# c976237222/HunyuanVideo_efficiency

Measured on AMD Instinct MI355X. Metric: denoise-steps/sec (720x1280x129f, HunyuanVideo DiT 20+40 blocks, bf16), higher is better.
Workload: dtype bf16

## Files before the change

hunyuanvideo_efficiency_amd/_lib.py:

```python
from __future__ import annotations

import ctypes as C
import os
import re

_HERE = os.path.dirname(os.path.abspath(__file__))
LIB_PATH = os.path.join(_HERE, "lib", "libhv_kernels.so")
TORCH_OPS_PATH = os.path.join(_HERE, "lib", "libhv_torch_ops.so")
ABI_VERSION = 8

_p, _i, _l, _f = C.c_void_p, C.c_int, C.c_int64, C.c_float

SIGNATURES = {
    "hv_abi_version": [],
    "hv_ln_modulate_bf16": [_p, _p, _p, _p, _l, _i, _l, _l, _f, _i, _p],
    "hv_qknorm_rope_bf16": [_p, _p, _p, _p, _p, _l, _l, _i, _i, _l, _l, _f, _p],
    "hv_qknorm_rope_scatter_bf16": [_p, _p, _p, _p, _p, _l, _l, _i, _i, _l, _l, _f, _p, _l, _i, _l, _p],
    "hv_gemm_bf16": [_p, _l, _p, _l, _p, _i, _i, _i, _p, _l, _i, _i, _p, _l, _i, _p, _p, _l, _p],
    "hv_linear_smallm_bf16": [_p, _p, _p, _p, _p, _i, _i, _i, _l, _l, _i, _p],
    "hv_timestep_embedding_bf16": [_p, _p, _i, _i, _f, _p],
    "hv_attn_fwd_bf16": [_p, _p, _p, _p, _l, _l, _l, _l, _i, _i, _i, _i, _f, _p, _l, _p],
    "hv_attn_workspace_bytes": [_i, _i, _i],
    "hv_attn_w4_loop_signature": [],
    "hv_attn_partial_bf16": [_p, _p, _p, _l, _l, _l, _i, _i, _i, _i, _f, _p, _p, _i, _i, _i, _p],
    "hv_attn_merge_bf16": [_p, _p, _p, _l, _i, _i, _i, _p],
    "hv_attn_suggest_splits": [_i, _i, _i],
    "hv_patchify_f32_bf16": [_p, _p, _i, _i, _i, _i, _p],
    "hv_unpatchify_bf16": [_p, _p, _i, _i, _i, _i, _l, _p],
    "hv_euler_step_f32": [_p, _p, _f, _l, _p],
    "hv_euler_step_f32_f32": [_p, _p, _f, _l, _p],
    "hv_masked_mean_bf16": [_p, _p, _p, _i, _i, _p],
    "hv_broadcast_row_bf16": [_p, _p, _l, _i, _l, _p],
    "hv_copy3d_bf16": [_p, _p, _i, _l, _i, _l, _l, _l, _l, _p],
    "hv_fp8_dequant_bf16": [_p, _p, _p, _l, _p],
    "hv_ln_modulate_fp8": [_p, _p, _p, _p, _p, _l, _i, _l, _l, _f, _p],
    "hv_quant_rows_fp8": [_p, _l, _p, _l, _p, _l, _i, _p],
    "hv_gemm_fp8": [_p, _l, _p, _p, _l, _p, _p, _i, _i, _i, _p, _l, _i, _i, _p, _l, _i, _p, _p, _l, _p],
    "hv_gemm_f16": [_p, _l, _p, _l, _p, _i, _i, _i, _p, _l, _i, _p, _l, _p],
    "hv_conv3d_causal_f16": [_p, _l, _p, _p, _p, _l, _i, _i, _i, _i, _i, _i, _i, _p, _l, _p, _l, _p],
    "hv_gn_partial_rows": [_l],
    "hv_subpixel_gn_partial_rows": [_i, _i, _i, _i],
    "hv_groupnorm_finalize_f16": [_p, _l, _l, _l, _i, _i, _f, _p, _p, _p, _p],
    "hv_groupnorm_affine_f16": [_p, _l, _l, _i, _i, _f, _p, _p, _p, _l, _p, _p],
    "hv_groupnorm_apply_f16": [_p, _l, _p, _l, _l, _i, _p, _i, _p],
    "hv_softmax_rows_f32_f16": [_p, _l, _p, _l, _i, _i, _i, _f, _i, _p],
    "hv_transpose_16b": [_p, _l, _p, _l, _i, _i, _p],
    "hv_conv3d_upsampled_subpixel_f16": [_p, _l, _p, _p, _i, _p, _p, _l, _i, _i, _i, _i, _i, _i, _p, _l, _p],
    "hv_conv3d_cout4_f16": [_p, _l, _p, _i, _p, _p, _p, _l, _i, _i, _i, _i, _i, _p, _l, _p],
    "hv_conv3d_cout4_planes_floats": [_l],
    "hv_conv3d_causal_strided_f16": [_p, _l, _p, _p, _p, _l, _i, _i, _i, _i, _i, _i, _i, _i, _p],
    "hv_temporal_resample_f16": [_p, _l, _p, _l, _i, _l, _i, _i, _i, _i, _p],
    "hv_vae_latent_tile_f16": [_p, _l, _l, _l, _l, _i, _i, _i, _i, _i, _p, _p],
    "hv_vae_blend_f16": [_p, _p, _p, _p, _p, _i, _i, _p],
    "hv_copy4d_16b": [_p, _p, _p, _p, _p, _p],
    "hv_vae_postprocess_f16_f32": [_p, _p, _l, _p],
    "hv_video_metrics": [_p, _l, _l, _l, _p, _l, _l, _l, _i, _i, _i, _i, _i, _i, _i, _p, _p, _p, _p, _l, _p],
    "hv_video_metrics_workspace_bytes": [_i, _i, _i, _i],
    "hv_lpips_conv1_f32": [_p, _l, _l, _l, _p, _l, _l, _l, _i, _i, _i, _i, _i, _p, _p, _p, _p, _p],
    "hv_lpips_conv2d_f32": [_p, _p, _p, _p, _i, _i, _i, _i, _i, _i, _i, _p],
    "hv_lpips_maxpool_f32": [_p, _p, _i, _i, _i, _i, _p],
    "hv_lpips_distance_f32": [_p, _p, _i, _l, _i, _i, _p, _p, _l, _p],
    "hv_lpips_distance_workspace_bytes": [_i, _l],
}


class HVKernelError(RuntimeError):
    pass


_lib = None


def load():
    global _lib
    if _lib is not None:
        return _lib
    if not os.path.exists(LIB_PATH):
        raise HVKernelError(
            f"{LIB_PATH} is missing: the HIP extension is not built (run __graft_entry__.build()). "
            "hunyuanvideo_efficiency_amd has no CPU or eager fallback.")
    lib = C.CDLL(LIB_PATH)
    for name, argtypes in SIGNATURES.items():
        try:
            fn = getattr(lib, name)
        except AttributeError as e:
            raise HVKernelError(f"{LIB_PATH} does not export {name}") from e
        fn.argtypes = argtypes
        fn.restype = C.c_int64 if name in ("hv_attn_workspace_bytes", "hv_gn_partial_rows", "hv_subpixel_gn_partial_rows", "hv_conv3d_cout4_planes_floats",
                                            "hv_video_metrics_workspace_bytes", "hv_lpips_distance_workspace_bytes") else C.c_int
    v = lib.hv_abi_version()
    if v != ABI_VERSION:
        raise HVKernelError(f"libhv_kernels ABI {v} != expected {ABI_VERSION}: rebuild the extension")
    inc = os.path.join(_HERE, "csrc", "hv_attention_w4_loop.inc")
    if os.path.exists(inc) and os.environ.get("HV_ALLOW_EXPERIMENT_LIB") != "1":
        with open(inc) as f:
            m = re.search(r"#define HV_W4_LOOP_SIGNATURE 0x([0-9a-f]{8})u", f.read(600))
        if m is None or (lib.hv_attn_w4_loop_signature() & 0xFFFFFFFF) != int(m.group(1), 16):
            raise HVKernelError(f"{LIB_PATH} was not compiled from {inc}: rebuild the extension (make -C hunyuanvideo_efficiency_amd/csrc); "
                                "HV_ALLOW_EXPERIMENT_LIB=1 admits a library built from another checkout (same-box A/Bs: tools/ab_attn.sh, tools/ab_run.sh)")
    _lib = lib
    return lib


def check(code: int, what: str):
    if code != 0:
        raise HVKernelError(f"{what} failed with code {code} "
                            f"({'bad argument' if code == -1 else 'launch failure' if code == -2 else 'unknown'})")


_hv = None


def torch_ops():
    global _hv
    if _hv is not None:
        return _hv
    import torch
    if not os.path.exists(TORCH_OPS_PATH):
        raise HVKernelError(
            f"{TORCH_OPS_PATH} is missing: the PyTorch custom-op library is not built (run __graft_entry__.build()). "
            "hunyuanvideo_efficiency_amd has no CPU or eager fallback.")
    torch.ops.load_library(TORCH_OPS_PATH)
    hv = torch.ops.hv
    v = int(hv.abi_version())
    if v != ABI_VERSION:
        raise HVKernelError(f"libhv_torch_ops / libhv_kernels ABI {v} != expected {ABI_VERSION}: rebuild the extension")
    for name in SIGNATURES:
        if not hasattr(hv, name[len("hv_"):]):
            raise HVKernelError(f"{TORCH_OPS_PATH} does not register torch.ops.hv.{name[len('hv_'):]}")
    _hv = hv
    return hv


def call(name: str, *args):
    op = getattr(torch_ops(), name)
    try:
        return op(*args)
    except (RuntimeError, NotImplementedError) as e:
        raise HVKernelError(f"hv::{name}: {str(e).splitlines()[0]}") from e


def host(name: str, *args) -> int:
    return int(getattr(torch_ops(), name)(*args))
```

hunyuanvideo_efficiency_amd/csrc/hv_api.hip:

```cpp
#include "hv_common.hpp"
#include "../../include/hv_kernels.h"
extern "C" int hv_abi_version(void) { return 8; }
```

hunyuanvideo_efficiency_amd/csrc/hv_attention.hip:

```cpp
#include "hv_attention.hpp"

using namespace hv_attn;

namespace {

constexpr int QTILE = 256;

__global__ __launch_bounds__(256) void attn_combine_kernel(const float* __restrict__ part_o, const float* __restrict__ part_ml,
                                                            bf16_t* __restrict__ o, int64_t so, int n_q, int n_heads, int n_splits) {
    const int64_t idx = (int64_t)blockIdx.x * blockDim.x + threadIdx.x;
    const int64_t total = (int64_t)n_q * n_heads * 32;
    if (idx >= total) return;
    const int d4 = (int)(idx & 31);
    const int64_t rh = idx >> 5;
    const int head = (int)(rh % n_heads);
    const int64_t row = rh / n_heads;
    float m = -INFINITY;
    for (int s = 0; s < n_splits; ++s) m = fmaxf(m, part_ml[(((int64_t)s * n_q + row) * n_heads + head) * 2]);
    float4 acc = make_float4(0.f, 0.f, 0.f, 0.f);
    float l = 0.f;
    for (int s = 0; s < n_splits; ++s) {
        const int64_t ri = ((int64_t)s * n_q + row) * n_heads + head;
        const float w = __builtin_amdgcn_exp2f(part_ml[ri * 2] - m);
        const float4 v = *reinterpret_cast<const float4*>(part_o + ri * D + d4 * 4);
        acc.x += v.x * w; acc.y += v.y * w; acc.z += v.z * w; acc.w += v.w * w;
        l += part_ml[ri * 2 + 1] * w;
    }
    const float inv = 1.0f / l;
    u32x2 w2;
    w2[0] = pack_bf2(acc.x * inv, acc.y * inv);
    w2[1] = pack_bf2(acc.z * inv, acc.w * inv);
    *reinterpret_cast<u32x2*>(o + row * so + head * D + d4 * 4) = w2;
}

int attn_launch(const AttnArgs& a, dim3 grid, hipStream_t stream) { return launch_w4(a, grid, stream); }

constexpr int KMAX_ROWS = 2048;
__global__ __launch_bounds__(256) void attn_kmax_kernel(const bf16_t* __restrict__ k, int64_t sk, int n_kv, unsigned* __restrict__ out) {
    __shared__ float wmax[4];
    const int head = blockIdx.y, t = threadIdx.x, ch = t & 15;
    const int r0 = blockIdx.x * KMAX_ROWS, r1 = min(r0 + KMAX_ROWS, n_kv);
    float best = 0.f;
    for (int row = r0 + (t >> 4); row < r1; row += 16) {
        const u32x4 w = *reinterpret_cast<const u32x4*>(k + (int64_t)row * sk + head * D + ch * 8);
        float s = 0.f;
#pragma unroll
        for (int j = 0; j < 4; ++j) {
            const float lo = bf2f_lo(w[j]), hi = bf2f_hi(w[j]);
            s += lo * lo + hi * hi;
        }
#pragma unroll
        for (int o = 8; o > 0; o >>= 1) s += __shfl_xor(s, o, 64);
        best = fmaxf(best, s);
    }
    best = fmaxf(best, __shfl_xor(best, 16, 64));
    best = fmaxf(best, __shfl_xor(best, 32, 64));
    if ((t & 63) == 0) wmax[t >> 6] = best;
    __syncthreads();
    if (t == 0) atomicMax(out + head, __float_as_uint(fmaxf(fmaxf(wmax[0], wmax[1]), fmaxf(wmax[2], wmax[3]))));
}

int attn_prepare_kmax(AttnArgs& a, void* workspace, int64_t workspace_bytes, hipStream_t stream) {
    a.kmax2 = nullptr;
    if (!workspace || workspace_bytes < KMAX_BYTES || a.n_heads > KMAX_HEADS || a.n_kv < 64 * KVT) return HV_OK;
    if (hipMemsetAsync(workspace, 0, KMAX_BYTES, stream) != hipSuccess) return HV_ERR_LAUNCH;
    attn_kmax_kernel<<<dim3((unsigned)((a.n_kv + KMAX_ROWS - 1) / KMAX_ROWS), (unsigned)a.n_heads), dim3(256), 0, stream>>>(a.k, a.sk, a.n_kv, (unsigned*)workspace);
    a.kmax2 = (const unsigned*)workspace;
    return HV_OK;
}

}

extern "C" int64_t hv_attn_workspace_bytes(int n_q, int n_kv, int n_heads) {
    (void)n_kv;
    return (int64_t)KMAX_BYTES + (int64_t)2 * n_q * n_heads * (128 + 2) * (int64_t)sizeof(float);
}

extern "C" int hv_attn_fwd_bf16(const void* q, const void* k, const void* v, void* o, int64_t stride_q, int64_t stride_k,
                                int64_t stride_v, int64_t stride_o, int n_q, int n_kv, int n_heads, int head_dim,
                                float scale, void* workspace, int64_t workspace_bytes, hipStream_t stream) {
    if (!q || !k || !v || !o || head_dim != D || n_heads <= 0 || n_q < 0 || n_kv < 0 || (stride_q & 7) || (stride_k & 7) ||
        (stride_v & 7) || (stride_o & 3))
        return HV_ERR_ARG;
    if (n_q == 0) return HV_OK;
    if (n_kv == 0) return HV_ERR_ARG;
    AttnArgs a;
    a.q = (const bf16_t*)q; a.k = (const bf16_t*)k; a.v = (const bf16_t*)v; a.o = (bf16_t*)o;
    a.sq = stride_q; a.sk = stride_k; a.sv = stride_v; a.so = stride_o;
    a.n_q = n_q; a.n_kv = n_kv; a.n_heads = n_heads;
    a.n_qtiles = (n_q + QTILE - 1) / QTILE;
    a.scale_log2e = scale * 1.4426950408889634f;
    a.n_splits = 1; a.split_keys = n_kv; a.part_o = nullptr; a.part_ml = nullptr; a.partial = 0;
    if (attn_prepare_kmax(a, workspace, workspace_bytes, stream) != HV_OK) return HV_ERR_LAUNCH;
    {
        const int64_t nwg = (int64_t)a.n_qtiles * n_heads;
        const int ntile = (n_kv + KVT - 1) / KVT;
        const double r1 = (double)((nwg + 255) / 256), r2 = 0.5 * (double)((2 * nwg + 255) / 256);
        if (workspace && ntile >= 64 && r2 < 0.97 * r1 && workspace_bytes >= hv_attn_workspace_bytes(n_q, n_kv, n_heads)) {
            a.n_splits = 2;
            a.split_keys = ((ntile + 1) / 2) * KVT;
            a.part_o = (float*)((char*)workspace + KMAX_BYTES);
            a.part_ml = a.part_o + (int64_t)2 * n_q * n_heads * D;
        }
    }
    if (attn_launch(a, dim3((unsigned)(a.n_qtiles * n_heads), (unsigned)a.n_splits), stream) != HV_OK) return HV_ERR_LAUNCH;
    if (a.n_splits > 1) {
        const int64_t total = (int64_t)n_q * n_heads * 32;
        attn_combine_kernel<<<dim3((unsigned)((total + 255) / 256)), dim3(256), 0, stream>>>(a.part_o, a.part_ml, a.o, a.so, n_q, n_heads,
                                                                                           a.n_splits);
    }
    return hv_check_launch();
}

extern "C" int hv_attn_partial_bf16(const void* q, const void* k, const void* v, int64_t stride_q, int64_t stride_k, int64_t stride_v,
                                    int n_q, int n_kv, int n_heads, int head_dim, float scale, void* part_o, void* part_ml,
                                    int n_slots, int slot, int splits, hipStream_t stream) {
    if (!q || !k || !v || !part_o || !part_ml || head_dim != D || n_heads <= 0 || n_q < 0 || n_kv <= 0 || (stride_q & 7) ||
        (stride_k & 7) || (stride_v & 7) || (splits != 1 && splits != 2) || slot < 0 || slot + splits > n_slots)
        return HV_ERR_ARG;
    if (n_q == 0) return HV_OK;
    const int ntile = (n_kv + KVT - 1) / KVT;
    if (splits == 2 && ntile < 2) return HV_ERR_ARG;
    AttnArgs a;
    a.q = (const bf16_t*)q; a.k = (const bf16_t*)k; a.v = (const bf16_t*)v; a.o = nullptr;
    a.sq = stride_q; a.sk = stride_k; a.sv = stride_v; a.so = 0;
    a.n_q = n_q; a.n_kv = n_kv; a.n_heads = n_heads;
    a.n_qtiles = (n_q + QTILE - 1) / QTILE;
    a.scale_log2e = scale * 1.4426950408889634f;
    a.n_splits = splits;
    a.split_keys = splits == 2 ? ((ntile + 1) / 2) * KVT : n_kv;
    a.part_o = (float*)part_o + (int64_t)slot * n_q * n_heads * D;
    a.part_ml = (float*)part_ml + (int64_t)slot * n_q * n_heads * 2;
    a.partial = 1;
    a.kmax2 = nullptr;
    if (attn_launch(a, dim3((unsigned)(a.n_qtiles * n_heads), (unsigned)splits), stream) != HV_OK) return HV_ERR_LAUNCH;
    return hv_check_launch();
}

extern "C" int hv_attn_merge_bf16(const void* part_o, const void* part_ml, void* o, int64_t stride_o, int n_q, int n_heads, int n_slots,
                                  hipStream_t stream) {
    if (!part_o || !part_ml || !o || n_heads <= 0 || n_q < 0 || n_slots <= 0 || (stride_o & 3)) return HV_ERR_ARG;
    if (n_q == 0) return HV_OK;
    const int64_t total = (int64_t)n_q * n_heads * 32;
    attn_combine_kernel<<<dim3((unsigned)((total + 255) / 256)), dim3(256), 0, stream>>>((const float*)part_o, (const float*)part_ml,
                                                                                       (bf16_t*)o, stride_o, n_q, n_heads, n_slots);
    return hv_check_launch();
}

extern "C" int hv_attn_suggest_splits(int n_q, int n_kv, int n_heads) {
    const int64_t nwg = (int64_t)((n_q + QTILE - 1) / QTILE) * n_heads;
    const int ntile = (n_kv + KVT - 1) / KVT;
    const double r1 = (double)((nwg + 255) / 256), r2 = 0.5 * (double)((2 * nwg + 255) / 256);
    return (ntile >= 64 && r2 < 0.97 * r1) ? 2 : 1;
}
```

hunyuanvideo_efficiency_amd/csrc/hv_attention.hpp:

```cpp
#pragma once
#include "hv_common.hpp"
#include "../../include/hv_kernels.h"
#include <type_traits>

namespace hv_attn {

constexpr int D = 128;
constexpr int KVT = 64;
constexpr int KV_TILE_BYTES = KVT * D * 2;

struct AttnArgs {
    const bf16_t* q; const bf16_t* k; const bf16_t* v; bf16_t* o;
    int64_t sq, sk, sv, so;
    int n_q, n_kv, n_heads, n_qtiles;
    float scale_log2e;
    int n_splits, split_keys;
    float* part_o;
    float* part_ml;
    int partial;
    const unsigned* kmax2;
};
constexpr int KMAX_BYTES = 256;
constexpr int KMAX_HEADS = 62;

typedef __attribute__((ext_vector_type(4))) short s16x4;
typedef __attribute__((address_space(3))) s16x4* lds_s16x4_ptr;
typedef __attribute__((address_space(3))) void* lds_void_ptr;

__device__ __forceinline__ float half_swap_max(float v) {
    auto r = __builtin_amdgcn_permlane32_swap(__float_as_uint(v), __float_as_uint(v), false, false);
    return fmaxf(__uint_as_float(r[0]), __uint_as_float(r[1]));
}
__device__ __forceinline__ float half_swap_sum(float v) {
    auto r = __builtin_amdgcn_permlane32_swap(__float_as_uint(v), __float_as_uint(v), false, false);
    return __uint_as_float(r[0]) + __uint_as_float(r[1]);
}

template <int I, int N, typename F>
__device__ __forceinline__ void static_for(F&& f) {
    if constexpr (I < N) {
        f(std::integral_constant<int, I>{});
        static_for<I + 1, N>(f);
    }
}

int launch_w4(const AttnArgs& a, dim3 grid, hipStream_t stream);

}
```

hunyuanvideo_efficiency_amd/csrc/hv_attention_w4.hip:

```cpp
#include "hv_attention.hpp"
#include "hv_agpr_clobbers.inc"

using namespace hv_attn;

namespace {

constexpr int W4_WAVES = 4, W4_QTILE = 256, W4_NBUF = 4;
constexpr int W4_KOFF = 0, W4_VOFF = W4_NBUF * KV_TILE_BYTES;
constexpr int W4_LDS = 2 * W4_NBUF * KV_TILE_BYTES;
constexpr int A_O = 0, A_Q = 128, A_KF = 192, A_VF = 224;
constexpr int RING = 8;
constexpr int PF = 4;
constexpr int WGRP = 2;
__host__ __device__ constexpr int frag_insts(int f) { return (f >= 16 && f < 32) ? 2 : 1; }
__host__ __device__ constexpr int wait_for(int f) { int n = 0; for (int i = WGRP; i < PF; ++i) n += frag_insts(f + i); return n; }

template <int KF, int QF, int WAIT>
__device__ __forceinline__ void mfma_s_first(f32x16& s, const f32x16& c) {
    if constexpr (WAIT >= 0)
        asm volatile("s_waitcnt lgkmcnt(%c6)\n\tv_mfma_f32_32x32x16_bf16 %0, a[%c2:%c3], a[%c4:%c5], %1"
                     : "=&v"(s) : "v"(c), "i"(KF), "i"(KF + 3), "i"(QF), "i"(QF + 3), "i"(WAIT) : HV_CLOBBER_ALL_AGPRS);
    else
        asm volatile("v_mfma_f32_32x32x16_bf16 %0, a[%c2:%c3], a[%c4:%c5], %1"
                     : "=&v"(s) : "v"(c), "i"(KF), "i"(KF + 3), "i"(QF), "i"(QF + 3) : HV_CLOBBER_ALL_AGPRS);
}
template <int KF, int QF, int WAIT>
__device__ __forceinline__ void mfma_s_zero(f32x16& s) {
    if constexpr (WAIT >= 0)
        asm volatile("s_waitcnt lgkmcnt(%c5)\n\tv_mfma_f32_32x32x16_bf16 %0, a[%c1:%c2], a[%c3:%c4], 0"
                     : "=&v"(s) : "i"(KF), "i"(KF + 3), "i"(QF), "i"(QF + 3), "i"(WAIT));
    else
        asm volatile("v_mfma_f32_32x32x16_bf16 %0, a[%c1:%c2], a[%c3:%c4], 0" : "=&v"(s) : "i"(KF), "i"(KF + 3), "i"(QF), "i"(QF + 3));
}
template <int KF, int QF, int WAIT>
__device__ __forceinline__ void mfma_s(f32x16& s) {
    if constexpr (WAIT >= 0)
        asm volatile("s_waitcnt lgkmcnt(%c5)\n\tv_mfma_f32_32x32x16_bf16 %0, a[%c1:%c2], a[%c3:%c4], %0"
                     : "+v"(s) : "i"(KF), "i"(KF + 3), "i"(QF), "i"(QF + 3), "i"(WAIT) : HV_CLOBBER_ALL_AGPRS);
    else
        asm volatile("v_mfma_f32_32x32x16_bf16 %0, a[%c1:%c2], a[%c3:%c4], %0" : "+v"(s) : "i"(KF), "i"(KF + 3), "i"(QF), "i"(QF + 3) : HV_CLOBBER_ALL_AGPRS);
}
template <int OT, int VF, int WAIT>
__device__ __forceinline__ void mfma_pv(const u32x4& p) {
    if constexpr (WAIT >= 0)
        asm volatile("s_waitcnt lgkmcnt(%c5)\n\tv_mfma_f32_32x32x16_bf16 a[%c1:%c2], a[%c3:%c4], %0, a[%c1:%c2]"
                     : : "v"(p), "i"(OT), "i"(OT + 15), "i"(VF), "i"(VF + 3), "i"(WAIT) : HV_CLOBBER_ALL_AGPRS);
    else
        asm volatile("v_mfma_f32_32x32x16_bf16 a[%c1:%c2], a[%c3:%c4], %0, a[%c1:%c2]" : : "v"(p), "i"(OT), "i"(OT + 15), "i"(VF), "i"(VF + 3) : HV_CLOBBER_ALL_AGPRS);
}
template <int AF, int OFF>
__device__ __forceinline__ void lds_k(uint32_t addr) {
    asm volatile("ds_read_b128 a[%c1:%c2], %0 offset:%c3" : : "v"(addr), "i"(AF), "i"(AF + 3), "i"(OFF));
}
template <int AF, int OFF>
__device__ __forceinline__ void lds_v(uint32_t addr) {
    asm volatile("ds_read_b64_tr_b16 a[%c1:%c2], %0 offset:%c5\n\tds_read_b64_tr_b16 a[%c3:%c4], %0 offset:%c6"
                 : : "v"(addr), "i"(AF), "i"(AF + 1), "i"(AF + 2), "i"(AF + 3), "i"(OFF), "i"(OFF + 8 * 256));
}
__device__ __forceinline__ void add_pinned(float& acc, float p) { asm volatile("v_add_f32 %0, %0, %1" : "+v"(acc) : "v"(p)); }
__device__ __forceinline__ void exp2_pinned(float& d, float x) { asm volatile("v_exp_f32 %0, %1" : "=v"(d) : "v"(x)); }
__device__ __forceinline__ void pack_pinned(uint32_t& w, float lo, float hi) { asm volatile("v_cvt_pk_bf16_f32 %0, %1, %2" : "=v"(w) : "v"(lo), "v"(hi)); }
__device__ __forceinline__ void max3_pinned(float& acc, float x, float y) { asm volatile("v_max3_f32 %0, %0, %1, %2" : "+v"(acc) : "v"(x), "v"(y)); }
template <int N>
__device__ __forceinline__ void acc_write(uint32_t v) { asm volatile("v_accvgpr_write_b32 a%c1, %0" : : "v"(v), "i"(N)); }
template <int N>
__device__ __forceinline__ float acc_read() {
    float v;
    asm volatile("v_accvgpr_read_b32 %0, a%c1" : "=v"(v) : "i"(N));
    return v;
}

#include "hv_attention_w4_loop.inc"

__host__ __device__ constexpr int exps_before(int g) { return g <= 32 ? g + (g + 3) / 4 : (g <= 56 ? 40 + (g - 32) : 64); }
__host__ __device__ constexpr int exps_in(int g) { return exps_before(g + 1) - exps_before(g); }

__global__ __launch_bounds__(256, 1) void attn_fwd_kernel_w4(AttnArgs a) {
#if defined(__HIP_DEVICE_COMPILE__)
    extern __shared__ __attribute__((aligned(16))) char smem[];
    const int tid = threadIdx.x, lane = tid & 63, wave = tid >> 6;
    const int lr = lane & 31, lh = lane >> 5;
    const int head = blockIdx.x / a.n_qtiles;
    const int qt = blockIdx.x % a.n_qtiles;
    if (a.n_splits > 1) {
        const int kv0 = blockIdx.y * a.split_keys;
        a.k += (int64_t)kv0 * a.sk;
        a.v += (int64_t)kv0 * a.sv;
        a.n_kv = min(a.n_kv - kv0, a.split_keys);
    }
    const int q0 = qt * W4_QTILE + wave * 64;
    const uint32_t lds0 = (uint32_t)(uintptr_t)smem;

    asm volatile("; hv_attention_w4: a[0:255] owned by inline asm" : : : HV_CLOBBER_ALL_AGPRS);
    static_for<0, 128>([&](auto I) { asm volatile("v_accvgpr_write_b32 a%c0, 0" : : "i"(A_O + decltype(I)::value)); });
    float qn2[2] = {0.f, 0.f};
#pragma unroll
    for (int qb = 0; qb < 2; ++qb) {
        const int qrow = min(q0 + qb * 32 + lr, a.n_q - 1);
        const bf16_t* qp = a.q + (int64_t)qrow * a.sq + head * D + lh * 8;
        u32x4 raw[8];
#pragma unroll
        for (int ks = 0; ks < 8; ++ks) raw[ks] = *reinterpret_cast<const u32x4*>(qp + ks * 16);
        static_for<0, 32>([&](auto I) {
            constexpr int i = decltype(I)::value;
            const uint32_t w = raw[i >> 2][i & 3];
            const uint32_t sc = pack_bf2(bf2f_lo(w) * a.scale_log2e, bf2f_hi(w) * a.scale_log2e);
            qn2[qb] += bf2f_lo(sc) * bf2f_lo(sc) + bf2f_hi(sc) * bf2f_hi(sc);
            if (qb == 0) acc_write<A_Q + i>(sc);
            else acc_write<A_Q + 32 + i>(sc);
        });
    }

    constexpr int KEYS_W = KVT / W4_WAVES, NP = KEYS_W / 4;
    const char* kbase = reinterpret_cast<const char*>(a.k + head * D);
    const char* vbase = reinterpret_cast<const char*>(a.v + head * D);
    const int k_row_bytes = (int)a.sk * 2, v_row_bytes = (int)a.sv * 2;
    uint32_t koff_row, koff_sw, voff0;
    {
        const int key = KEYS_W * wave + (lane >> 4), dcp = lane & 15;
        koff_row = (uint32_t)(key * k_row_bytes);
        koff_sw = (uint32_t)((dcp ^ (key & 3)) << 4);
        voff0 = (uint32_t)(key * v_row_bytes + ((dcp ^ ((key & 3) << 2)) << 4));
    }
    u32x4 koff4, voff4;
#pragma unroll
    for (int i = 0; i < NP; ++i) {
        koff4[i] = koff_row + (koff_sw ^ (uint32_t)(i << 6)) + (uint32_t)(4 * i * k_row_bytes) - (uint32_t)(i * 1024);
        voff4[i] = voff0 + (uint32_t)(4 * i * v_row_bytes) - (uint32_t)(i * 1024);
    }
    const int wave_u = __builtin_amdgcn_readfirstlane(wave);
    const int wave_lds = wave_u * (KEYS_W * 256);
    const int64_t k_tile_bytes = (int64_t)KVT * a.sk * 2, v_tile_bytes = (int64_t)KVT * a.sv * 2;
    auto k_rsrc = [&](const char* tile_ptr, int rows) { return __builtin_amdgcn_make_buffer_rsrc((void*)tile_ptr, 0, rows * k_row_bytes, 0x00020000); };
    auto v_rsrc = [&](const char* tile_ptr, int rows) { return __builtin_amdgcn_make_buffer_rsrc((void*)tile_ptr, 0, rows * v_row_bytes, 0x00020000); };
    auto dma_k_piece = [&](auto rsrc, int lds_off, int i) {
        __builtin_amdgcn_raw_ptr_buffer_load_lds(rsrc, (lds_void_ptr)(smem + lds_off + wave_lds + i * 1024), 16, koff_row + (koff_sw ^ (uint32_t)(i << 6)), 4 * i * k_row_bytes, 0, 0);
    };
    auto dma_v_piece = [&](auto rsrc, int lds_off, int i) {
        __builtin_amdgcn_raw_ptr_buffer_load_lds(rsrc, (lds_void_ptr)(smem + lds_off + wave_lds + i * 1024), 16, voff0, 4 * i * v_row_bytes, 0, 0);
    };
    auto tile_rows = [&](int tile) { return min(a.n_kv - tile * KVT, KVT); };
    auto dma_k = [&](int tile, int buf) {
        auto r = k_rsrc(kbase + tile * k_tile_bytes, tile_rows(tile));
#pragma unroll
        for (int i = 0; i < NP; ++i) dma_k_piece(r, W4_KOFF + buf * KV_TILE_BYTES, i);
    };
    auto dma_v = [&](int tile, int buf) {
        auto r = v_rsrc(vbase + tile * v_tile_bytes, tile_rows(tile));
#pragma unroll
        for (int i = 0; i < NP; ++i) dma_v_piece(r, W4_VOFF + buf * KV_TILE_BYTES, i);
    };

    uint32_t kread0, vread;
    {
        kread0 = lds0 + W4_KOFF + lr * 256 + ((lh ^ (lr & 15)) << 4);
        const int vq = (lane & 15) >> 2, vp = lane & 3, vG = lane >> 4;
        const int key = 4 * (vG >> 1) + vq;
        const int chunk16 = ((vG & 1) * 16 + 4 * vp) >> 3;
        vread = lds0 + W4_VOFF + key * 256 + ((chunk16 ^ ((key & 3) << 2)) << 4) + (vp & 1) * 8;
    }
    u32x4 vks_lo, vks_hi, vv4;
#pragma unroll
    for (int i = 0; i < 4; ++i) {
        vks_lo[i] = kread0 ^ (uint32_t)(i << 5);
        vks_hi[i] = kread0 ^ (uint32_t)((i + 4) << 5);
        vv4[i] = vread ^ (uint32_t)(i << 6);
    }
    uint32_t vk0, vv[4];
    auto set_vk = [&](int buf_bytes) { vk0 = kread0 + buf_bytes; };
    auto set_vv = [&](int buf_bytes) {
        const uint32_t b = vread + buf_bytes;
#pragma unroll
        for (int db = 0; db < 4; ++db) vv[db] = b ^ (db << 6);
    };

    float m_run[2] = {0.f, 0.f}, l_run[2] = {0.f, 0.f};
    float l2_run[2] = {0.f, 0.f};
    f32x16 negm[2];
    constexpr float THR = 8.0f;
    bool static_max = false;
    const int ntiles = (a.n_kv + KVT - 1) / KVT;

    auto tile_max = [&](f32x16 (&S)[2][2], int t, bool last, float (&mx)[2]) __attribute__((always_inline)) {
        if (last && (a.n_kv & (KVT - 1))) {
            const int kbase_i = t * KVT + 4 * lh;
#pragma unroll
            for (int qb = 0; qb < 2; ++qb)
#pragma unroll
                for (int kb = 0; kb < 2; ++kb)
#pragma unroll
                    for (int r = 0; r < 16; ++r) {
                        const int key = kbase_i + kb * 32 + (r & 3) + 8 * (r >> 2);
                        if (key >= a.n_kv) S[qb][kb][r] = -INFINITY;
                    }
        }
#pragma unroll
        for (int qb = 0; qb < 2; ++qb) {
            float m = S[qb][0][0];
#pragma unroll
            for (int r = 1; r < 16; ++r) m = fmaxf(m, S[qb][0][r]);
#pragma unroll
            for (int r = 0; r < 16; ++r) m = fmaxf(m, S[qb][1][r]);
            mx[qb] = half_swap_max(m);
        }
    };
    auto raise_max = [&](f32x16 (&Sc)[2][2], const float (&mx)[2]) __attribute__((always_inline)) {
        asm volatile("s_nop 7\n\ts_nop 7\n\ts_nop 7" ::: "memory");
        static_for<0, 2>([&](auto QB) {
            constexpr int qb = decltype(QB)::value;
            if (__any(mx[qb] > THR)) {
                const float d = fmaxf(half_swap_max(mx[qb]), 0.f);
                const float alpha = __builtin_amdgcn_exp2f(-d);
                l_run[qb] = (l_run[qb] + l2_run[qb]) * alpha;
                l2_run[qb] = 0.f;
                m_run[qb] += d;
#pragma unroll
                for (int kb = 0; kb < 2; ++kb)
#pragma unroll
                    for (int r = 0; r < 16; ++r) Sc[qb][kb][r] -= d;
#pragma unroll
                for (int r = 0; r < 16; ++r) negm[qb][r] = -m_run[qb];
                static_for<0, 64>([&](auto I) {
                    constexpr int n = A_O + 64 * qb + decltype(I)::value;
                    float o = acc_read<n>();
                    o *= alpha;
                    acc_write<n>(__float_as_uint(o));
                });
                asm volatile("s_nop 3" ::: "memory");
            }
        });
        asm volatile("" : "+v"(negm[0]), "+v"(negm[1]));
    };

    auto body = [&](f32x16 (&Sc)[2][2], f32x16 (&Sn)[2][2], int t, const float (&mx_c)[2], float (&mx_n)[2]) __attribute__((always_inline)) {
        constexpr bool FULL = false;
        if (!static_max && __any(mx_c[0] > THR || mx_c[1] > THR)) raise_max(Sc, mx_c);
        const int rb0 = (t & 3) * KV_TILE_BYTES, rb2 = ((t + 2) & 3) * KV_TILE_BYTES, rb3 = ((t + 3) & 3) * KV_TILE_BYTES;
        const bool do_k = FULL || (t + 3 < ntiles), do_v = FULL || (t + 2 < ntiles);
        u32x4 pw[2][4];
        float ex[64];
        float mxa[2] = {-INFINITY, -INFINITY};
        const auto krs = k_rsrc(kbase + (FULL ? t + 3 : min(t + 3, ntiles - 1)) * k_tile_bytes, FULL ? KVT : tile_rows(min(t + 3, ntiles - 1)));
        const auto vrs = v_rsrc(vbase + (FULL ? t + 2 : min(t + 2, ntiles - 1)) * v_tile_bytes, FULL ? KVT : tile_rows(min(t + 2, ntiles - 1)));
        auto add_e = [&](auto Ec) {
            constexpr int e = decltype(Ec)::value, qb = (e >> 3) & 1;
            add_pinned(l_run[qb], ex[e]);
        };
        auto exp_e = [&](auto Ec) {
            constexpr int e = decltype(Ec)::value, kk = e >> 4, qb = (e >> 3) & 1, j = e & 7;
            exp2_pinned(ex[e], Sc[qb][kk >> 1][8 * (kk & 1) + j]);
        };
        auto pack_e = [&](auto Ec) {
            constexpr int e = decltype(Ec)::value, kk = e >> 4, qb = (e >> 3) & 1, j = e & 7;
            if constexpr (j & 1) {
                uint32_t w;
// ... 264 lines not shown
```

hunyuanvideo_efficiency_amd/csrc/hv_common.hpp:

```cpp
#pragma once
#include <hip/hip_runtime.h>
#include <stdint.h>

#define HV_OK 0
#define HV_ERR_ARG (-1)
#define HV_ERR_LAUNCH (-2)

typedef __attribute__((ext_vector_type(8))) __bf16 bf16x8;
typedef __attribute__((ext_vector_type(4))) __bf16 bf16x4;
typedef __attribute__((ext_vector_type(2))) __bf16 bf16x2;
typedef __attribute__((ext_vector_type(4))) float f32x4;
typedef __attribute__((ext_vector_type(16))) float f32x16;
typedef __attribute__((ext_vector_type(4))) uint32_t u32x4;
typedef __attribute__((ext_vector_type(2))) uint32_t u32x2;
typedef __attribute__((ext_vector_type(2))) float f32x2;

typedef uint16_t bf16_t;

__device__ __forceinline__ float bf2f(bf16_t v) { return __uint_as_float(((uint32_t)v) << 16); }
__device__ __forceinline__ float bf2f_lo(uint32_t w) { return __uint_as_float(w << 16); }
__device__ __forceinline__ float bf2f_hi(uint32_t w) { return __uint_as_float(w & 0xFFFF0000u); }
__device__ __forceinline__ bf16_t f2bf(float f) {
    __bf16 h = (__bf16)f;
    return __builtin_bit_cast(bf16_t, h);
}
__device__ __forceinline__ uint32_t pack_bf2(float lo, float hi) {
    bf16x2 v;
    v[0] = (__bf16)lo;
    v[1] = (__bf16)hi;
    return __builtin_bit_cast(uint32_t, v);
}
__device__ __forceinline__ float rbf(float f) { return bf2f(f2bf(f)); }

__device__ __forceinline__ void unpack8(const u32x4& w, float (&f)[8]) {
#pragma unroll
    for (int i = 0; i < 4; ++i) {
        f[2 * i] = bf2f_lo(w[i]);
        f[2 * i + 1] = bf2f_hi(w[i]);
    }
}
__device__ __forceinline__ u32x4 pack8(const float (&f)[8]) {
    u32x4 w;
#pragma unroll
    for (int i = 0; i < 4; ++i) w[i] = pack_bf2(f[2 * i], f[2 * i + 1]);
    return w;
}

typedef _Float16 h16;
__device__ __forceinline__ float h2f(uint16_t v) { return (float)__builtin_bit_cast(h16, v); }
__device__ __forceinline__ uint16_t f2h(float f) { return __builtin_bit_cast(uint16_t, (h16)f); }
__device__ __forceinline__ float rh(float f) { return (float)(h16)f; }
__device__ __forceinline__ void unpack8h(const u32x4& w, float (&f)[8]) {
#pragma unroll
    for (int i = 0; i < 4; ++i) {
        f[2 * i] = h2f((uint16_t)(w[i] & 0xFFFFu));
        f[2 * i + 1] = h2f((uint16_t)(w[i] >> 16));
    }
}
__device__ __forceinline__ u32x4 pack8h(const float (&f)[8]) {
    u32x4 w;
#pragma unroll
    for (int i = 0; i < 4; ++i) w[i] = (uint32_t)f2h(f[2 * i]) | ((uint32_t)f2h(f[2 * i + 1]) << 16);
    return w;
}

template <typename T, typename Op>
__device__ __forceinline__ T wave_reduce(T v, Op op) {
#pragma unroll
    for (int o = 32; o > 0; o >>= 1) v = op(v, __shfl_xor(v, o, 64));
    return v;
}
struct WaveAdd {
    template <typename T> __device__ __forceinline__ T operator()(T a, T b) const { return a + b; }
};
struct WaveMax {
    __device__ __forceinline__ float operator()(float a, float b) const { return fmaxf(a, b); }
    __device__ __forceinline__ int operator()(int a, int b) const { return max(a, b); }
};
struct WaveMin {
    __device__ __forceinline__ int operator()(int a, int b) const { return min(a, b); }
};
template <typename T> __device__ __forceinline__ T wave_sum(T v) { return wave_reduce(v, WaveAdd{}); }
template <typename T> __device__ __forceinline__ T wave_max(T v) { return wave_reduce(v, WaveMax{}); }
template <typename T> __device__ __forceinline__ T wave_min(T v) { return wave_reduce(v, WaveMin{}); }

__device__ __forceinline__ float gelu_tanh_f(float x) {
    const float k0 = 0.7978845608028654f, k1 = 0.044715f;
    float u = k0 * (x + k1 * x * x * x);
    float e = __builtin_amdgcn_exp2f(u * 2.8853900817779268f);
    float t = 1.0f - 2.0f * __builtin_amdgcn_rcpf(e + 1.0f);
    return 0.5f * x * (1.0f + t);
}
__device__ __forceinline__ float silu_f(float x) { return x * __builtin_amdgcn_rcpf(1.0f + __expf(-x)); }

__device__ __forceinline__ uint32_t quantise(float x, int rescale) {
    if (rescale) x = __fmul_rn(__fadd_rn(x, 1.0f), 0.5f);
    x = fminf(fmaxf(x, 0.0f), 1.0f);
    return (uint32_t)(int)__fmul_rn(x, 255.0f);
}

struct HvPerDeviceOnce { bool done[64] = {}; };
static inline int hv_set_max_lds(HvPerDeviceOnce& once, const void* fn, int bytes) {
    int dev = 0;
    if (hipGetDevice(&dev) != hipSuccess || dev < 0 || dev >= 64) return HV_ERR_LAUNCH;
    if (!once.done[dev]) {
        if (hipFuncSetAttribute(fn, hipFuncAttributeMaxDynamicSharedMemorySize, bytes) != hipSuccess) return HV_ERR_LAUNCH;
        once.done[dev] = true;
    }
    return HV_OK;
}

static inline int hv_check_launch() {
    hipError_t e = hipGetLastError();
    return e == hipSuccess ? HV_OK : HV_ERR_LAUNCH;
}

__device__ __forceinline__ f32x2 f16x2_minus(uint32_t w, float plo, float phi) {
    float lo, hi;
    asm("v_fma_mix_f32 %0, %1, 1.0, -%2 op_sel_hi:[1,0,0]" : "=v"(lo) : "v"(w), "v"(plo));
    asm("v_fma_mix_f32 %0, %1, 1.0, -%2 op_sel:[1,0,0] op_sel_hi:[1,0,0]" : "=v"(hi) : "v"(w), "v"(phi));
    return f32x2{lo, hi};
}
```

hunyuanvideo_efficiency_amd/csrc/hv_rowwise.hip:

```cpp
#include "hv_common.hpp"
#include "../../include/hv_kernels.h"
#include <type_traits>


template <int MAXC>
__device__ __forceinline__ float ln_load_row(const bf16_t* xr, int lane, int nchunk, float (&v)[MAXC][8]) {
    float s = 0.f;
#pragma unroll
    for (int c = 0; c < MAXC; ++c) {
        const int ch = lane + c * 64;
        if (ch < nchunk) {
            unpack8(*reinterpret_cast<const u32x4*>(xr + ch * 8), v[c]);
#pragma unroll
            for (int j = 0; j < 8; ++j) s += v[c][j];
        }
    }
    return s;
}
__device__ __forceinline__ void ln_load_coeffs(const bf16_t* mul, const bf16_t* add, int ch, int mode,
                                               float (&m)[8], float (&a)[8]) {
    if (mul) {
        unpack8(*reinterpret_cast<const u32x4*>(mul + ch * 8), m);
        if (mode == 0) {
#pragma unroll
// ... 113 lines not shown
            }
        }
    }
    const float rstd = rsqrtf(wave_sum(q) / (float)D + eps);
    float amax = 0.f;
#pragma unroll
    for (int c = 0; c < MAXC; ++c) {
        const int ch = lane + c * 64;
        if (ch < nchunk) {
            float m[8], a[8];
            ln_load_coeffs(mul, add, ch, 0, m, a);
#pragma unroll
            for (int j = 0; j < 8; ++j) {
                v[c][j] = rbf((v[c][j] - mean) * rstd * m[j] + a[j]);
                amax = fmaxf(amax, fabsf(v[c][j]));
            }
        }
    }
    const float sc = fp8_row_scale(wave_max(amax));
    const float inv = 1.0f / sc;
    if (lane == 0) row_scale[row] = sc;
    uint8_t* orow = out + row * ldo;
#pragma unroll
    for (int c = 0; c < MAXC; ++c) {
        const int ch = lane + c * 64;
        if (ch < nchunk) *reinterpret_cast<u32x2*>(orow + ch * 8) = pack8_fp8(v[c], inv);
    }
}

extern "C" int hv_ln_modulate_fp8(const void* x, const void* shift, const void* scale, void* out_q, float* out_row_scale, int64_t M,
                                  int D, int64_t ldx, int64_t ldq, float eps, hipStream_t stream) {
    if (!x || !out_q || !out_row_scale || M < 0 || D <= 0 || (D & 7) || D > 4096 || (ldx & 7) || (ldq & 15)) return HV_ERR_ARG;
    if (M == 0) return HV_OK;
    dim3 grid((unsigned)((M + 3) / 4)), block(256);
    const bf16_t *xp = (const bf16_t*)x, *ap = (const bf16_t*)shift, *mp = (const bf16_t*)scale;
    ln_dispatch_maxc(D, [&](auto maxc) {
        ln_mod_fp8_kernel<decltype(maxc)::value><<<grid, block, 0, stream>>>(xp, ap, mp, (uint8_t*)out_q, out_row_scale, M, D, ldx, ldq, eps);
    });
    return hv_check_launch();
}

__global__ __launch_bounds__(256) void quant_rows_fp8_kernel(const bf16_t* __restrict__ x, int64_t ldx, uint8_t* __restrict__ out,
                                                              int64_t ldo, float* __restrict__ row_scale, int64_t M, int K) {
    const int lane = threadIdx.x & 63;
    const int64_t row = (int64_t)blockIdx.x * 4 + (threadIdx.x >> 6);
    if (row >= M) return;
    const bf16_t* xr = x + row * ldx;
    const int nchunk = K >> 3;
    float amax = 0.f;
    for (int ch = lane; ch < nchunk; ch += 64) {
        float f[8];
        unpack8(*reinterpret_cast<const u32x4*>(xr + ch * 8), f);
#pragma unroll
        for (int j = 0; j < 8; ++j) amax = fmaxf(amax, fabsf(f[j]));
    }
    const float sc = fp8_row_scale(wave_max(amax));
    const float inv = 1.0f / sc;
    if (lane == 0) row_scale[row] = sc;
    uint8_t* orow = out + row * ldo;
    for (int ch = lane; ch < nchunk; ch += 64) {
        float f[8];
        unpack8(*reinterpret_cast<const u32x4*>(xr + ch * 8), f);
        *reinterpret_cast<u32x2*>(orow + ch * 8) = pack8_fp8(f, inv);
    }
}

extern "C" int hv_quant_rows_fp8(const void* x, int64_t ldx, void* out_q, int64_t ldq, float* out_row_scale, int64_t M, int K,
                                 hipStream_t stream) {
    if (!x || !out_q || !out_row_scale || M < 0 || K <= 0 || (K & 7) || (ldx & 7) || (ldq & 15)) return HV_ERR_ARG;
    if (M == 0) return HV_OK;
    quant_rows_fp8_kernel<<<dim3((unsigned)((M + 3) / 4)), dim3(256), 0, stream>>>((const bf16_t*)x, ldx, (uint8_t*)out_q, ldq,
                                                                                  out_row_scale, M, K);
    return hv_check_launch();
}

__global__ __launch_bounds__(256) void qknorm_rope_kernel(bf16_t* __restrict__ qkv, const bf16_t* __restrict__ qw,
                                                           const bf16_t* __restrict__ kw, const float* __restrict__ cosT,
                                                           const float* __restrict__ sinT, int64_t n_rows, int64_t n_rope,
                                                           int H, int64_t ld, int64_t k_off, float eps, bf16_t* __restrict__ dst,
                                                           int64_t dst_ld, int hpb, int64_t dst_bs) {
    const int64_t row = blockIdx.x;
    const int sub = threadIdx.x & 15;
    const int grp = threadIdx.x >> 4;
    float wq[8], wk[8], c[8], s[8];
    unpack8(*reinterpret_cast<const u32x4*>(qw + sub * 8), wq);
    unpack8(*reinterpret_cast<const u32x4*>(kw + sub * 8), wk);
    const bool rope = row < n_rope;
    if (rope) {
        const float4* cp = reinterpret_cast<const float4*>(cosT + row * 128 + sub * 8);
        const float4* sp = reinterpret_cast<const float4*>(sinT + row * 128 + sub * 8);
        float4 c0 = cp[0], c1 = cp[1], s0 = sp[0], s1 = sp[1];
        c[0] = c0.x, c[1] = c0.y, c[2] = c0.z, c[3] = c0.w, c[4] = c1.x, c[5] = c1.y, c[6] = c1.z, c[7] = c1.w;
        s[0] = s0.x, s[1] = s0.y, s[2] = s0.z, s[3] = s0.w, s[4] = s1.x, s[5] = s1.y, s[6] = s1.z, s[7] = s1.w;
    }
    for (int hv = grp; hv < 2 * H; hv += 16) {
        const bool is_k = hv >= H;
        const int h = is_k ? hv - H : hv;
        bf16_t* p = qkv + row * ld + (is_k ? k_off : 0) + h * 128 + sub * 8;
        float x[8];
        unpack8(*reinterpret_cast<const u32x4*>(p), x);
        if (dst) p = dst + (int64_t)(hv / hpb) * dst_bs + row * dst_ld + (hv % hpb) * 128 + sub * 8;
        float ss = 0.f;
#pragma unroll
        for (int j = 0; j < 8; ++j) ss += x[j] * x[j];
#pragma unroll
        for (int o = 8; o > 0; o >>= 1) ss += __shfl_xor(ss, o, 16);
        const float r = rsqrtf(ss * (1.0f / 128.0f) + eps);
        float y[8];
#pragma unroll
        for (int j = 0; j < 8; ++j) y[j] = rbf(rbf(x[j] * r) * (is_k ? wk[j] : wq[j]));
        if (rope) {
            float o[8];
#pragma unroll
            for (int j = 0; j < 8; j += 2) {
                o[j] = y[j] * c[j] - y[j + 1] * s[j];
                o[j + 1] = y[j + 1] * c[j + 1] + y[j] * s[j + 1];
            }
            *reinterpret_cast<u32x4*>(p) = pack8(o);
        } else {
            *reinterpret_cast<u32x4*>(p) = pack8(y);
        }
    }
}

extern "C" int hv_qknorm_rope_bf16(void* qkv, const void* q_weight, const void* k_weight, const float* cos_tab,
                                   const float* sin_tab, int64_t n_rows, int64_t n_rope, int n_heads, int head_dim,
                                   int64_t ld, int64_t k_offset, float eps, hipStream_t stream) {
    if (!qkv || !q_weight || !k_weight || head_dim != 128 || n_heads <= 0 || n_rows < 0 || n_rope < 0 ||
        n_rope > n_rows || (ld & 7) || (k_offset & 7) || (n_rope > 0 && (!cos_tab || !sin_tab)))
        return HV_ERR_ARG;
    if (n_rows == 0) return HV_OK;
    qknorm_rope_kernel<<<dim3((unsigned)n_rows), dim3(256), 0, stream>>>((bf16_t*)qkv, (const bf16_t*)q_weight,
                                                                          (const bf16_t*)k_weight, cos_tab, sin_tab, n_rows,
                                                                          n_rope, n_heads, ld, k_offset, eps, nullptr, 0, 1, 0);
    return hv_check_launch();
}

extern "C" int hv_qknorm_rope_scatter_bf16(const void* qkv, const void* q_weight, const void* k_weight, const float* cos_tab,
                                           const float* sin_tab, int64_t n_rows, int64_t n_rope, int n_heads, int head_dim,
                                           int64_t ld, int64_t k_offset, float eps, void* dst, int64_t dst_ld,
                                           int heads_per_block, int64_t dst_block_stride, hipStream_t stream) {
    if (!qkv || !dst || !q_weight || !k_weight || head_dim != 128 || n_heads <= 0 || n_rows < 0 || n_rope < 0 || n_rope > n_rows ||
        (ld & 7) || (k_offset & 7) || (dst_ld & 7) || (dst_block_stride & 7) || heads_per_block <= 0 ||
        (n_rope > 0 && (!cos_tab || !sin_tab)))
        return HV_ERR_ARG;
    if (n_rows == 0) return HV_OK;
    qknorm_rope_kernel<<<dim3((unsigned)n_rows), dim3(256), 0, stream>>>((bf16_t*)const_cast<void*>(qkv), (const bf16_t*)q_weight,
                                                                          (const bf16_t*)k_weight, cos_tab, sin_tab, n_rows, n_rope,
                                                                          n_heads, ld, k_offset, eps, (bf16_t*)dst, dst_ld,
                                                                          heads_per_block, dst_block_stride);
    return hv_check_launch();
}

template <int MM>
__global__ __launch_bounds__(256) void gemv_kernel(const bf16_t* __restrict__ x, const bf16_t* __restrict__ W,
                                                    const bf16_t* __restrict__ b, const bf16_t* __restrict__ addend,
                                                    bf16_t* __restrict__ out, int N, int K, int64_t ldx, int64_t ldo, int act) {
    const int lane = threadIdx.x & 63;
    const int n = blockIdx.x * 4 + (threadIdx.x >> 6);
    if (n >= N) return;
    float acc[MM];
#pragma unroll
    for (int m = 0; m < MM; ++m) acc[m] = 0.f;
    const bf16_t* wr = W + (int64_t)n * K;
    for (int k0 = lane * 8; k0 < K; k0 += 512) {
        float w[8];
        unpack8(*reinterpret_cast<const u32x4*>(wr + k0), w);
#pragma unroll
        for (int m = 0; m < MM; ++m) {
            float xv[8];
            unpack8(*reinterpret_cast<const u32x4*>(x + m * ldx + k0), xv);
#pragma unroll
            for (int j = 0; j < 8; ++j) {
                float a = xv[j];
                if (act & 1) a = rbf(silu_f(a));
                acc[m] += a * w[j];
            }
        }
    }
#pragma unroll
    for (int m = 0; m < MM; ++m) {
        float r = wave_sum(acc[m]);
        if (lane == 0) {
            if (b) r += bf2f(b[n]);
            if (act & 2) r = silu_f(rbf(r));
            if (addend) r = rbf(r) + bf2f(addend[m * ldo + n]);
            out[m * ldo + n] = f2bf(r);
        }
    }
}

extern "C" int hv_linear_smallm_bf16(const void* x, const void* W, const void* bias, const void* addend, void* out, int M,
                                     int N, int K, int64_t ldx, int64_t ldo, int act, hipStream_t stream) {
    if (!x || !W || !out || M < 1 || M > 4 || N < 1 || K < 8 || (K & 7) || (ldx & 7)) return HV_ERR_ARG;
    dim3 grid((N + 3) / 4), block(256);
    const bf16_t *xp = (const bf16_t*)x, *wp = (const bf16_t*)W, *bp = (const bf16_t*)bias, *ap = (const bf16_t*)addend;
    bf16_t* op = (bf16_t*)out;
    switch (M) {
        case 1: gemv_kernel<1><<<grid, block, 0, stream>>>(xp, wp, bp, ap, op, N, K, ldx, ldo, act); break;
        case 2: gemv_kernel<2><<<grid, block, 0, stream>>>(xp, wp, bp, ap, op, N, K, ldx, ldo, act); break;
        case 3: gemv_kernel<3><<<grid, block, 0, stream>>>(xp, wp, bp, ap, op, N, K, ldx, ldo, act); break;
        default: gemv_kernel<4><<<grid, block, 0, stream>>>(xp, wp, bp, ap, op, N, K, ldx, ldo, act); break;
    }
    return hv_check_launch();
}

__global__ __launch_bounds__(256) void patchify_kernel(const float* __restrict__ x, bf16_t* __restrict__ A, int C, int T,
                                                        int H, int W) {
    const int Hp = H >> 1, Wp = W >> 1;
    const int64_t ntok = (int64_t)T * Hp * Wp;
    const int64_t idx = (int64_t)blockIdx.x * blockDim.x + threadIdx.x;
    if (idx >= ntok * C) return;
    const int c = (int)(idx % C);
    const int64_t tok = idx / C;
    const int w = (int)(tok % Wp), h = (int)((tok / Wp) % Hp), t = (int)(tok / ((int64_t)Wp * Hp));
    const float* p = x + (((int64_t)c * T + t) * H + 2 * h) * W + 2 * w;
    float2 r0 = *reinterpret_cast<const float2*>(p);
    float2 r1 = *reinterpret_cast<const float2*>(p + W);
    u32x2 o;
    o[0] = pack_bf2(r0.x, r0.y);
    o[1] = pack_bf2(r1.x, r1.y);
    *reinterpret_cast<u32x2*>(A + tok * (C * 4) + c * 4) = o;
}

extern "C" int hv_patchify_f32_bf16(const float* x, void* A, int C, int T, int H, int W, hipStream_t stream) {
    if (!x || !A || C <= 0 || T <= 0 || H <= 0 || W <= 0 || (H & 1) || (W & 1)) return HV_ERR_ARG;
    const int64_t n = (int64_t)T * (H / 2) * (W / 2) * C;
    patchify_kernel<<<dim3((unsigned)((n + 255) / 256)), dim3(256), 0, stream>>>(x, (bf16_t*)A, C, T, H, W);
    return hv_check_launch();
}

__global__ __launch_bounds__(256) void unpatchify_kernel(const bf16_t* __restrict__ y, bf16_t* __restrict__ out, int C,
                                                          int T, int H, int W, int64_t ldy) {
    const int Hp = H >> 1, Wp = W >> 1;
    const int64_t ntok = (int64_t)T * Hp * Wp;
    const int64_t idx = (int64_t)blockIdx.x * blockDim.x + threadIdx.x;
    if (idx >= ntok * C) return;
    const int64_t tok = idx % ntok;
    const int c = (int)(idx / ntok);
    const int w = (int)(tok % Wp), h = (int)((tok / Wp) % Hp), t = (int)(tok / ((int64_t)Wp * Hp));
    u32x2 v = *reinterpret_cast<const u32x2*>(y + tok * ldy + c * 4);
    bf16_t* p = out + (((int64_t)c * T + t) * H + 2 * h) * W + 2 * w;
    *reinterpret_cast<uint32_t*>(p) = v[0];
    *reinterpret_cast<uint32_t*>(p + W) = v[1];
}

extern "C" int hv_unpatchify_bf16(const void* y, void* out, int C, int T, int H, int W, int64_t ldy, hipStream_t stream) {
    if (!y || !out || C <= 0 || T <= 0 || (H & 1) || (W & 1) || (ldy & 3)) return HV_ERR_ARG;
    const int64_t n = (int64_t)T * (H / 2) * (W / 2) * C;
    unpatchify_kernel<<<dim3((unsigned)((n + 255) / 256)), dim3(256), 0, stream>>>((const bf16_t*)y, (bf16_t*)out, C, T, H,
                                                                                  W, ldy);
    return hv_check_launch();
}

__global__ __launch_bounds__(256) void euler_kernel(float* __restrict__ s, const bf16_t* __restrict__ v, float dt, int64_t n) {
    const int64_t i = ((int64_t)blockIdx.x * blockDim.x + threadIdx.x) * 4;
    if (i + 3 < n) {
        float4 a = *reinterpret_cast<float4*>(s + i);
        u32x2 w = *reinterpret_cast<const u32x2*>(v + i);
        a.x += bf2f_lo(w[0]) * dt, a.y += bf2f_hi(w[0]) * dt, a.z += bf2f_lo(w[1]) * dt, a.w += bf2f_hi(w[1]) * dt;
        *reinterpret_cast<float4*>(s + i) = a;
    } else {
        for (int64_t j = i; j < n; ++j) s[j] += bf2f(v[j]) * dt;
    }
}

extern "C" int hv_euler_step_f32(float* sample, const void* model_out_bf16, float dt, int64_t n, hipStream_t stream) {
    if (!sample || !model_out_bf16 || n < 0) return HV_ERR_ARG;
    if (n == 0) return HV_OK;
    euler_kernel<<<dim3((unsigned)((n / 4 + 256) / 256)), dim3(256), 0, stream>>>(sample, (const bf16_t*)model_out_bf16, dt, n);
    return hv_check_launch();
}

__global__ __launch_bounds__(256) void euler_f32_kernel(float* __restrict__ s, const float* __restrict__ v, float dt, int64_t n) {
    const int64_t i = ((int64_t)blockIdx.x * blockDim.x + threadIdx.x) * 4;
    if (i + 3 < n) {
        float4 a = *reinterpret_cast<float4*>(s + i);
        const float4 b = *reinterpret_cast<const float4*>(v + i);
        a.x += b.x * dt, a.y += b.y * dt, a.z += b.z * dt, a.w += b.w * dt;
        *reinterpret_cast<float4*>(s + i) = a;
    } else {
        for (int64_t j = i; j < n; ++j) s[j] += v[j] * dt;
    }
}

extern "C" int hv_euler_step_f32_f32(float* sample, const float* model_out_f32, float dt, int64_t n, hipStream_t stream) {
    if (!sample || !model_out_f32 || n < 0) return HV_ERR_ARG;
    if (n == 0) return HV_OK;
    euler_f32_kernel<<<dim3((unsigned)((n / 4 + 256) / 256)), dim3(256), 0, stream>>>(sample, model_out_f32, dt, n);
    return hv_check_launch();
}

__global__ __launch_bounds__(256) void masked_mean_kernel(const bf16_t* __restrict__ x, const int* __restrict__ mask,
                                                           bf16_t* __restrict__ out, int L, int D) {
    const int d = blockIdx.x * blockDim.x + threadIdx.x;
    if (d >= D) return;
    float s = 0.f, c = 0.f;
    for (int l = 0; l < L; ++l) {
        const float m = mask ? (float)mask[l] : 1.0f;
        s += bf2f(x[(int64_t)l * D + d]) * m;
        c += m;
    }
    out[d] = f2bf(s / c);
}

extern "C" int hv_masked_mean_bf16(const void* x, const int* mask, void* out, int L, int D, hipStream_t stream) {
// ... 96 lines not shown
```

hunyuanvideo_efficiency_amd/csrc/hv_torch_ops.cpp:

```cpp
#include <torch/library.h>
#include <ATen/core/Tensor.h>
#include <c10/hip/HIPStream.h>
#include <c10/hip/HIPGuard.h>
#include <optional>
#include <vector>
#include "../../include/hv_kernels.h"

namespace {
using OptT = std::optional<at::Tensor>;

struct Dev {
    c10::DeviceIndex idx = -1;
    const char* op;
    explicit Dev(const char* o) : op(o) {}
    void* p(const OptT& t, const char* name) {
        if (!t.has_value() || !t->defined()) return nullptr;
        TORCH_CHECK(t->is_cuda(), "hv::", op, ": ", name, " must be a GPU tensor (this library has no CPU path), got ", t->device());
        if (idx < 0) idx = t->device().index();
        TORCH_CHECK(t->device().index() == idx, "hv::", op, ": ", name, " is on a different GPU than the other tensors");
        return t->data_ptr();
    }
};

inline void check_rc(int rc, const char* op) {
    TORCH_CHECK(rc == 0, "hv::", op, " failed with code ", rc, rc == -1 ? " (bad argument)" : rc == -2 ? " (launch failure)" : "");
}

int64_t op_abi_version() {
    return (int64_t)hv_abi_version();
}

void op_ln_modulate_bf16(const OptT& x, const OptT& shift_or_bias, const OptT& scale_or_weight, const OptT& out, int64_t M, int64_t D, int64_t ldx, int64_t ldo, double eps, int64_t mode) {
    Dev dev("ln_modulate_bf16");
    auto a0 = (const void*)dev.p(x, "x");
    auto a1 = (const void*)dev.p(shift_or_bias, "shift_or_bias");
    auto a2 = (const void*)dev.p(scale_or_weight, "scale_or_weight");
    auto a3 = (void*)dev.p(out, "out");
    TORCH_CHECK(dev.idx >= 0, "hv::ln_modulate_bf16: needs at least one GPU tensor");
    c10::hip::HIPGuard guard(dev.idx);
    hipStream_t stream = c10::hip::getCurrentHIPStream(dev.idx).stream();
    check_rc(hv_ln_modulate_bf16(a0, a1, a2, a3, (int64_t)M, (int)D, (int64_t)ldx, (int64_t)ldo, (float)eps, (int)mode, stream), "ln_modulate_bf16");
}

void op_qknorm_rope_bf16(const OptT& qkv, const OptT& q_weight, const OptT& k_weight, const OptT& cos_tab, const OptT& sin_tab, int64_t n_rows, int64_t n_rope, int64_t n_heads, int64_t head_dim, int64_t ld, int64_t k_offset, double eps) {
    Dev dev("qknorm_rope_bf16");
    auto a0 = (void*)dev.p(qkv, "qkv");
    auto a1 = (const void*)dev.p(q_weight, "q_weight");
    auto a2 = (const void*)dev.p(k_weight, "k_weight");
    auto a3 = (const float*)dev.p(cos_tab, "cos_tab");
    auto a4 = (const float*)dev.p(sin_tab, "sin_tab");
    TORCH_CHECK(dev.idx >= 0, "hv::qknorm_rope_bf16: needs at least one GPU tensor");
    c10::hip::HIPGuard guard(dev.idx);
    hipStream_t stream = c10::hip::getCurrentHIPStream(dev.idx).stream();
    check_rc(hv_qknorm_rope_bf16(a0, a1, a2, a3, a4, (int64_t)n_rows, (int64_t)n_rope, (int)n_heads, (int)head_dim, (int64_t)ld, (int64_t)k_offset, (float)eps, stream), "qknorm_rope_bf16");
}

void op_qknorm_rope_scatter_bf16(const OptT& qkv, const OptT& q_weight, const OptT& k_weight, const OptT& cos_tab, const OptT& sin_tab, int64_t n_rows, int64_t n_rope, int64_t n_heads, int64_t head_dim, int64_t ld, int64_t k_offset, double eps, const OptT& dst, int64_t dst_ld, int64_t heads_per_block, int64_t dst_block_stride) {
    Dev dev("qknorm_rope_scatter_bf16");
    auto a0 = (const void*)dev.p(qkv, "qkv");
    auto a1 = (const void*)dev.p(q_weight, "q_weight");
    auto a2 = (const void*)dev.p(k_weight, "k_weight");
    auto a3 = (const float*)dev.p(cos_tab, "cos_tab");
    auto a4 = (const float*)dev.p(sin_tab, "sin_tab");
    auto a12 = (void*)dev.p(dst, "dst");
    TORCH_CHECK(dev.idx >= 0, "hv::qknorm_rope_scatter_bf16: needs at least one GPU tensor");
    c10::hip::HIPGuard guard(dev.idx);
    hipStream_t stream = c10::hip::getCurrentHIPStream(dev.idx).stream();
    check_rc(hv_qknorm_rope_scatter_bf16(a0, a1, a2, a3, a4, (int64_t)n_rows, (int64_t)n_rope, (int)n_heads, (int)head_dim, (int64_t)ld, (int64_t)k_offset, (float)eps, a12, (int64_t)dst_ld, (int)heads_per_block, (int64_t)dst_block_stride, stream), "qknorm_rope_scatter_bf16");
}

void op_gemm_bf16(const OptT& A, int64_t lda, const OptT& W, int64_t ldw, const OptT& bias, int64_t M, int64_t N, int64_t K, const OptT& out0, int64_t ld0, int64_t act0, int64_t n_split, const OptT& out1, int64_t ld1, int64_t act1, const OptT& gate, const OptT& res, int64_t ld_res) {
    Dev dev("gemm_bf16");
    auto a0 = (const void*)dev.p(A, "A");
    auto a2 = (const void*)dev.p(W, "W");
    auto a4 = (const void*)dev.p(bias, "bias");
    auto a8 = (void*)dev.p(out0, "out0");
    auto a12 = (void*)dev.p(out1, "out1");
    auto a15 = (const void*)dev.p(gate, "gate");
    auto a16 = (const void*)dev.p(res, "res");
    TORCH_CHECK(dev.idx >= 0, "hv::gemm_bf16: needs at least one GPU tensor");
    c10::hip::HIPGuard guard(dev.idx);
    hipStream_t stream = c10::hip::getCurrentHIPStream(dev.idx).stream();
    check_rc(hv_gemm_bf16(a0, (int64_t)lda, a2, (int64_t)ldw, a4, (int)M, (int)N, (int)K, a8, (int64_t)ld0, (int)act0, (int)n_split, a12, (int64_t)ld1, (int)act1, a15, a16, (int64_t)ld_res, stream), "gemm_bf16");
}

void op_linear_smallm_bf16(const OptT& x, const OptT& W, const OptT& bias, const OptT& addend, const OptT& out, int64_t M, int64_t N, int64_t K, int64_t ldx, int64_t ldo, int64_t act) {
    Dev dev("linear_smallm_bf16");
    auto a0 = (const void*)dev.p(x, "x");
    auto a1 = (const void*)dev.p(W, "W");
    auto a2 = (const void*)dev.p(bias, "bias");
    auto a3 = (const void*)dev.p(addend, "addend");
    auto a4 = (void*)dev.p(out, "out");
    TORCH_CHECK(dev.idx >= 0, "hv::linear_smallm_bf16: needs at least one GPU tensor");
    c10::hip::HIPGuard guard(dev.idx);
    hipStream_t stream = c10::hip::getCurrentHIPStream(dev.idx).stream();
    check_rc(hv_linear_smallm_bf16(a0, a1, a2, a3, a4, (int)M, (int)N, (int)K, (int64_t)ldx, (int64_t)ldo, (int)act, stream), "linear_smallm_bf16");
}

void op_timestep_embedding_bf16(const OptT& t, const OptT& out, int64_t n_t, int64_t dim, double max_period) {
    Dev dev("timestep_embedding_bf16");
    auto a0 = (const float*)dev.p(t, "t");
    auto a1 = (void*)dev.p(out, "out");
    TORCH_CHECK(dev.idx >= 0, "hv::timestep_embedding_bf16: needs at least one GPU tensor");
    c10::hip::HIPGuard guard(dev.idx);
    hipStream_t stream = c10::hip::getCurrentHIPStream(dev.idx).stream();
    check_rc(hv_timestep_embedding_bf16(a0, a1, (int)n_t, (int)dim, (float)max_period, stream), "timestep_embedding_bf16");
}

void op_attn_fwd_bf16(const OptT& q, const OptT& k, const OptT& v, const OptT& o, int64_t stride_q, int64_t stride_k, int64_t stride_v, int64_t stride_o, int64_t n_q, int64_t n_kv, int64_t n_heads, int64_t head_dim, double scale, const OptT& workspace, int64_t workspace_bytes) {
    Dev dev("attn_fwd_bf16");
    auto a0 = (const void*)dev.p(q, "q");
    auto a1 = (const void*)dev.p(k, "k");
    auto a2 = (const void*)dev.p(v, "v");
    auto a3 = (void*)dev.p(o, "o");
    auto a13 = (void*)dev.p(workspace, "workspace");
    TORCH_CHECK(dev.idx >= 0, "hv::attn_fwd_bf16: needs at least one GPU tensor");
    c10::hip::HIPGuard guard(dev.idx);
    hipStream_t stream = c10::hip::getCurrentHIPStream(dev.idx).stream();
    check_rc(hv_attn_fwd_bf16(a0, a1, a2, a3, (int64_t)stride_q, (int64_t)stride_k, (int64_t)stride_v, (int64_t)stride_o, (int)n_q, (int)n_kv, (int)n_heads, (int)head_dim, (float)scale, a13, (int64_t)workspace_bytes, stream), "attn_fwd_bf16");
}

int64_t op_attn_workspace_bytes(int64_t n_q, int64_t n_kv, int64_t n_heads) {
    return (int64_t)hv_attn_workspace_bytes((int)n_q, (int)n_kv, (int)n_heads);
}

int64_t op_attn_w4_loop_signature() {
    return (int64_t)hv_attn_w4_loop_signature();
}

void op_attn_partial_bf16(const OptT& q, const OptT& k, const OptT& v, int64_t stride_q, int64_t stride_k, int64_t stride_v, int64_t n_q, int64_t n_kv, int64_t n_heads, int64_t head_dim, double scale, const OptT& part_o, const OptT& part_ml, int64_t n_slots, int64_t slot, int64_t splits) {
    Dev dev("attn_partial_bf16");
    auto a0 = (const void*)dev.p(q, "q");
    auto a1 = (const void*)dev.p(k, "k");
    auto a2 = (const void*)dev.p(v, "v");
    auto a11 = (void*)dev.p(part_o, "part_o");
    auto a12 = (void*)dev.p(part_ml, "part_ml");
    TORCH_CHECK(dev.idx >= 0, "hv::attn_partial_bf16: needs at least one GPU tensor");
    c10::hip::HIPGuard guard(dev.idx);
    hipStream_t stream = c10::hip::getCurrentHIPStream(dev.idx).stream();
    check_rc(hv_attn_partial_bf16(a0, a1, a2, (int64_t)stride_q, (int64_t)stride_k, (int64_t)stride_v, (int)n_q, (int)n_kv, (int)n_heads, (int)head_dim, (float)scale, a11, a12, (int)n_slots, (int)slot, (int)splits, stream), "attn_partial_bf16");
}

void op_attn_merge_bf16(const OptT& part_o, const OptT& part_ml, const OptT& o, int64_t stride_o, int64_t n_q, int64_t n_heads, int64_t n_slots) {
    Dev dev("attn_merge_bf16");
    auto a0 = (const void*)dev.p(part_o, "part_o");
    auto a1 = (const void*)dev.p(part_ml, "part_ml");
    auto a2 = (void*)dev.p(o, "o");
    TORCH_CHECK(dev.idx >= 0, "hv::attn_merge_bf16: needs at least one GPU tensor");
    c10::hip::HIPGuard guard(dev.idx);
    hipStream_t stream = c10::hip::getCurrentHIPStream(dev.idx).stream();
    check_rc(hv_attn_merge_bf16(a0, a1, a2, (int64_t)stride_o, (int)n_q, (int)n_heads, (int)n_slots, stream), "attn_merge_bf16");
}

int64_t op_attn_suggest_splits(int64_t n_q, int64_t n_kv, int64_t n_heads) {
    return (int64_t)hv_attn_suggest_splits((int)n_q, (int)n_kv, (int)n_heads);
}

void op_patchify_f32_bf16(const OptT& x, const OptT& A, int64_t C, int64_t T, int64_t H, int64_t W) {
    Dev dev("patchify_f32_bf16");
    auto a0 = (const float*)dev.p(x, "x");
    auto a1 = (void*)dev.p(A, "A");
    TORCH_CHECK(dev.idx >= 0, "hv::patchify_f32_bf16: needs at least one GPU tensor");
    c10::hip::HIPGuard guard(dev.idx);
    hipStream_t stream = c10::hip::getCurrentHIPStream(dev.idx).stream();
    check_rc(hv_patchify_f32_bf16(a0, a1, (int)C, (int)T, (int)H, (int)W, stream), "patchify_f32_bf16");
}

void op_unpatchify_bf16(const OptT& y, const OptT& out, int64_t C, int64_t T, int64_t H, int64_t W, int64_t ldy) {
    Dev dev("unpatchify_bf16");
    auto a0 = (const void*)dev.p(y, "y");
    auto a1 = (void*)dev.p(out, "out");
    TORCH_CHECK(dev.idx >= 0, "hv::unpatchify_bf16: needs at least one GPU tensor");
    c10::hip::HIPGuard guard(dev.idx);
    hipStream_t stream = c10::hip::getCurrentHIPStream(dev.idx).stream();
    check_rc(hv_unpatchify_bf16(a0, a1, (int)C, (int)T, (int)H, (int)W, (int64_t)ldy, stream), "unpatchify_bf16");
}

void op_euler_step_f32(const OptT& sample, const OptT& model_out_bf16, double dt, int64_t n) {
    Dev dev("euler_step_f32");
    auto a0 = (float*)dev.p(sample, "sample");
    auto a1 = (const void*)dev.p(model_out_bf16, "model_out_bf16");
    TORCH_CHECK(dev.idx >= 0, "hv::euler_step_f32: needs at least one GPU tensor");
    c10::hip::HIPGuard guard(dev.idx);
    hipStream_t stream = c10::hip::getCurrentHIPStream(dev.idx).stream();
    check_rc(hv_euler_step_f32(a0, a1, (float)dt, (int64_t)n, stream), "euler_step_f32");
}

void op_euler_step_f32_f32(const OptT& sample, const OptT& model_out_f32, double dt, int64_t n) {
    Dev dev("euler_step_f32_f32");
    auto a0 = (float*)dev.p(sample, "sample");
    auto a1 = (const float*)dev.p(model_out_f32, "model_out_f32");
    TORCH_CHECK(dev.idx >= 0, "hv::euler_step_f32_f32: needs at least one GPU tensor");
    c10::hip::HIPGuard guard(dev.idx);
    hipStream_t stream = c10::hip::getCurrentHIPStream(dev.idx).stream();
    check_rc(hv_euler_step_f32_f32(a0, a1, (float)dt, (int64_t)n, stream), "euler_step_f32_f32");
}

void op_masked_mean_bf16(const OptT& x, const OptT& mask, const OptT& out, int64_t L, int64_t D) {
    Dev dev("masked_mean_bf16");
    auto a0 = (const void*)dev.p(x, "x");
    auto a1 = (const int*)dev.p(mask, "mask");
    auto a2 = (void*)dev.p(out, "out");
    TORCH_CHECK(dev.idx >= 0, "hv::masked_mean_bf16: needs at least one GPU tensor");
    c10::hip::HIPGuard guard(dev.idx);
    hipStream_t stream = c10::hip::getCurrentHIPStream(dev.idx).stream();
    check_rc(hv_masked_mean_bf16(a0, a1, a2, (int)L, (int)D, stream), "masked_mean_bf16");
}

void op_broadcast_row_bf16(const OptT& src, const OptT& dst, int64_t n_rows, int64_t D, int64_t ld) {
    Dev dev("broadcast_row_bf16");
    auto a0 = (const void*)dev.p(src, "src");
    auto a1 = (void*)dev.p(dst, "dst");
    TORCH_CHECK(dev.idx >= 0, "hv::broadcast_row_bf16: needs at least one GPU tensor");
    c10::hip::HIPGuard guard(dev.idx);
    hipStream_t stream = c10::hip::getCurrentHIPStream(dev.idx).stream();
    check_rc(hv_broadcast_row_bf16(a0, a1, (int64_t)n_rows, (int)D, (int64_t)ld, stream), "broadcast_row_bf16");
}

void op_copy3d_bf16(const OptT& src, const OptT& dst, int64_t n_batch, int64_t rows, int64_t cols, int64_t src_batch_stride, int64_t src_ld, int64_t dst_batch_stride, int64_t dst_ld) {
    Dev dev("copy3d_bf16");
    auto a0 = (const void*)dev.p(src, "src");
    auto a1 = (void*)dev.p(dst, "dst");
    TORCH_CHECK(dev.idx >= 0, "hv::copy3d_bf16: needs at least one GPU tensor");
    c10::hip::HIPGuard guard(dev.idx);
    hipStream_t stream = c10::hip::getCurrentHIPStream(dev.idx).stream();
    check_rc(hv_copy3d_bf16(a0, a1, (int)n_batch, (int64_t)rows, (int)cols, (int64_t)src_batch_stride, (int64_t)src_ld, (int64_t)dst_batch_stride, (int64_t)dst_ld, stream), "copy3d_bf16");
}

void op_fp8_dequant_bf16(const OptT& w_e4m3fn, const OptT& scale_bf16, const OptT& out_bf16, int64_t n) {
    Dev dev("fp8_dequant_bf16");
    auto a0 = (const void*)dev.p(w_e4m3fn, "w_e4m3fn");
    auto a1 = (const void*)dev.p(scale_bf16, "scale_bf16");
    auto a2 = (void*)dev.p(out_bf16, "out_bf16");
    TORCH_CHECK(dev.idx >= 0, "hv::fp8_dequant_bf16: needs at least one GPU tensor");
    c10::hip::HIPGuard guard(dev.idx);
    hipStream_t stream = c10::hip::getCurrentHIPStream(dev.idx).stream();
    check_rc(hv_fp8_dequant_bf16(a0, a1, a2, (int64_t)n, stream), "fp8_dequant_bf16");
}

void op_ln_modulate_fp8(const OptT& x, const OptT& shift, const OptT& scale, const OptT& out_q, const OptT& out_row_scale, int64_t M, int64_t D, int64_t ldx, int64_t ldq, double eps) {
    Dev dev("ln_modulate_fp8");
    auto a0 = (const void*)dev.p(x, "x");
    auto a1 = (const void*)dev.p(shift, "shift");
    auto a2 = (const void*)dev.p(scale, "scale");
    auto a3 = (void*)dev.p(out_q, "out_q");
    auto a4 = (float*)dev.p(out_row_scale, "out_row_scale");
    TORCH_CHECK(dev.idx >= 0, "hv::ln_modulate_fp8: needs at least one GPU tensor");
    c10::hip::HIPGuard guard(dev.idx);
    hipStream_t stream = c10::hip::getCurrentHIPStream(dev.idx).stream();
    check_rc(hv_ln_modulate_fp8(a0, a1, a2, a3, a4, (int64_t)M, (int)D, (int64_t)ldx, (int64_t)ldq, (float)eps, stream), "ln_modulate_fp8");
}

void op_quant_rows_fp8(const OptT& x, int64_t ldx, const OptT& out_q, int64_t ldq, const OptT& out_row_scale, int64_t M, int64_t K) {
    Dev dev("quant_rows_fp8");
    auto a0 = (const void*)dev.p(x, "x");
    auto a2 = (void*)dev.p(out_q, "out_q");
    auto a4 = (float*)dev.p(out_row_scale, "out_row_scale");
    TORCH_CHECK(dev.idx >= 0, "hv::quant_rows_fp8: needs at least one GPU tensor");
    c10::hip::HIPGuard guard(dev.idx);
    hipStream_t stream = c10::hip::getCurrentHIPStream(dev.idx).stream();
    check_rc(hv_quant_rows_fp8(a0, (int64_t)ldx, a2, (int64_t)ldq, a4, (int64_t)M, (int)K, stream), "quant_rows_fp8");
}

void op_gemm_fp8(const OptT& A_q, int64_t lda, const OptT& a_row_scale, const OptT& W_q, int64_t ldw, const OptT& w_scale_bf16, const OptT& bias, int64_t M, int64_t N, int64_t K, const OptT& out0, int64_t ld0, int64_t act0, int64_t n_split, const OptT& out1, int64_t ld1, int64_t act1, const OptT& gate, const OptT& res, int64_t ld_res) {
    Dev dev("gemm_fp8");
    auto a0 = (const void*)dev.p(A_q, "A_q");
    auto a2 = (const float*)dev.p(a_row_scale, "a_row_scale");
    auto a3 = (const void*)dev.p(W_q, "W_q");
    auto a5 = (const void*)dev.p(w_scale_bf16, "w_scale_bf16");
    auto a6 = (const void*)dev.p(bias, "bias");
    auto a10 = (void*)dev.p(out0, "out0");
    auto a14 = (void*)dev.p(out1, "out1");
// ... 125 lines not shown
    auto a2 = (void*)dev.p(y, "y");
    auto a6 = (const float*)dev.p(affine, "affine");
    TORCH_CHECK(dev.idx >= 0, "hv::groupnorm_apply_f16: needs at least one GPU tensor");
    c10::hip::HIPGuard guard(dev.idx);
    hipStream_t stream = c10::hip::getCurrentHIPStream(dev.idx).stream();
    check_rc(hv_groupnorm_apply_f16(a0, (int64_t)ldx, a2, (int64_t)ldy, (int64_t)M, (int)C, a6, (int)silu, stream), "groupnorm_apply_f16");
}

void op_softmax_rows_f32_f16(const OptT& S, int64_t ld_s, const OptT& P, int64_t ld_p, int64_t rows, int64_t cols, int64_t cols_pad, double scale, int64_t causal_block) {
    Dev dev("softmax_rows_f32_f16");
    auto a0 = (const float*)dev.p(S, "S");
    auto a2 = (void*)dev.p(P, "P");
    TORCH_CHECK(dev.idx >= 0, "hv::softmax_rows_f32_f16: needs at least one GPU tensor");
    c10::hip::HIPGuard guard(dev.idx);
    hipStream_t stream = c10::hip::getCurrentHIPStream(dev.idx).stream();
    check_rc(hv_softmax_rows_f32_f16(a0, (int64_t)ld_s, a2, (int64_t)ld_p, (int)rows, (int)cols, (int)cols_pad, (float)scale, (int)causal_block, stream), "softmax_rows_f32_f16");
}

void op_transpose_16b(const OptT& src, int64_t ld_src, const OptT& dst, int64_t ld_dst, int64_t R, int64_t C) {
    Dev dev("transpose_16b");
    auto a0 = (const void*)dev.p(src, "src");
    auto a2 = (void*)dev.p(dst, "dst");
    TORCH_CHECK(dev.idx >= 0, "hv::transpose_16b: needs at least one GPU tensor");
    c10::hip::HIPGuard guard(dev.idx);
    hipStream_t stream = c10::hip::getCurrentHIPStream(dev.idx).stream();
    check_rc(hv_transpose_16b(a0, (int64_t)ld_src, a2, (int64_t)ld_dst, (int)R, (int)C, stream), "transpose_16b");
}

void op_vae_latent_tile_f16(const OptT& z, int64_t sc, int64_t st, int64_t sh, int64_t sw, int64_t C, int64_t T, int64_t H, int64_t W, int64_t Cpad, const OptT& out) {
    Dev dev("vae_latent_tile_f16");
    auto a0 = (const float*)dev.p(z, "z");
    auto a10 = (void*)dev.p(out, "out");
    TORCH_CHECK(dev.idx >= 0, "hv::vae_latent_tile_f16: needs at least one GPU tensor");
    c10::hip::HIPGuard guard(dev.idx);
    hipStream_t stream = c10::hip::getCurrentHIPStream(dev.idx).stream();
    check_rc(hv_vae_latent_tile_f16(a0, (int64_t)sc, (int64_t)st, (int64_t)sh, (int64_t)sw, (int)C, (int)T, (int)H, (int)W, (int)Cpad, a10, stream), "vae_latent_tile_f16");
}

void op_vae_blend_f16(const OptT& a, at::IntArrayRef a_strides, const OptT& b, at::IntArrayRef b_strides, at::IntArrayRef dims, int64_t axis, int64_t extent) {
    Dev dev("vae_blend_f16");
    TORCH_CHECK(a_strides.size() == 4, "hv::vae_blend_f16: a_strides must have 4 elements, got ", a_strides.size());
    TORCH_CHECK(b_strides.size() == 4, "hv::vae_blend_f16: b_strides must have 4 elements, got ", b_strides.size());
    TORCH_CHECK(dims.size() == 4, "hv::vae_blend_f16: dims must have 4 elements, got ", dims.size());
    std::vector<int> dims_i(dims.begin(), dims.end());
    auto a0 = (const void*)dev.p(a, "a");
    auto a2 = (void*)dev.p(b, "b");
    TORCH_CHECK(dev.idx >= 0, "hv::vae_blend_f16: needs at least one GPU tensor");
    c10::hip::HIPGuard guard(dev.idx);
    hipStream_t stream = c10::hip::getCurrentHIPStream(dev.idx).stream();
    check_rc(hv_vae_blend_f16(a0, a_strides.data(), a2, b_strides.data(), dims_i.data(), (int)axis, (int)extent, stream), "vae_blend_f16");
}

void op_copy4d_16b(const OptT& src, at::IntArrayRef src_strides, const OptT& dst, at::IntArrayRef dst_strides, at::IntArrayRef dims) {
    Dev dev("copy4d_16b");
    TORCH_CHECK(src_strides.size() == 4, "hv::copy4d_16b: src_strides must have 4 elements, got ", src_strides.size());
    TORCH_CHECK(dst_strides.size() == 4, "hv::copy4d_16b: dst_strides must have 4 elements, got ", dst_strides.size());
    TORCH_CHECK(dims.size() == 4, "hv::copy4d_16b: dims must have 4 elements, got ", dims.size());
    std::vector<int> dims_i(dims.begin(), dims.end());
    auto a0 = (const void*)dev.p(src, "src");
    auto a2 = (void*)dev.p(dst, "dst");
    TORCH_CHECK(dev.idx >= 0, "hv::copy4d_16b: needs at least one GPU tensor");
    c10::hip::HIPGuard guard(dev.idx);
    hipStream_t stream = c10::hip::getCurrentHIPStream(dev.idx).stream();
    check_rc(hv_copy4d_16b(a0, src_strides.data(), a2, dst_strides.data(), dims_i.data(), stream), "copy4d_16b");
}

void op_vae_postprocess_f16_f32(const OptT& x, const OptT& out, int64_t n) {
    Dev dev("vae_postprocess_f16_f32");
    auto a0 = (const void*)dev.p(x, "x");
    auto a1 = (float*)dev.p(out, "out");
    TORCH_CHECK(dev.idx >= 0, "hv::vae_postprocess_f16_f32: needs at least one GPU tensor");
    c10::hip::HIPGuard guard(dev.idx);
    hipStream_t stream = c10::hip::getCurrentHIPStream(dev.idx).stream();
    check_rc(hv_vae_postprocess_f16_f32(a0, a1, (int64_t)n, stream), "vae_postprocess_f16_f32");
}

void op_video_metrics(const OptT& a, int64_t a_sc, int64_t a_st, int64_t a_sh, const OptT& b, int64_t b_sc, int64_t b_st, int64_t b_sh, int64_t dtype, int64_t C, int64_t T, int64_t H, int64_t W, int64_t rescale, int64_t passes, const OptT& sse, const OptT& minmax, const OptT& ssim_sum, const OptT& workspace, int64_t workspace_bytes) {
    Dev dev("video_metrics");
    auto a0 = (const void*)dev.p(a, "a");
    auto a4 = (const void*)dev.p(b, "b");
    auto a15 = (void*)dev.p(sse, "sse");
    auto a16 = (void*)dev.p(minmax, "minmax");
    auto a17 = (void*)dev.p(ssim_sum, "ssim_sum");
    auto a18 = (void*)dev.p(workspace, "workspace");
    TORCH_CHECK(dev.idx >= 0, "hv::video_metrics: needs at least one GPU tensor");
    c10::hip::HIPGuard guard(dev.idx);
    hipStream_t stream = c10::hip::getCurrentHIPStream(dev.idx).stream();
    check_rc(hv_video_metrics(a0, (int64_t)a_sc, (int64_t)a_st, (int64_t)a_sh, a4, (int64_t)b_sc, (int64_t)b_st, (int64_t)b_sh, (int)dtype, (int)C, (int)T, (int)H, (int)W, (int)rescale, (int)passes, a15, a16, a17, a18, (int64_t)workspace_bytes, stream), "video_metrics");
}

int64_t op_video_metrics_workspace_bytes(int64_t C, int64_t T, int64_t H, int64_t W) {
    return (int64_t)hv_video_metrics_workspace_bytes((int)C, (int)T, (int)H, (int)W);
}

void op_lpips_conv1_f32(const OptT& a, int64_t a_sc, int64_t a_st, int64_t a_sh, const OptT& b, int64_t b_sc, int64_t b_st, int64_t b_sh, int64_t dtype, int64_t T, int64_t H, int64_t W, int64_t rescale, const OptT& lut, const OptT& w, const OptT& bias, const OptT& y) {
    Dev dev("lpips_conv1_f32");
    auto a0 = (const void*)dev.p(a, "a");
    auto a4 = (const void*)dev.p(b, "b");
    auto a13 = (const float*)dev.p(lut, "lut");
    auto a14 = (const float*)dev.p(w, "w");
    auto a15 = (const float*)dev.p(bias, "bias");
    auto a16 = (float*)dev.p(y, "y");
    TORCH_CHECK(dev.idx >= 0, "hv::lpips_conv1_f32: needs at least one GPU tensor");
    c10::hip::HIPGuard guard(dev.idx);
    hipStream_t stream = c10::hip::getCurrentHIPStream(dev.idx).stream();
    check_rc(hv_lpips_conv1_f32(a0, (int64_t)a_sc, (int64_t)a_st, (int64_t)a_sh, a4, (int64_t)b_sc, (int64_t)b_st, (int64_t)b_sh, (int)dtype, (int)T, (int)H, (int)W, (int)rescale, a13, a14, a15, a16, stream), "lpips_conv1_f32");
}

void op_lpips_conv2d_f32(const OptT& x, const OptT& w, const OptT& bias, const OptT& y, int64_t N, int64_t H, int64_t W, int64_t Cin, int64_t Cout, int64_t ksize, int64_t pad) {
    Dev dev("lpips_conv2d_f32");
    auto a0 = (const float*)dev.p(x, "x");
    auto a1 = (const float*)dev.p(w, "w");
    auto a2 = (const float*)dev.p(bias, "bias");
    auto a3 = (float*)dev.p(y, "y");
    TORCH_CHECK(dev.idx >= 0, "hv::lpips_conv2d_f32: needs at least one GPU tensor");
    c10::hip::HIPGuard guard(dev.idx);
    hipStream_t stream = c10::hip::getCurrentHIPStream(dev.idx).stream();
    check_rc(hv_lpips_conv2d_f32(a0, a1, a2, a3, (int)N, (int)H, (int)W, (int)Cin, (int)Cout, (int)ksize, (int)pad, stream), "lpips_conv2d_f32");
}

void op_lpips_maxpool_f32(const OptT& x, const OptT& y, int64_t N, int64_t H, int64_t W, int64_t C) {
    Dev dev("lpips_maxpool_f32");
    auto a0 = (const float*)dev.p(x, "x");
    auto a1 = (float*)dev.p(y, "y");
    TORCH_CHECK(dev.idx >= 0, "hv::lpips_maxpool_f32: needs at least one GPU tensor");
    c10::hip::HIPGuard guard(dev.idx);
    hipStream_t stream = c10::hip::getCurrentHIPStream(dev.idx).stream();
    check_rc(hv_lpips_maxpool_f32(a0, a1, (int)N, (int)H, (int)W, (int)C, stream), "lpips_maxpool_f32");
}

void op_lpips_distance_f32(const OptT& f, const OptT& lin, int64_t T, int64_t P, int64_t C, int64_t layer, const OptT& out, const OptT& workspace, int64_t workspace_bytes) {
    Dev dev("lpips_distance_f32");
    auto a0 = (const float*)dev.p(f, "f");
    auto a1 = (const float*)dev.p(lin, "lin");
    auto a6 = (double*)dev.p(out, "out");
    auto a7 = (void*)dev.p(workspace, "workspace");
    TORCH_CHECK(dev.idx >= 0, "hv::lpips_distance_f32: needs at least one GPU tensor");
    c10::hip::HIPGuard guard(dev.idx);
    hipStream_t stream = c10::hip::getCurrentHIPStream(dev.idx).stream();
    check_rc(hv_lpips_distance_f32(a0, a1, (int)T, (int64_t)P, (int)C, (int)layer, a6, a7, (int64_t)workspace_bytes, stream), "lpips_distance_f32");
}

int64_t op_lpips_distance_workspace_bytes(int64_t T, int64_t P) {
    return (int64_t)hv_lpips_distance_workspace_bytes((int)T, (int64_t)P);
}

}

TORCH_LIBRARY(hv, m) {
    m.def("abi_version() -> int");
    m.def("ln_modulate_bf16(Tensor? x, Tensor? shift_or_bias, Tensor? scale_or_weight, Tensor(a!)? out, int M, int D, int ldx, int ldo, float eps, int mode) -> ()");
    m.def("qknorm_rope_bf16(Tensor(a!)? qkv, Tensor? q_weight, Tensor? k_weight, Tensor? cos_tab, Tensor? sin_tab, int n_rows, int n_rope, int n_heads, int head_dim, int ld, int k_offset, float eps) -> ()");
    m.def("qknorm_rope_scatter_bf16(Tensor? qkv, Tensor? q_weight, Tensor? k_weight, Tensor? cos_tab, Tensor? sin_tab, int n_rows, int n_rope, int n_heads, int head_dim, int ld, int k_offset, float eps, Tensor(a!)? dst, int dst_ld, int heads_per_block, int dst_block_stride) -> ()");
    m.def("gemm_bf16(Tensor? A, int lda, Tensor? W, int ldw, Tensor? bias, int M, int N, int K, Tensor(a!)? out0, int ld0, int act0, int n_split, Tensor(b!)? out1, int ld1, int act1, Tensor? gate, Tensor? res, int ld_res) -> ()");
    m.def("linear_smallm_bf16(Tensor? x, Tensor? W, Tensor? bias, Tensor? addend, Tensor(a!)? out, int M, int N, int K, int ldx, int ldo, int act) -> ()");
    m.def("timestep_embedding_bf16(Tensor? t, Tensor(a!)? out, int n_t, int dim, float max_period) -> ()");
    m.def("attn_fwd_bf16(Tensor? q, Tensor? k, Tensor? v, Tensor(a!)? o, int stride_q, int stride_k, int stride_v, int stride_o, int n_q, int n_kv, int n_heads, int head_dim, float scale, Tensor(b!)? workspace, int workspace_bytes) -> ()");
    m.def("attn_workspace_bytes(int n_q, int n_kv, int n_heads) -> int");
    m.def("attn_w4_loop_signature() -> int");
    m.def("attn_partial_bf16(Tensor? q, Tensor? k, Tensor? v, int stride_q, int stride_k, int stride_v, int n_q, int n_kv, int n_heads, int head_dim, float scale, Tensor(a!)? part_o, Tensor(b!)? part_ml, int n_slots, int slot, int splits) -> ()");
    m.def("attn_merge_bf16(Tensor? part_o, Tensor? part_ml, Tensor(a!)? o, int stride_o, int n_q, int n_heads, int n_slots) -> ()");
    m.def("attn_suggest_splits(int n_q, int n_kv, int n_heads) -> int");
    m.def("patchify_f32_bf16(Tensor? x, Tensor(a!)? A, int C, int T, int H, int W) -> ()");
    m.def("unpatchify_bf16(Tensor? y, Tensor(a!)? out, int C, int T, int H, int W, int ldy) -> ()");
    m.def("euler_step_f32(Tensor(a!)? sample, Tensor? model_out_bf16, float dt, int n) -> ()");
    m.def("euler_step_f32_f32(Tensor(a!)? sample, Tensor? model_out_f32, float dt, int n) -> ()");
    m.def("masked_mean_bf16(Tensor? x, Tensor? mask, Tensor(a!)? out, int L, int D) -> ()");
    m.def("broadcast_row_bf16(Tensor? src, Tensor(a!)? dst, int n_rows, int D, int ld) -> ()");
    m.def("copy3d_bf16(Tensor? src, Tensor(a!)? dst, int n_batch, int rows, int cols, int src_batch_stride, int src_ld, int dst_batch_stride, int dst_ld) -> ()");
    m.def("fp8_dequant_bf16(Tensor? w_e4m3fn, Tensor? scale_bf16, Tensor(a!)? out_bf16, int n) -> ()");
    m.def("ln_modulate_fp8(Tensor? x, Tensor? shift, Tensor? scale, Tensor(a!)? out_q, Tensor(b!)? out_row_scale, int M, int D, int ldx, int ldq, float eps) -> ()");
    m.def("quant_rows_fp8(Tensor? x, int ldx, Tensor(a!)? out_q, int ldq, Tensor(b!)? out_row_scale, int M, int K) -> ()");
    m.def("gemm_fp8(Tensor? A_q, int lda, Tensor? a_row_scale, Tensor? W_q, int ldw, Tensor? w_scale_bf16, Tensor? bias, int M, int N, int K, Tensor(a!)? out0, int ld0, int act0, int n_split, Tensor(b!)? out1, int ld1, int act1, Tensor? gate, Tensor? res, int ld_res) -> ()");
    m.def("gemm_f16(Tensor? A, int lda, Tensor? W, int ldw, Tensor? bias, int M, int N, int K, Tensor(a!)? out, int ldo, int out_is_f32, Tensor? res, int ld_res) -> ()");
    m.def("conv3d_causal_f16(Tensor? x, int ldx, Tensor? w_taps, Tensor? bias, Tensor(a!)? out, int ldo, int T, int H, int W, int Cin, int Cout, int up_t, int up_hw, Tensor? res, int ld_res, Tensor(b!)? gn_partial, int gn_partial_floats) -> ()");
    m.def("gn_partial_rows(int M) -> int");
    m.def("subpixel_gn_partial_rows(int sT, int sH, int sW, int up_t) -> int");
    m.def("conv3d_upsampled_subpixel_f16(Tensor? x, int ldx, Tensor? w_sub, Tensor? tap_table, int ntap, Tensor? bias, Tensor(a!)? out, int ldo, int sT, int sH, int sW, int Cin, int Cout, int up_t, Tensor(b!)? gn_partial, int gn_partial_floats) -> ()");
    m.def("conv3d_cout4_f16(Tensor? x, int ldx, Tensor? affine, int silu, Tensor? w_frag, Tensor? bias, Tensor(a!)? out, int ldo, int T, int H, int W, int Cin, int Cout, Tensor(b!)? planes, int planes_floats) -> ()");
    m.def("conv3d_cout4_planes_floats(int M) -> int");
    m.def("conv3d_causal_strided_f16(Tensor? x, int ldx, Tensor? w_taps, Tensor? bias, Tensor(a!)? out, int ldo, int sT, int sH, int sW, int Cin, int Cout, int stride_t, int stride_h, int stride_w) -> ()");
    m.def("temporal_resample_f16(Tensor? x, int ldx, Tensor(a!)? out, int ldo, int T_in, int HW, int C, int mode, int k, int s) -> ()");
    m.def("groupnorm_affine_f16(Tensor? x, int ldx, int M, int C, int groups, float eps, Tensor? weight, Tensor? bias, Tensor(a!)? partial_ws, int partial_ws_floats, Tensor(b!)? affine_out) -> ()");
    m.def("groupnorm_finalize_f16(Tensor? partial, int partial_floats, int nrow, int M, int C, int groups, float eps, Tensor? weight, Tensor? bias, Tensor(a!)? affine_out) -> ()");
    m.def("groupnorm_apply_f16(Tensor? x, int ldx, Tensor(a!)? y, int ldy, int M, int C, Tensor? affine, int silu) -> ()");
    m.def("softmax_rows_f32_f16(Tensor? S, int ld_s, Tensor(a!)? P, int ld_p, int rows, int cols, int cols_pad, float scale, int causal_block) -> ()");
    m.def("transpose_16b(Tensor? src, int ld_src, Tensor(a!)? dst, int ld_dst, int R, int C) -> ()");
    m.def("vae_latent_tile_f16(Tensor? z, int sc, int st, int sh, int sw, int C, int T, int H, int W, int Cpad, Tensor(a!)? out) -> ()");
    m.def("vae_blend_f16(Tensor? a, int[] a_strides, Tensor(a!)? b, int[] b_strides, int[] dims, int axis, int extent) -> ()");
    m.def("copy4d_16b(Tensor? src, int[] src_strides, Tensor(a!)? dst, int[] dst_strides, int[] dims) -> ()");
    m.def("vae_postprocess_f16_f32(Tensor? x, Tensor(a!)? out, int n) -> ()");
    m.def("video_metrics(Tensor? a, int a_sc, int a_st, int a_sh, Tensor? b, int b_sc, int b_st, int b_sh, int dtype, int C, int T, int H, int W, int rescale, int passes, Tensor(a!)? sse, Tensor(b!)? minmax, Tensor(c!)? ssim_sum, Tensor(d!)? workspace, int workspace_bytes) -> ()");
    m.def("video_metrics_workspace_bytes(int C, int T, int H, int W) -> int");
    m.def("lpips_conv1_f32(Tensor? a, int a_sc, int a_st, int a_sh, Tensor? b, int b_sc, int b_st, int b_sh, int dtype, int T, int H, int W, int rescale, Tensor? lut, Tensor? w, Tensor? bias, Tensor(a!)? y) -> ()");
    m.def("lpips_conv2d_f32(Tensor? x, Tensor? w, Tensor? bias, Tensor(a!)? y, int N, int H, int W, int Cin, int Cout, int ksize, int pad) -> ()");
    m.def("lpips_maxpool_f32(Tensor? x, Tensor(a!)? y, int N, int H, int W, int C) -> ()");
    m.def("lpips_distance_f32(Tensor? f, Tensor? lin, int T, int P, int C, int layer, Tensor(a!)? out, Tensor(b!)? workspace, int workspace_bytes) -> ()");
    m.def("lpips_distance_workspace_bytes(int T, int P) -> int");
}

TORCH_LIBRARY_IMPL(hv, CUDA, m) {
    m.impl("ln_modulate_bf16", &op_ln_modulate_bf16);
    m.impl("qknorm_rope_bf16", &op_qknorm_rope_bf16);
    m.impl("qknorm_rope_scatter_bf16", &op_qknorm_rope_scatter_bf16);
    m.impl("gemm_bf16", &op_gemm_bf16);
    m.impl("linear_smallm_bf16", &op_linear_smallm_bf16);
    m.impl("timestep_embedding_bf16", &op_timestep_embedding_bf16);
    m.impl("attn_fwd_bf16", &op_attn_fwd_bf16);
    m.impl("attn_partial_bf16", &op_attn_partial_bf16);
    m.impl("attn_merge_bf16", &op_attn_merge_bf16);
    m.impl("patchify_f32_bf16", &op_patchify_f32_bf16);
    m.impl("unpatchify_bf16", &op_unpatchify_bf16);
    m.impl("euler_step_f32", &op_euler_step_f32);
    m.impl("euler_step_f32_f32", &op_euler_step_f32_f32);
    m.impl("masked_mean_bf16", &op_masked_mean_bf16);
    m.impl("broadcast_row_bf16", &op_broadcast_row_bf16);
    m.impl("copy3d_bf16", &op_copy3d_bf16);
    m.impl("fp8_dequant_bf16", &op_fp8_dequant_bf16);
    m.impl("ln_modulate_fp8", &op_ln_modulate_fp8);
    m.impl("quant_rows_fp8", &op_quant_rows_fp8);
    m.impl("gemm_fp8", &op_gemm_fp8);
    m.impl("gemm_f16", &op_gemm_f16);
    m.impl("conv3d_causal_f16", &op_conv3d_causal_f16);
    m.impl("conv3d_upsampled_subpixel_f16", &op_conv3d_upsampled_subpixel_f16);
    m.impl("conv3d_cout4_f16", &op_conv3d_cout4_f16);
    m.impl("conv3d_causal_strided_f16", &op_conv3d_causal_strided_f16);
    m.impl("temporal_resample_f16", &op_temporal_resample_f16);
    m.impl("groupnorm_affine_f16", &op_groupnorm_affine_f16);
    m.impl("groupnorm_finalize_f16", &op_groupnorm_finalize_f16);
    m.impl("groupnorm_apply_f16", &op_groupnorm_apply_f16);
    m.impl("softmax_rows_f32_f16", &op_softmax_rows_f32_f16);
    m.impl("transpose_16b", &op_transpose_16b);
    m.impl("vae_latent_tile_f16", &op_vae_latent_tile_f16);
    m.impl("vae_blend_f16", &op_vae_blend_f16);
    m.impl("copy4d_16b", &op_copy4d_16b);
    m.impl("vae_postprocess_f16_f32", &op_vae_postprocess_f16_f32);
    m.impl("video_metrics", &op_video_metrics);
    m.impl("lpips_conv1_f32", &op_lpips_conv1_f32);
    m.impl("lpips_conv2d_f32", &op_lpips_conv2d_f32);
    m.impl("lpips_maxpool_f32", &op_lpips_maxpool_f32);
    m.impl("lpips_distance_f32", &op_lpips_distance_f32);
}

TORCH_LIBRARY_IMPL(hv, CompositeExplicitAutograd, m) {
    m.impl("abi_version", &op_abi_version);
    m.impl("attn_workspace_bytes", &op_attn_workspace_bytes);
    m.impl("attn_w4_loop_signature", &op_attn_w4_loop_signature);
    m.impl("attn_suggest_splits", &op_attn_suggest_splits);
    m.impl("gn_partial_rows", &op_gn_partial_rows);
    m.impl("subpixel_gn_partial_rows", &op_subpixel_gn_partial_rows);
    m.impl("conv3d_cout4_planes_floats", &op_conv3d_cout4_planes_floats);
    m.impl("video_metrics_workspace_bytes", &op_video_metrics_workspace_bytes);
    m.impl("lpips_distance_workspace_bytes", &op_lpips_distance_workspace_bytes);
}
```

hunyuanvideo_efficiency_amd/modules/attenion.py:

```python
from __future__ import annotations

from typing import Optional

import torch

from .. import ops

BF16 = torch.bfloat16
def n_valid_text(text_mask: torch.Tensor) -> int:
    hit = getattr(text_mask, "_hv_n_valid", None)
    if hit is not None and hit[0] == text_mask._version:
        return hit[1]
    m = text_mask[0].to("cpu").to(torch.int64)
    n = int(m.sum())
    if not bool((m[:n] != 0).all()):
        raise NotImplementedError("text_mask must be a prefix mask (valid tokens first)")
    try:
        text_mask._hv_n_valid = (text_mask._version, n)
    except (AttributeError, RuntimeError):
        pass
    return n


def get_cu_seqlens(text_mask: torch.Tensor, img_len: int) -> torch.Tensor:
    batch_size = text_mask.shape[0]
    text_len = text_mask.sum(dim=1).to("cpu")
    max_len = text_mask.shape[1] + img_len
    cu = [0]
    for i in range(batch_size):
        cu.append(i * max_len + int(text_len[i]) + img_len)
        cu.append((i + 1) * max_len)
    return torch.tensor(cu, dtype=torch.int32, device=text_mask.device)


def _flat2d(t: torch.Tensor) -> torch.Tensor:
    if t.dim() == 4:
        assert t.shape[0] == 1
        t = t[0]
    s, h, d = t.shape
    assert t.stride(2) == 1 and t.stride(1) == d, "heads must be packed inside a token row"
    return t.as_strided((s, h * d), (t.stride(0), 1), t.storage_offset())


def attention(q, k, v, mode="flash", drop_rate=0, attn_mask=None, causal=False, cu_seqlens_q=None, cu_seqlens_kv=None,
              max_seqlen_q=None, max_seqlen_kv=None, batch_size=1):
    if drop_rate != 0 or causal:
        raise NotImplementedError("inference path: dropout 0, non-causal")
    if attn_mask is not None:
        raise NotImplementedError("attn_mask: use cu_seqlens segments (the DiT path never passes a mask here)")
    b, s, a, d = q.shape
    if b != 1:
        raise NotImplementedError("batch size 1")
    out = torch.empty(b, s, a * d, dtype=BF16, device=q.device)
    q2, k2, v2 = _flat2d(q), _flat2d(k), _flat2d(v)
    if mode == "flash":
        bounds = [int(x) for x in cu_seqlens_q.tolist()]
        assert list(cu_seqlens_kv.tolist()) == bounds, "self-attention: q and kv segments coincide"
    elif mode in ("torch", "vanilla"):
        bounds = [0, s]
    else:
        raise NotImplementedError(f"Unsupported attention mode: {mode}")
    for lo, hi in zip(bounds[:-1], bounds[1:]):
        if hi > lo:
            ops.attn_fwd(q2[lo:hi], k2[lo:hi], v2[lo:hi], out[0, lo:hi], a)
    return out


def segment_attention_(hybrid_seq_parallel_attn, qkv: torch.Tensor, cat: torch.Tensor, s_img: int, cu1: int, heads: int, d: int):
    s = qkv.shape[0]
    q, k, v, o = qkv[:, :d], qkv[:, d:2 * d], qkv[:, 2 * d:], cat[:, :d]
    if hybrid_seq_parallel_attn is None:
        if cu1 > 0:
            ops.attn_fwd(q[:cu1], k[:cu1], v[:cu1], o[:cu1], heads)
    else:
        hybrid_seq_parallel_attn.run_fused(qkv, cat, s_img, cu1, heads, d)
    if s > cu1:
        ops.attn_fwd(q[cu1:], k[cu1:], v[cu1:], o[cu1:], heads)


def pad_segment_attention_(qkv: torch.Tensor, cat: torch.Tensor, cu1: int, heads: int, d: int):
    if qkv.shape[0] > cu1:
        ops.attn_fwd(qkv[cu1:, :d], qkv[cu1:, d:2 * d], qkv[cu1:, 2 * d:], cat[cu1:, :d], heads)


def parallel_attention(hybrid_seq_parallel_attn, q, k, v, img_q_len, img_kv_len, cu_seqlens_q, cu_seqlens_kv):
    cu1 = int(cu_seqlens_q[1])
    attn1 = hybrid_seq_parallel_attn(
        None, q[:, :img_q_len], k[:, :img_kv_len], v[:, :img_kv_len], dropout_p=0.0, causal=False,
        joint_tensor_query=q[:, img_q_len:cu1], joint_tensor_key=k[:, img_kv_len:cu1],
        joint_tensor_value=v[:, img_kv_len:cu1], joint_strategy="rear")
    b, s, a, d = q.shape
    out = torch.empty(b, s, a * d, dtype=BF16, device=q.device)
    out[:, :cu1] = attn1.reshape(b, cu1, a * d)
    if s > cu1:
        ops.attn_fwd(_flat2d(q)[cu1:], _flat2d(k)[cu1:], _flat2d(v)[cu1:], out[0, cu1:], a)
    return out
```

hunyuanvideo_efficiency_amd/modules/models.py:

```python
from __future__ import annotations

from typing import Any, Dict, List, Optional, Tuple, Union

import torch
import torch.nn as nn

from .. import ops
from .attenion import get_cu_seqlens, n_valid_text, segment_attention_, pad_segment_attention_
from .token_refiner import SingleTokenRefiner
from .layers import ParamLinear, ParamNormWeight, ModulateDiT, MLP, MLPEmbedder, TimestepEmbedder, PatchEmbed, FinalLayer

BF16 = torch.bfloat16


class _Workspace:

    def __init__(self, s_img: int, s_txt: int, d: int, mlp: int, device):
        s = s_img + s_txt
        self.key = (s_img, s_txt, d, mlp, str(device))
        self.x = torch.empty(s, d, dtype=BF16, device=device)
        self.xmod = torch.empty(s, d, dtype=BF16, device=device)
        self.qkv = torch.empty(s, 3 * d, dtype=BF16, device=device)
        self.cat = torch.empty(s, d + mlp, dtype=BF16, device=device)
        self.patches = None
        self.final = None
        self.xq = self.xs = self.catq = self.cats = None

    def fp8_buffers(self):
        if self.xq is None:
            s, d = self.x.shape
            dev = self.x.device
            self.xq = torch.empty(s, d, dtype=torch.float8_e4m3fn, device=dev)
            self.xs = torch.empty(s, dtype=torch.float32, device=dev)
            self.catq = torch.empty(s, self.cat.shape[1], dtype=torch.float8_e4m3fn, device=dev)
            self.cats = torch.empty(s, dtype=torch.float32, device=dev)
        return self


def _use_fp8_mfma(block, *layers) -> bool:
    return bool(getattr(block, "fp8_mfma", False)) and all(
        l.weight.dtype == torch.float8_e4m3fn and l.in_features >= 384 and l.in_features % 128 == 0 for l in layers)


def _ln(ws: _Workspace, lo: int, hi: int, shift, scale, fp8: bool):
    if fp8:
        ws.fp8_buffers()
        ops.ln_modulate_fp8(ws.x[lo:hi], shift, scale, out_q=ws.xq[lo:hi], out_scale=ws.xs[lo:hi])
    else:
        ops.ln_modulate(ws.x[lo:hi], shift, scale, out=ws.xmod[lo:hi])


def _gemm(ws: _Workspace, layer, src: str, lo: int, hi: int, fp8: bool, wrows: Optional[slice] = None, **epi):
    d = ws.x.shape[1]
    cols = {"xmod": None, "attn": slice(0, d), "hid": slice(d, None), "cat": slice(None)}[src]
    b = layer.bias if wrows is None or layer.bias is None else layer.bias[wrows]
    if not fp8:
        a = ws.xmod[lo:hi] if src == "xmod" else ws.cat[lo:hi, cols]
        w = layer.w()
        return ops.gemm(a, w if wrows is None else w[wrows], b, **epi)
    ws.fp8_buffers()
    if src == "xmod":
        aq, asc = ws.xq[lo:hi], ws.xs[lo:hi]
    else:
        aq, asc = ops.quant_rows_fp8(ws.cat[lo:hi, cols], out_q=ws.catq[lo:hi, cols], out_scale=ws.cats[lo:hi])
    w8 = layer.weight if wrows is None else layer.weight[wrows]
    return ops.gemm_fp8(aq, asc, w8, layer.fp8_scale, b, **epi)


def _sp_chunked_qkv(sp, ws: _Workspace, layer, fp8, q_norm_w, k_norm_w, cos, sin, s_img: int, cu1: int, n_rope: int, H: int, d: int):
    ld = ws.qkv.stride(0)
    sp.begin(s_img, cu1 - s_img, H, ws.qkv.device)
    for c, which, norm_w in ((0, "q", q_norm_w), (1, "k", k_norm_w), (2, "v", None)):
        dst = sp.chunk_dst(which) if hasattr(sp, "chunk_dst") else None
        chunk = dst if dst is not None else ws.qkv[:s_img, c * d:(c + 1) * d]
        _gemm(ws, layer, "xmod", 0, s_img, fp8, wrows=slice(c * d, (c + 1) * d), out=chunk)
        joint = ws.qkv[s_img:cu1, c * d:(c + 1) * d]
        if norm_w is not None:
            packed = sp.pack_dst(which) if dst is None and hasattr(sp, "pack_dst") else None
            ops.qknorm_rope_(chunk, norm_w, norm_w, cos, sin, n_rope, H // 2, (H // 2) * 128, out=packed)
            if packed is not None:
                sp.send_packed(which, joint, ld)
                continue
        sp.send(which, chunk, chunk.stride(0), joint, ld)


class MMDoubleStreamBlock(nn.Module):

    def __init__(self, hidden_size: int, heads_num: int, mlp_width_ratio: float, mlp_act_type: str = "gelu_tanh",
                 qk_norm: bool = True, qk_norm_type: str = "rms", qkv_bias: bool = False,
                 dtype: Optional[torch.dtype] = None, device: Optional[torch.device] = None):
        super().__init__()
        if mlp_act_type != "gelu_tanh" or not qk_norm or qk_norm_type != "rms":
            raise NotImplementedError("only gelu_tanh MLP and RMS qk-norm have kernels (the shipped configuration)")
        fk = {"device": device, "dtype": dtype}
        self.deterministic = False
        self.heads_num = heads_num
        head_dim = hidden_size // heads_num
        mlp_hidden = int(hidden_size * mlp_width_ratio)
        for s in ("img", "txt"):
            setattr(self, f"{s}_mod", ModulateDiT(hidden_size, 6, **fk))
            setattr(self, f"{s}_attn_qkv", ParamLinear(hidden_size, hidden_size * 3, qkv_bias, **fk))
            setattr(self, f"{s}_attn_q_norm", ParamNormWeight(head_dim, **fk))
            setattr(self, f"{s}_attn_k_norm", ParamNormWeight(head_dim, **fk))
            setattr(self, f"{s}_attn_proj", ParamLinear(hidden_size, hidden_size, qkv_bias, **fk))
            setattr(self, f"{s}_mlp", MLP(hidden_size, mlp_hidden, **fk))
        self.hybrid_seq_parallel_attn = None

    def enable_deterministic(self):
        self.deterministic = True

    def disable_deterministic(self):
        self.deterministic = False

    def run(self, ws: _Workspace, s_img: int, s_txt: int, vec: torch.Tensor, cu1: int,
            cos: Optional[torch.Tensor], sin: Optional[torch.Tensor]):
        d = ws.x.shape[1]
        H = self.heads_num
        streams = (("txt", s_img, s_img + s_txt, 0), ("img", 0, s_img, s_img if cos is not None else 0))
        sp = self.hybrid_seq_parallel_attn
        overlap = sp is not None and hasattr(sp, "send") and H % 2 == 0
        mods = {}
        fp8 = {s: _use_fp8_mfma(self, getattr(self, f"{s}_attn_qkv"), getattr(self, f"{s}_attn_proj"), getattr(self, f"{s}_mlp").fc1,
                                getattr(self, f"{s}_mlp").fc2) for s in ("img", "txt")}
        for s, lo, hi, n_rope in streams:
            mod = getattr(self, f"{s}_mod")
            m = ops.linear_smallm(vec, mod.linear.w(), mod.linear.bias, silu_in=True)
            mods[s] = [m[0, i * d:(i + 1) * d] for i in range(6)]
            sh1, sc1 = mods[s][0], mods[s][1]
            _ln(ws, lo, hi, sh1, sc1, fp8[s])
            qkv_l = getattr(self, f"{s}_attn_qkv")
            qw, kw = getattr(self, f"{s}_attn_q_norm").weight, getattr(self, f"{s}_attn_k_norm").weight
            if overlap and s == "img":
                _sp_chunked_qkv(sp, ws, qkv_l, fp8[s], qw, kw, cos, sin, s_img, cu1, n_rope, H, d)
            else:
                _gemm(ws, qkv_l, "xmod", lo, hi, fp8[s], out=ws.qkv[lo:hi])
                ops.qknorm_rope_(ws.qkv[lo:hi], qw, kw, cos, sin, n_rope, H, d)
        segs = None
        if overlap:
            segs = sp.attend_async(ws.cat, ws.cat.stride(0))
            pad_segment_attention_(ws.qkv, ws.cat, cu1, H, d)
        else:
            segment_attention_(sp, ws.qkv, ws.cat, s_img, cu1, H, d)
        streams = (streams[1], streams[0])
        for s, lo, hi, _ in streams:
            _, _, g1, sh2, sc2, g2 = mods[s]
            proj, mlp = getattr(self, f"{s}_attn_proj"), getattr(self, f"{s}_mlp")
            x = ws.x[lo:hi]
            if s == "img" and segs is not None:
                for r0, r1, finish in segs:
                    finish()
                    r1 = min(r1, hi)
                    _gemm(ws, proj, "attn", r0, r1, fp8[s], out=ws.x[r0:r1], gate=g1, res=ws.x[r0:r1])
            else:
                _gemm(ws, proj, "attn", lo, hi, fp8[s], out=x, gate=g1, res=x)
            _ln(ws, lo, hi, sh2, sc2, fp8[s])
            _gemm(ws, mlp.fc1, "xmod", lo, hi, fp8[s], out=ws.cat[lo:hi, d:], act=ops.ACT_GELU_TANH)
            _gemm(ws, mlp.fc2, "hid", lo, hi, fp8[s], out=x, gate=g2, res=x)

    def forward(self, img, txt, vec, cu_seqlens_q=None, cu_seqlens_kv=None, max_seqlen_q=None, max_seqlen_kv=None,
                freqs_cis: tuple = None) -> Tuple[torch.Tensor, torch.Tensor]:
        assert img.shape[0] == 1, "batch 1 (cfg-distilled model, SURVEY.md top)"
        s_img, s_txt, d = img.shape[1], txt.shape[1], img.shape[2]
        ws = _Workspace(s_img, s_txt, d, self.img_mlp.fc1.weight.shape[0], img.device)
        ws.x[:s_img].copy_(img[0])
        ws.x[s_img:].copy_(txt[0])
        cu1 = int(cu_seqlens_q[1])
        cos, sin = freqs_cis if freqs_cis is not None else (None, None)
        self.run(ws, s_img, s_txt, vec.to(BF16).contiguous(), cu1, cos, sin)
        return ws.x[None, :s_img], ws.x[None, s_img:]


class MMSingleStreamBlock(nn.Module):

    def __init__(self, hidden_size: int, heads_num: int, mlp_width_ratio: float = 4.0, mlp_act_type: str = "gelu_tanh",
                 qk_norm: bool = True, qk_norm_type: str = "rms", qk_scale: float = None,
                 dtype: Optional[torch.dtype] = None, device: Optional[torch.device] = None):
        super().__init__()
        if mlp_act_type != "gelu_tanh" or not qk_norm or qk_norm_type != "rms" or qk_scale is not None:
            raise NotImplementedError("only gelu_tanh MLP, RMS qk-norm and the default scale have kernels")
        fk = {"device": device, "dtype": dtype}
        self.deterministic = False
        self.hidden_size = hidden_size
        self.heads_num = heads_num
        head_dim = hidden_size // heads_num
        self.mlp_hidden_dim = int(hidden_size * mlp_width_ratio)
        self.scale = head_dim ** -0.5
        self.linear1 = ParamLinear(hidden_size, hidden_size * 3 + self.mlp_hidden_dim, True, **fk)
        self.linear2 = ParamLinear(hidden_size + self.mlp_hidden_dim, hidden_size, True, **fk)
        self.q_norm = ParamNormWeight(head_dim, **fk)
        self.k_norm = ParamNormWeight(head_dim, **fk)
        self.modulation = ModulateDiT(hidden_size, 3, **fk)
        self.hybrid_seq_parallel_attn = None

    def enable_deterministic(self):
        self.deterministic = True

    def disable_deterministic(self):
        self.deterministic = False

    def run(self, ws: _Workspace, s_img: int, s_txt: int, vec: torch.Tensor, cu1: int,
            cos: Optional[torch.Tensor], sin: Optional[torch.Tensor]):
        d, H = self.hidden_size, self.heads_num
        m = ops.linear_smallm(vec, self.modulation.linear.w(), self.modulation.linear.bias, silu_in=True)
        shift, scale, gate = m[0, :d], m[0, d:2 * d], m[0, 2 * d:]
        fp8 = _use_fp8_mfma(self, self.linear1, self.linear2)
        s_all = ws.x.shape[0]
        _ln(ws, 0, s_all, shift, scale, fp8)
        sp = self.hybrid_seq_parallel_attn
        n_rope = s_img if cos is not None else 0
        if sp is not None and hasattr(sp, "send") and H % 2 == 0:
            _gemm(ws, self.linear1, "xmod", s_img, s_all, fp8, wrows=slice(0, 3 * d), out=ws.qkv[s_img:])
            ops.qknorm_rope_(ws.qkv[s_img:], self.q_norm.weight, self.k_norm.weight, None, None, 0, H, d)
            _sp_chunked_qkv(sp, ws, self.linear1, fp8, self.q_norm.weight, self.k_norm.weight, cos, sin, s_img, cu1, n_rope, H, d)
            _gemm(ws, self.linear1, "xmod", 0, s_all, fp8, wrows=slice(3 * d, None), out=ws.cat[:, d:], act=ops.ACT_GELU_TANH)
            segs = sp.attend_async(ws.cat, ws.cat.stride(0))
            pad_segment_attention_(ws.qkv, ws.cat, cu1, H, d)
            for i, (r0, r1, finish) in enumerate(segs):
                finish()
                r1 = s_all if i == len(segs) - 1 else r1
                _gemm(ws, self.linear2, "cat", r0, r1, fp8, out=ws.x[r0:r1], gate=gate, res=ws.x[r0:r1])
            return
        else:
            _gemm(ws, self.linear1, "xmod", 0, s_all, fp8, out=ws.qkv, n_split=3 * d, out1=ws.cat[:, d:], act1=ops.ACT_GELU_TANH)
            ops.qknorm_rope_(ws.qkv, self.q_norm.weight, self.k_norm.weight, cos, sin, n_rope, H, d)
            segment_attention_(sp, ws.qkv, ws.cat, s_img, cu1, H, d)
        _gemm(ws, self.linear2, "cat", 0, s_all, fp8, out=ws.x, gate=gate, res=ws.x)

    def forward(self, x, vec, txt_len, cu_seqlens_q=None, cu_seqlens_kv=None, max_seqlen_q=None, max_seqlen_kv=None,
                freqs_cis: Tuple[torch.Tensor, torch.Tensor] = None) -> torch.Tensor:
        assert x.shape[0] == 1
        s, d = x.shape[1], x.shape[2]
        ws = _Workspace(s - txt_len, txt_len, d, self.mlp_hidden_dim, x.device)
        ws.x.copy_(x[0])
        cos, sin = freqs_cis if freqs_cis is not None else (None, None)
        self.run(ws, s - txt_len, txt_len, vec.to(BF16).contiguous(), int(cu_seqlens_q[1]), cos, sin)
        return ws.x[None]


class _Config(dict):
    __getattr__ = dict.__getitem__


class HYVideoDiffusionTransformer(nn.Module):

    def __init__(self, args: Any, patch_size: list = [1, 2, 2], in_channels: int = 4, out_channels: int = None,
                 hidden_size: int = 3072, heads_num: int = 24, mlp_width_ratio: float = 4.0, mlp_act_type: str = "gelu_tanh",
                 mm_double_blocks_depth: int = 20, mm_single_blocks_depth: int = 40, rope_dim_list: List[int] = [16, 56, 56],
                 qkv_bias: bool = True, qk_norm: bool = True, qk_norm_type: str = "rms", guidance_embed: bool = False,
                 text_projection: str = "single_refiner", use_attention_mask: bool = True,
                 dtype: Optional[torch.dtype] = None, device: Optional[torch.device] = None):
        super().__init__()
        fk = {"device": device, "dtype": dtype}
        self.config = _Config(patch_size=patch_size, in_channels=in_channels, out_channels=out_channels,
                              hidden_size=hidden_size, heads_num=heads_num, mlp_width_ratio=mlp_width_ratio,
                              mlp_act_type=mlp_act_type, mm_double_blocks_depth=mm_double_blocks_depth,
                              mm_single_blocks_depth=mm_single_blocks_depth, rope_dim_list=rope_dim_list,
                              qkv_bias=qkv_bias, qk_norm=qk_norm, qk_norm_type=qk_norm_type,
                              guidance_embed=guidance_embed, text_projection=text_projection,
                              use_attention_mask=use_attention_mask)
        self.patch_size = patch_size
        self.in_channels = in_channels
        self.out_channels = in_channels if out_channels is None else out_channels
        self.unpatchify_channels = self.out_channels
        self.guidance_embed = guidance_embed
        self.rope_dim_list = rope_dim_list
        self.use_attention_mask = use_attention_mask
        self.text_projection = text_projection
        self.text_states_dim = args.text_states_dim
        self.text_states_dim_2 = args.text_states_dim_2
        if hidden_size % heads_num != 0:
            raise ValueError(f"Hidden size {hidden_size} must be divisible by heads_num {heads_num}")
        pe_dim = hidden_size // heads_num
        if sum(rope_dim_list) != pe_dim:
            raise ValueError(f"Got {rope_dim_list} but expected positional dim {pe_dim}")
        if pe_dim != 128:
            raise NotImplementedError("kernels are built for head_dim 128 (HunyuanVideo: 3072/24)")
        if list(patch_size) != [1, 2, 2]:
            raise NotImplementedError("kernels are built for patch_size [1,2,2]")
        if text_projection != "single_refiner":
            raise NotImplementedError(f"Unsupported text_projection: {text_projection}")
        self.hidden_size = hidden_size
        self.heads_num = heads_num
        self.mlp_hidden = int(hidden_size * mlp_width_ratio)

        self.img_in = PatchEmbed(self.patch_size, self.in_channels, self.hidden_size, **fk)
        self.txt_in = SingleTokenRefiner(self.text_states_dim, hidden_size, heads_num, depth=2, **fk)
        self.time_in = TimestepEmbedder(self.hidden_size, **fk)
        self.vector_in = MLPEmbedder(self.text_states_dim_2, self.hidden_size, **fk)
        self.guidance_in = TimestepEmbedder(self.hidden_size, **fk) if guidance_embed else None
        self.double_blocks = nn.ModuleList([
            MMDoubleStreamBlock(self.hidden_size, self.heads_num, mlp_width_ratio=mlp_width_ratio, mlp_act_type=mlp_act_type,
                                qk_norm=qk_norm, qk_norm_type=qk_norm_type, qkv_bias=qkv_bias, **fk)
            for _ in range(mm_double_blocks_depth)])
        self.single_blocks = nn.ModuleList([
            MMSingleStreamBlock(self.hidden_size, self.heads_num, mlp_width_ratio=mlp_width_ratio, mlp_act_type=mlp_act_type,
                                qk_norm=qk_norm, qk_norm_type=qk_norm_type, **fk)
            for _ in range(mm_single_blocks_depth)])
        self.final_layer = FinalLayer(self.hidden_size, self.patch_size, self.out_channels, **fk)
        self._ws: Optional[_Workspace] = None

    @property
    def dtype(self):
        return self.img_in.proj.weight.dtype

    def enable_deterministic(self):
        for b in list(self.double_blocks) + list(self.single_blocks):
            b.enable_deterministic()

    def disable_deterministic(self):
        for b in list(self.double_blocks) + list(self.single_blocks):
            b.disable_deterministic()

    def _workspace(self, s_img: int, s_txt: int, device) -> _Workspace:
        key = (s_img, s_txt, self.hidden_size, self.mlp_hidden, str(device))
        if self._ws is None or self._ws.key != key:
            self._ws = None
            self._ws = _Workspace(s_img, s_txt, self.hidden_size, self.mlp_hidden, device)
        return self._ws

    def forward(self, x: torch.Tensor, t: torch.Tensor, text_states: torch.Tensor = None, text_mask: torch.Tensor = None,
                text_states_2: Optional[torch.Tensor] = None, freqs_cos: Optional[torch.Tensor] = None,
                freqs_sin: Optional[torch.Tensor] = None, guidance: torch.Tensor = None,
                return_dict: bool = True) -> Union[torch.Tensor, Dict[str, torch.Tensor]]:
        if self.dtype != BF16:
            raise TypeError(f"parameters must be bf16 (got {self.dtype}); build with dtype=torch.bfloat16 or call .to()")
        B = x.shape[0]
        if B == 1:
            out = self._forward_one(x, t, text_states, text_mask, text_states_2, freqs_cos, freqs_sin, guidance, 0)
        else:
            t = t.reshape(-1)
            if t.numel() == 1:
                t = t.expand(B)
            outs = []
            for b in range(B):
                g_b = None if guidance is None else guidance.reshape(-1)[b:b + 1] if guidance.numel() > 1 else guidance
                outs.append(self._forward_one(x[b:b + 1], t[b:b + 1], text_states, text_mask,
                                              None if text_states_2 is None else text_states_2[b:b + 1], freqs_cos, freqs_sin, g_b, b))
            out = torch.cat(outs, 0)
        if return_dict:
            return {"x": out}
        return out

    def _forward_one(self, x, t, text_states, text_mask, text_states_2, freqs_cos, freqs_sin, guidance, b: int) -> torch.Tensor:
        dev = x.device
        _, _, ot, oh, ow = x.shape
        tt, th, tw = ot // self.patch_size[0], oh // self.patch_size[1], ow // self.patch_size[2]
        s_img, s_txt, d = tt * th * tw, text_states.shape[1], self.hidden_size
        ws = self._workspace(s_img, s_txt, dev)

        t32 = t.reshape(-1).to(torch.float32)
        vec = self.time_in.run(t32)
        vec = self.vector_in.run(text_states_2.to(BF16).reshape(1, -1), addend=vec)
        if self.guidance_embed:
            if guidance is None:
                raise ValueError("Didn't get guidance strength for guidance distilled model.")
            vec = self.guidance_in.run(guidance.reshape(-1).to(torch.float32), addend=vec)

        self.img_in.run(x[0].to(torch.float32).contiguous(), ws, s_img)
        mask_all = text_mask if self.use_attention_mask else None
        tc_all = getattr(text_states, "_hv_txt_cache", None)
        key = (text_states._version, None if mask_all is None else mask_all._version, id(self.txt_in),
               tuple(p._version for p in self.txt_in.parameters()))
        if tc_all is None or tc_all.get("key") != key or tc_all.get("mask") is not mask_all:
            tc_all = {"key": key, "mask": mask_all, "rows": {}}
            try:
                text_states._hv_txt_cache = tc_all
            except (AttributeError, RuntimeError):
                pass
        tc = tc_all["rows"].get(b)
        if tc is None:
            tc = tc_all["rows"][b] = {"text_bf16": text_states[b].to(BF16).contiguous(),
                                      "mask": None if mask_all is None else (mask_all if mask_all.shape[0] == 1 else mask_all[b:b + 1]),
                                      "mask_cu": None if text_mask is None else (text_mask if text_mask.shape[0] == 1 else text_mask[b:b + 1])}
        mask = tc["mask"]
        self.txt_in.run(tc["text_bf16"], t32, mask, out=ws.x[s_img:], cache=tc)

        if text_mask is not None and tc.get("mask_cu_src") is not text_mask:
            tc["mask_cu"] = text_mask if text_mask.shape[0] == 1 else text_mask[b:b + 1]
            tc["mask_cu_src"] = text_mask
        cu1 = s_img + (n_valid_text(tc["mask_cu"]) if text_mask is not None else s_txt)
        cos = freqs_cos.to(device=dev, dtype=torch.float32).contiguous() if freqs_cos is not None else None
        sin = freqs_sin.to(device=dev, dtype=torch.float32).contiguous() if freqs_sin is not None else None

        for block in self.double_blocks:
            block.run(ws, s_img, s_txt, vec, cu1, cos, sin)
        for block in self.single_blocks:
            block.run(ws, s_img, s_txt, vec, cu1, cos, sin)

        img = self.final_layer.run(ws, s_img, vec)
        out = ops.unpatchify(img, self.unpatchify_channels, ot, oh, ow)
        return out[None]

    def params_count(self):
        counts = {
            "double": sum(sum(p.numel() for p in m.parameters())
                          for b in self.double_blocks
                          for m in (b.img_attn_qkv, b.img_attn_proj, b.img_mlp, b.txt_attn_qkv, b.txt_attn_proj, b.txt_mlp)),
            "single": sum(sum(p.numel() for p in m.parameters()) for b in self.single_blocks for m in (b.linear1, b.linear2)),
            "total": sum(p.numel() for p in self.parameters()),
        }
        counts["attn+mlp"] = counts["double"] + counts["single"]
        return counts


HUNYUAN_VIDEO_CONFIG = {
    "HYVideo-T/2": dict(mm_double_blocks_depth=20, mm_single_blocks_depth=40, rope_dim_list=[16, 56, 56],
                        hidden_size=3072, heads_num=24, mlp_width_ratio=4),
    "HYVideo-T/2-cfgdistill": dict(mm_double_blocks_depth=20, mm_single_blocks_depth=40, rope_dim_list=[16, 56, 56],
                                   hidden_size=3072, heads_num=24, mlp_width_ratio=4, guidance_embed=True),
}
```

hunyuanvideo_efficiency_amd/ops.py:

```python
from __future__ import annotations

from typing import Optional

import torch

from . import _lib

BF16 = torch.bfloat16
ACT_NONE, ACT_GELU_TANH, ACT_SILU = 0, 1, 2
PROFILE_ATTN = None


def _chk(t: torch.Tensor, dtype, name: str, last_contig: bool = True):
    if not t.is_cuda:
        raise _lib.HVKernelError(f"{name}: expected a GPU tensor (this package has no CPU path), got {t.device}")
    if t.dtype != dtype:
        raise TypeError(f"{name}: expected {dtype}, got {t.dtype}")
    if last_contig and t.dim() > 0 and t.stride(-1) != 1:
        raise ValueError(f"{name}: innermost dimension must be contiguous")


def _rows(t: torch.Tensor, name: str):
    if t.dim() == 1:
        return 1, t.shape[0], t.shape[0]
    d = t.shape[-1]
    n = t.numel() // d
    ld = t.stride(-2)
    exp = ld
    for i in range(t.dim() - 2, -1, -1):
        if t.shape[i] != 1 and t.stride(i) != exp:
            raise ValueError(f"{name}: rows are not uniformly strided {t.shape} {t.stride()}")
        exp *= t.shape[i]
    return n, d, ld


def _chk_mod_vectors(shift, scale, d: int):
    for t, n in ((shift, "shift"), (scale, "scale")):
        if t is not None:
            _chk(t, BF16, n)
            assert t.numel() == d and t.is_contiguous(), f"{n} must be a contiguous [{d}] vector (batch 1)"


def ln_modulate(x, shift=None, scale=None, out=None, eps: float = 1e-6, affine: bool = False):
    _chk(x, BF16, "x")
    m, d, ldx = _rows(x, "x")
    if out is None:
        out = torch.empty(x.shape, dtype=BF16, device=x.device)
    _chk(out, BF16, "out")
    mo, do, ldo = _rows(out, "out")
    assert (mo, do) == (m, d)
    _chk_mod_vectors(shift, scale, d)
    _lib.call("ln_modulate_bf16", x, shift, scale, out, m, d, ldx, ldo, eps,
                                               1 if affine else 0)
    return out


def qknorm_rope_(qkv, q_weight, k_weight, cos, sin, n_rope: int, n_heads: int, k_offset: int, eps: float = 1e-6, out=None):
    _chk(qkv, BF16, "qkv")
    n, _, ld = _rows(qkv, "qkv")
    _chk(q_weight, BF16, "q_weight"), _chk(k_weight, BF16, "k_weight")
    if n_rope > 0:
        _chk(cos, torch.float32, "cos"), _chk(sin, torch.float32, "sin")
        assert cos.is_contiguous() and sin.is_contiguous() and cos.shape[-1] == 128 and cos.shape[0] >= n_rope
    if out is not None:
        _chk(out, BF16, "out", False)
        assert out.dim() == 3 and out.shape[0] == n and out.stride(2) == 1 and out.shape[2] % 128 == 0
        assert out.shape[1] * out.shape[2] == 2 * n_heads * 128, (out.shape, n_heads)
        _lib.call("qknorm_rope_scatter_bf16", qkv, q_weight, k_weight, cos, sin, n, n_rope, n_heads, 128, ld, k_offset, eps,
                  out, out.stride(0), out.shape[2] // 128, out.stride(1))
        return out
    _lib.call("qknorm_rope_bf16", qkv, q_weight, k_weight, cos, sin, n,
                                               n_rope, n_heads, 128, ld, k_offset, eps)
    return qkv


def _gemm_epilogue(out_shape, device, m: int, n: int, n_split: int, out, out1, bias, gate, res):
    n0 = n_split if 0 < n_split < n else n
    if out is None:
        out = torch.empty(*out_shape, n0, dtype=BF16, device=device)
    _chk(out, BF16, "out")
    mo, no, ld0 = _rows(out, "out")
    assert mo == m and no >= n0
    ld1 = 0
    if n0 < n:
        _chk(out1, BF16, "out1")
        m1, n1, ld1 = _rows(out1, "out1")
        assert m1 == m and n1 >= n - n0
    for t, nm in ((bias, "bias"), (gate, "gate")):
        if t is not None:
            _chk(t, BF16, nm)
            assert t.numel() == n and t.is_contiguous()
    ld_res = 0
    if res is not None:
        _chk(res, BF16, "res")
        mr, nr, ld_res = _rows(res, "res")
        assert mr == m and nr == n
    return out, n0, ld0, ld1, ld_res


def gemm(a, w, bias=None, out=None, act: int = ACT_NONE, n_split: int = 0, out1=None, act1: int = ACT_NONE,
         gate=None, res=None):
    _chk(a, BF16, "a"), _chk(w, BF16, "w")
    m, k, lda = _rows(a, "a")
    n, kw, ldw = _rows(w, "w")
    assert k == kw, (a.shape, w.shape)
    out, n0, ld0, ld1, ld_res = _gemm_epilogue(a.shape[:-1], a.device, m, n, n_split, out, out1, bias, gate, res)
    _lib.call("gemm_bf16", a, lda, w, ldw, bias, m, n, k, out, ld0, act, n0,
                                        out1, ld1, act1, gate, res, ld_res)
    return out


def linear_smallm(x, w, bias=None, silu_in: bool = False, silu_out: bool = False, out=None, addend=None):
    _chk(x, BF16, "x"), _chk(w, BF16, "w")
    m, k, ldx = _rows(x, "x")
    n, kw, ldw = _rows(w, "w")
    assert k == kw and ldw == k and m <= 4
    if out is None:
        out = torch.empty(*x.shape[:-1], n, dtype=BF16, device=x.device)
    _, _, ldo = _rows(out, "out")
    if bias is not None:
        _chk(bias, BF16, "bias")
    if addend is not None:
        _chk(addend, BF16, "addend")
        assert addend.shape == out.shape and addend.stride() == out.stride()
    _lib.call("linear_smallm_bf16", x, w, bias, addend, out, m, n, k, ldx, ldo,
                                                 (1 if silu_in else 0) | (2 if silu_out else 0))
    return out


_attn_ws = {}


ATTN_MIN_WORKSPACE = 256


def _attn_workspace(n_q, n_kv, n_heads, device):
    if n_kv < 64 * 64:
        return None
    n_wg = ((n_q + 255) // 256) * n_heads
    need = ATTN_MIN_WORKSPACE if n_wg >= 16 * 256 else int(_lib.host("attn_workspace_bytes", n_q, n_kv, n_heads))
    key = str(device)
    ws = _attn_ws.get(key)
    if ws is None or ws.numel() < need:
        ws = torch.empty(need, dtype=torch.uint8, device=device)
        _attn_ws[key] = ws
    return ws


def attn_fwd(q, k, v, out, n_heads: int, scale: Optional[float] = None, kv_split_workspace: bool = True):
    for t, nm in ((q, "q"), (k, "k"), (v, "v"), (out, "out")):
        _chk(t, BF16, nm)
        assert t.dim() == 2
    n_q, n_kv = q.shape[0], k.shape[0]
    assert v.shape[0] == n_kv and out.shape[0] == n_q
    if scale is None:
        scale = 128 ** -0.5
    prof = PROFILE_ATTN
    if prof is not None:
        e0, e1 = torch.cuda.Event(enable_timing=True), torch.cuda.Event(enable_timing=True)
        e0.record()
    ws = _attn_workspace(n_q, n_kv, n_heads, q.device) if kv_split_workspace else None
    _lib.call("attn_fwd_bf16", q, k, v, out, q.stride(0), k.stride(0), v.stride(0),
                                            out.stride(0), n_q, n_kv, n_heads, 128, scale, ws,
                                            0 if ws is None else ws.numel())
    if prof is not None:
        e1.record()
        prof.append((e0, e1, n_q, n_kv, n_heads))
    return out


class AttnPartials:

    def __init__(self, n_slots: int, n_q: int, n_heads: int, device):
        self.n_slots, self.n_q, self.n_heads = n_slots, n_q, n_heads
        self.o = torch.empty(n_slots, n_q, n_heads, 128, dtype=torch.float32, device=device)
        self.ml = torch.empty(n_slots, n_q, n_heads, 2, dtype=torch.float32, device=device)
        self.used = 0


def attn_suggest_splits(n_q: int, n_kv: int, n_heads: int) -> int:
    return int(_lib.host("attn_suggest_splits", n_q, n_kv, n_heads))


def attn_partial(q, k, v, parts: AttnPartials, n_heads: int, splits: int = 1, scale: Optional[float] = None):
    for t, nm in ((q, "q"), (k, "k"), (v, "v")):
        _chk(t, BF16, nm)
        assert t.dim() == 2
    n_q, n_kv = q.shape[0], k.shape[0]
    assert v.shape[0] == n_kv and n_q == parts.n_q and n_heads == parts.n_heads and parts.used + splits <= parts.n_slots
    if scale is None:
        scale = 128 ** -0.5
    prof = PROFILE_ATTN
    if prof is not None:
        e0, e1 = torch.cuda.Event(enable_timing=True), torch.cuda.Event(enable_timing=True)
        e0.record()
    _lib.call("attn_partial_bf16", q, k, v, q.stride(0), k.stride(0), v.stride(0), n_q, n_kv, n_heads,
                                                128, scale, parts.o, parts.ml, parts.n_slots, parts.used, splits)
    if prof is not None:
        e1.record()
        prof.append((e0, e1, n_q, n_kv, n_heads))
    parts.used += splits


def attn_merge(parts: AttnPartials, out):
    _chk(out, BF16, "out")
    assert out.dim() == 2 and out.shape[0] == parts.n_q and parts.used >= 1
    _lib.call("attn_merge_bf16", parts.o, parts.ml, out, out.stride(0), parts.n_q, parts.n_heads,
                                              parts.used)
    return out


def patchify(x_f32, out=None):
    _chk(x_f32, torch.float32, "x")
    assert x_f32.is_contiguous() and x_f32.dim() == 4
    c, t, h, w = x_f32.shape
    if out is None:
        out = torch.empty(t * (h // 2) * (w // 2), c * 4, dtype=BF16, device=x_f32.device)
    _lib.call("patchify_f32_bf16", x_f32, out, c, t, h, w)
    return out


def unpatchify(y, c: int, t: int, h: int, w: int, out=None):
    _chk(y, BF16, "y")
    assert y.dim() == 2
    if out is None:
        out = torch.empty(c, t, h, w, dtype=BF16, device=y.device)
    _lib.call("unpatchify_bf16", y, out, c, t, h, w, y.stride(0))
    return out


def euler_step_(sample_f32, model_out_bf16, dt: float):
    _chk(sample_f32, torch.float32, "sample"), _chk(model_out_bf16, BF16, "model_out")
    assert sample_f32.is_contiguous() and model_out_bf16.is_contiguous() and sample_f32.numel() == model_out_bf16.numel()
    _lib.call("euler_step_f32", sample_f32, model_out_bf16, float(dt), sample_f32.numel())
    return sample_f32


def euler_step_f32_(sample_f32, model_out_f32, dt: float):
    _chk(sample_f32, torch.float32, "sample"), _chk(model_out_f32, torch.float32, "model_out")
    assert sample_f32.is_contiguous() and model_out_f32.is_contiguous() and sample_f32.numel() == model_out_f32.numel()
    _lib.call("euler_step_f32_f32", sample_f32, model_out_f32, float(dt), sample_f32.numel())
    return sample_f32


def masked_mean(x, mask_i32=None):
    _chk(x, BF16, "x")
    assert x.dim() == 2 and x.is_contiguous()
    out = torch.empty(x.shape[1], dtype=BF16, device=x.device)
    if mask_i32 is not None:
        _chk(mask_i32, torch.int32, "mask")
    _lib.call("masked_mean_bf16", x, mask_i32, out, x.shape[0], x.shape[1])
    return out


def broadcast_row_(src, dst):
    _chk(src, BF16, "src"), _chk(dst, BF16, "dst")
    assert dst.dim() == 2 and src.numel() == dst.shape[1]
    _lib.call("broadcast_row_bf16", src, dst, dst.shape[0], dst.shape[1], dst.stride(0))
    return dst


def timestep_embedding(t_f32, dim: int = 256, max_period: float = 10000.0):
    _chk(t_f32, torch.float32, "t")
    t_f32 = t_f32.reshape(-1).contiguous()
    out = torch.empty(t_f32.numel(), dim, dtype=BF16, device=t_f32.device)
    _lib.call("timestep_embedding_bf16", t_f32, out, t_f32.numel(), dim, max_period)
    return out


def fp8_dequant(w8, scale_bf16, out_bf16):
    if not w8.is_cuda or w8.dtype != torch.float8_e4m3fn:
        raise _lib.HVKernelError("fp8_dequant: expected a float8_e4m3fn GPU tensor")
    _chk(scale_bf16, BF16, "scale"), _chk(out_bf16, BF16, "out")
    assert w8.is_contiguous() and out_bf16.is_contiguous() and out_bf16.numel() == w8.numel()
    _lib.call("fp8_dequant_bf16", w8, scale_bf16, out_bf16, w8.numel())
    return out_bf16


FP8 = torch.float8_e4m3fn


def ln_modulate_fp8(x, shift=None, scale=None, out_q=None, out_scale=None, eps: float = 1e-6):
    _chk(x, BF16, "x")
    m, d, ldx = _rows(x, "x")
    if out_q is None:
        out_q = torch.empty(m, d, dtype=FP8, device=x.device)
    if out_scale is None:
        out_scale = torch.empty(m, dtype=torch.float32, device=x.device)
    assert out_q.dtype == FP8 and out_q.is_cuda and out_q.shape[-1] == d and out_q.stride(-1) == 1 and out_scale.numel() >= m
    _chk_mod_vectors(shift, scale, d)
    _lib.call("ln_modulate_fp8", x, shift, scale, out_q, out_scale, m, d, ldx, out_q.stride(-2) if out_q.dim() > 1 else d, eps)
    return out_q, out_scale


def quant_rows_fp8(x, out_q=None, out_scale=None):
    _chk(x, BF16, "x")
    m, k, ldx = _rows(x, "x")
    if out_q is None:
        out_q = torch.empty(m, k, dtype=FP8, device=x.device)
    if out_scale is None:
        out_scale = torch.empty(m, dtype=torch.float32, device=x.device)
    assert out_q.dtype == FP8 and out_q.is_cuda and out_q.shape[-1] == k and out_q.stride(-1) == 1 and out_scale.numel() >= m
    _lib.call("quant_rows_fp8", x, ldx, out_q, out_q.stride(-2) if out_q.dim() > 1 else k, out_scale, m, k)
    return out_q, out_scale


def gemm_fp8(a_q, a_scale, w_q, w_scale, bias=None, out=None, act: int = ACT_NONE, n_split: int = 0, out1=None,
             act1: int = ACT_NONE, gate=None, res=None):
    for t, nm in ((a_q, "a_q"), (w_q, "w_q")):
        if not t.is_cuda or t.dtype != FP8:
            raise _lib.HVKernelError(f"gemm_fp8: {nm} must be a float8_e4m3fn GPU tensor")
    _chk(a_scale, torch.float32, "a_scale"), _chk(w_scale, BF16, "w_scale")
    m, k, lda = _rows(a_q, "a_q")
    n, kw, ldw = _rows(w_q, "w_q")
    assert k == kw and a_scale.numel() >= m and w_scale.numel() == 1
    out, n0, ld0, ld1, ld_res = _gemm_epilogue((m,), a_q.device, m, n, n_split, out, out1, bias, gate, res)
    _lib.call("gemm_fp8", a_q, lda, a_scale, w_q, ldw, w_scale, bias, m, n, k, out, ld0, act, n0, out1, ld1, act1, gate, res, ld_res)
# ... 8 lines not shown
```

include/hv_kernels.h:

```cpp
#ifndef HV_KERNELS_H
#define HV_KERNELS_H

#include <stdint.h>

#ifdef __cplusplus
extern "C" {
#endif

#ifndef __HIP__
typedef struct ihipStream_t* hipStream_t;
#endif

int hv_abi_version(void);

int hv_ln_modulate_bf16(const void* x, const void* shift_or_bias, const void* scale_or_weight, void* out,
                        int64_t M, int D, int64_t ldx, int64_t ldo, float eps, int mode, hipStream_t stream);

int hv_qknorm_rope_bf16(void* qkv, const void* q_weight, const void* k_weight, const float* cos_tab,
                        const float* sin_tab, int64_t n_rows, int64_t n_rope, int n_heads, int head_dim,
                        int64_t ld, int64_t k_offset, float eps, hipStream_t stream);

int hv_qknorm_rope_scatter_bf16(const void* qkv, const void* q_weight, const void* k_weight, const float* cos_tab,
                                const float* sin_tab, int64_t n_rows, int64_t n_rope, int n_heads, int head_dim, int64_t ld,
                                int64_t k_offset, float eps, void* dst, int64_t dst_ld, int heads_per_block,
                                int64_t dst_block_stride, hipStream_t stream);

int hv_gemm_bf16(const void* A, int64_t lda, const void* W, int64_t ldw, const void* bias, int M, int N, int K,
                 void* out0, int64_t ld0, int act0, int n_split, void* out1, int64_t ld1, int act1,
                 const void* gate, const void* res, int64_t ld_res, hipStream_t stream);

int hv_linear_smallm_bf16(const void* x, const void* W, const void* bias, const void* addend, void* out, int M,
                          int N, int K, int64_t ldx, int64_t ldo, int act, hipStream_t stream);

int hv_timestep_embedding_bf16(const float* t, void* out, int n_t, int dim, float max_period, hipStream_t stream);

#define HV_ATTN_MIN_WORKSPACE_BYTES 256
int hv_attn_fwd_bf16(const void* q, const void* k, const void* v, void* o, int64_t stride_q, int64_t stride_k,
                     int64_t stride_v, int64_t stride_o, int n_q, int n_kv, int n_heads, int head_dim,
                     float scale, void* workspace, int64_t workspace_bytes, hipStream_t stream);

int64_t hv_attn_workspace_bytes(int n_q, int n_kv, int n_heads);
int hv_attn_w4_loop_signature(void);

int hv_attn_partial_bf16(const void* q, const void* k, const void* v, int64_t stride_q, int64_t stride_k, int64_t stride_v,
                         int n_q, int n_kv, int n_heads, int head_dim, float scale, void* part_o, void* part_ml,
                         int n_slots, int slot, int splits, hipStream_t stream);

int hv_attn_merge_bf16(const void* part_o, const void* part_ml, void* o, int64_t stride_o, int n_q, int n_heads, int n_slots,
                       hipStream_t stream);

int hv_attn_suggest_splits(int n_q, int n_kv, int n_heads);

int hv_patchify_f32_bf16(const float* x, void* A, int C, int T, int H, int W, hipStream_t stream);

int hv_unpatchify_bf16(const void* y, void* out, int C, int T, int H, int W, int64_t ldy, hipStream_t stream);

int hv_euler_step_f32(float* sample, const void* model_out_bf16, float dt, int64_t n, hipStream_t stream);

int hv_euler_step_f32_f32(float* sample, const float* model_out_f32, float dt, int64_t n, hipStream_t stream);

int hv_masked_mean_bf16(const void* x, const int* mask, void* out, int L, int D, hipStream_t stream);

int hv_broadcast_row_bf16(const void* src, void* dst, int64_t n_rows, int D, int64_t ld, hipStream_t stream);

int hv_copy3d_bf16(const void* src, void* dst, int n_batch, int64_t rows, int cols, int64_t src_batch_stride,
                   int64_t src_ld, int64_t dst_batch_stride, int64_t dst_ld, hipStream_t stream);

int hv_fp8_dequant_bf16(const void* w_e4m3fn, const void* scale_bf16, void* out_bf16, int64_t n, hipStream_t stream);


int hv_ln_modulate_fp8(const void* x, const void* shift, const void* scale, void* out_q, float* out_row_scale, int64_t M,
                       int D, int64_t ldx, int64_t ldq, float eps, hipStream_t stream);

int hv_quant_rows_fp8(const void* x, int64_t ldx, void* out_q, int64_t ldq, float* out_row_scale, int64_t M, int K,
                      hipStream_t stream);

int hv_gemm_fp8(const void* A_q, int64_t lda, const float* a_row_scale, const void* W_q, int64_t ldw, const void* w_scale_bf16,
                const void* bias, int M, int N, int K, void* out0, int64_t ld0, int act0, int n_split, void* out1, int64_t ld1,
                int act1, const void* gate, const void* res, int64_t ld_res, hipStream_t stream);


int hv_gemm_f16(const void* A, int64_t lda, const void* W, int64_t ldw, const void* bias, int M, int N, int K,
                void* out, int64_t ldo, int out_is_f32, const void* res, int64_t ld_res, hipStream_t stream);

int hv_conv3d_causal_f16(const void* x, int64_t ldx, const void* w_taps, const void* bias, void* out, int64_t ldo,
                         int T, int H, int W, int Cin, int Cout, int up_t, int up_hw, const void* res,
                         int64_t ld_res, float* gn_partial, int64_t gn_partial_floats, hipStream_t stream);

int64_t hv_gn_partial_rows(int64_t M);
int64_t hv_subpixel_gn_partial_rows(int sT, int sH, int sW, int up_t);

int hv_conv3d_upsampled_subpixel_f16(const void* x, int64_t ldx, const void* w_sub, const void* tap_table, int ntap,
                                     const void* bias, void* out, int64_t ldo, int sT, int sH, int sW, int Cin, int Cout,
                                     int up_t, float* gn_partial, int64_t gn_partial_floats, hipStream_t stream);

int hv_conv3d_cout4_f16(const void* x, int64_t ldx, const float* affine, int silu, const void* w_frag, const void* bias, void* out,
                        int64_t ldo, int T, int H, int W, int Cin, int Cout, float* planes, int64_t planes_floats, hipStream_t stream);
int64_t hv_conv3d_cout4_planes_floats(int64_t M);

int hv_conv3d_causal_strided_f16(const void* x, int64_t ldx, const void* w_taps, const void* bias, void* out, int64_t ldo,
                                 int sT, int sH, int sW, int Cin, int Cout, int stride_t, int stride_h, int stride_w,
                                 hipStream_t stream);

int hv_temporal_resample_f16(const void* x, int64_t ldx, void* out, int64_t ldo, int T_in, int64_t HW, int C, int mode,
                             int k, int s, hipStream_t stream);

int hv_groupnorm_affine_f16(const void* x, int64_t ldx, int64_t M, int C, int groups, float eps, const void* weight,
                            const void* bias, float* partial_ws, int64_t partial_ws_floats, float* affine_out,
                            hipStream_t stream);

#define HV_GN_FOLD_WS_FLOATS 16384
int hv_groupnorm_finalize_f16(const float* partial, int64_t partial_floats, int64_t nrow, int64_t M, int C, int groups, float eps,
                              const void* weight, const void* bias, float* affine_out, hipStream_t stream);

int hv_groupnorm_apply_f16(const void* x, int64_t ldx, void* y, int64_t ldy, int64_t M, int C, const float* affine,
                           int silu, hipStream_t stream);

int hv_softmax_rows_f32_f16(const float* S, int64_t ld_s, void* P, int64_t ld_p, int rows, int cols, int cols_pad,
                            float scale, int causal_block, hipStream_t stream);

int hv_transpose_16b(const void* src, int64_t ld_src, void* dst, int64_t ld_dst, int R, int C, hipStream_t stream);

int hv_vae_latent_tile_f16(const float* z, int64_t sc, int64_t st, int64_t sh, int64_t sw, int C, int T, int H, int W,
                           int Cpad, void* out, hipStream_t stream);

int hv_vae_blend_f16(const void* a, const int64_t* a_strides, void* b, const int64_t* b_strides, const int* dims,
                     int axis, int extent, hipStream_t stream);

int hv_copy4d_16b(const void* src, const int64_t* src_strides, void* dst, const int64_t* dst_strides, const int* dims,
                  hipStream_t stream);

int hv_vae_postprocess_f16_f32(const void* x, float* out, int64_t n, hipStream_t stream);

int hv_video_metrics(const void* a, int64_t a_sc, int64_t a_st, int64_t a_sh, const void* b, int64_t b_sc, int64_t b_st,
                     int64_t b_sh, int dtype, int C, int T, int H, int W, int rescale, int passes, void* sse, void* minmax,
                     void* ssim_sum, void* workspace, int64_t workspace_bytes, hipStream_t stream);
int64_t hv_video_metrics_workspace_bytes(int C, int T, int H, int W);

int hv_lpips_conv1_f32(const void* a, int64_t a_sc, int64_t a_st, int64_t a_sh, const void* b, int64_t b_sc, int64_t b_st,
                       int64_t b_sh, int dtype, int T, int H, int W, int rescale, const float* lut, const float* w,
                       const float* bias, float* y, hipStream_t stream);

int hv_lpips_conv2d_f32(const float* x, const float* w, const float* bias, float* y, int N, int H, int W, int Cin, int Cout,
                        int ksize, int pad, hipStream_t stream);

int hv_lpips_maxpool_f32(const float* x, float* y, int N, int H, int W, int C, hipStream_t stream);

int hv_lpips_distance_f32(const float* f, const float* lin, int T, int64_t P, int C, int layer, double* out, void* workspace,
                          int64_t workspace_bytes, hipStream_t stream);
int64_t hv_lpips_distance_workspace_bytes(int T, int64_t P);

#ifdef __cplusplus
}
#endif
#endif
```

Before: 0.1217.

## Fuse Q RMSNorm+RoPE into attention prologue and K-norm with key-max bound

After: 0.1217, median of 6. Within noise of the previous version (+0.0%).

```diff
diff --git a/hunyuanvideo_efficiency_amd/_lib.py b/hunyuanvideo_efficiency_amd/_lib.py
--- a/hunyuanvideo_efficiency_amd/_lib.py
+++ b/hunyuanvideo_efficiency_amd/_lib.py
@@ -7,7 +7,7 @@
 _HERE = os.path.dirname(os.path.abspath(__file__))
 LIB_PATH = os.path.join(_HERE, "lib", "libhv_kernels.so")
 TORCH_OPS_PATH = os.path.join(_HERE, "lib", "libhv_torch_ops.so")
-ABI_VERSION = 8
+ABI_VERSION = 9
 
 _p, _i, _l, _f = C.c_void_p, C.c_int, C.c_int64, C.c_float
 
@@ -16,10 +16,13 @@
     "hv_ln_modulate_bf16": [_p, _p, _p, _p, _l, _i, _l, _l, _f, _i, _p],
     "hv_qknorm_rope_bf16": [_p, _p, _p, _p, _p, _l, _l, _i, _i, _l, _l, _f, _p],
     "hv_qknorm_rope_scatter_bf16": [_p, _p, _p, _p, _p, _l, _l, _i, _i, _l, _l, _f, _p, _l, _i, _l, _p],
+    "hv_knorm_rope_kmax_bf16": [_p, _p, _p, _p, _l, _l, _l, _i, _i, _l, _l, _f, _p, _p],
+    "hv_knorm_rows_per_block": [],
     "hv_gemm_bf16": [_p, _l, _p, _l, _p, _i, _i, _i, _p, _l, _i, _i, _p, _l, _i, _p, _p, _l, _p],
     "hv_linear_smallm_bf16": [_p, _p, _p, _p, _p, _i, _i, _i, _l, _l, _i, _p],
     "hv_timestep_embedding_bf16": [_p, _p, _i, _i, _f, _p],
     "hv_attn_fwd_bf16": [_p, _p, _p, _p, _l, _l, _l, _l, _i, _i, _i, _i, _f, _p, _l, _p],
+    "hv_attn_fwd_qnorm_bf16": [_p, _p, _p, _p, _l, _l, _l, _l, _i, _i, _i, _i, _f, _p, _p, _p, _p, _i, _f, _p, _p, _l, _p],
     "hv_attn_workspace_bytes": [_i, _i, _i],
     "hv_attn_w4_loop_signature": [],
     "hv_attn_partial_bf16": [_p, _p, _p, _l, _l, _l, _i, _i, _i, _i, _f, _p, _p, _i, _i, _i, _p],
diff --git a/hunyuanvideo_efficiency_amd/csrc/hv_api.hip b/hunyuanvideo_efficiency_amd/csrc/hv_api.hip
--- a/hunyuanvideo_efficiency_amd/csrc/hv_api.hip
+++ b/hunyuanvideo_efficiency_amd/csrc/hv_api.hip
@@ -1,3 +1,3 @@
 #include "hv_common.hpp"
 #include "../../include/hv_kernels.h"
-extern "C" int hv_abi_version(void) { return 8; }
+extern "C" int hv_abi_version(void) { return 9; }
diff --git a/hunyuanvideo_efficiency_amd/csrc/hv_attention.hip b/hunyuanvideo_efficiency_amd/csrc/hv_attention.hip
--- a/hunyuanvideo_efficiency_amd/csrc/hv_attention.hip
+++ b/hunyuanvideo_efficiency_amd/csrc/hv_attention.hip
@@ -76,12 +76,17 @@
     return (int64_t)KMAX_BYTES + (int64_t)2 * n_q * n_heads * (128 + 2) * (int64_t)sizeof(float);
 }
 
-extern "C" int hv_attn_fwd_bf16(const void* q, const void* k, const void* v, void* o, int64_t stride_q, int64_t stride_k,
-                                int64_t stride_v, int64_t stride_o, int n_q, int n_kv, int n_heads, int head_dim,
-                                float scale, void* workspace, int64_t workspace_bytes, hipStream_t stream) {
+namespace {
+
+struct QNormArgs { const void* w_lo; const void* w_hi; const float* cos_tab; const float* sin_tab; int n_split; float eps; };
+
+int attn_fwd_impl(const void* q, const void* k, const void* v, void* o, int64_t stride_q, int64_t stride_k, int64_t stride_v,
+                  int64_t stride_o, int n_q, int n_kv, int n_heads, int head_dim, float scale, const QNormArgs* qn, void* bound,
+                  void* workspace, int64_t workspace_bytes, hipStream_t stream) {
     if (!q || !k || !v || !o || head_dim != D || n_heads <= 0 || n_q < 0 || n_kv < 0 || (stride_q & 7) || (stride_k & 7) ||
         (stride_v & 7) || (stride_o & 3))
         return HV_ERR_ARG;
+    if (qn && (!qn->w_lo || !qn->w_hi || qn->n_split < 0 || qn->n_split > n_q || (!qn->cos_tab) != (!qn->sin_tab))) return HV_ERR_ARG;
     if (n_q == 0) return HV_OK;
     if (n_kv == 0) return HV_ERR_ARG;
     AttnArgs a;
@@ -91,7 +96,13 @@
     a.n_qtiles = (n_q + QTILE - 1) / QTILE;
     a.scale_log2e = scale * 1.4426950408889634f;
     a.n_splits = 1; a.split_keys = n_kv; a.part_o = nullptr; a.part_ml = nullptr; a.partial = 0;
-    if (attn_prepare_kmax(a, workspace, workspace_bytes, stream) != HV_OK) return HV_ERR_LAUNCH;
+    if (qn) {
+        a.qw_lo = (const bf16_t*)qn->w_lo; a.qw_hi = (const bf16_t*)qn->w_hi;
+        a.q_cos = qn->cos_tab; a.q_sin = qn->sin_tab; a.q_split = qn->n_split; a.q_eps = qn->eps;
+        a.kmax2 = (bound && n_heads <= KMAX_HEADS && n_kv >= 64 * KVT) ? (const unsigned*)bound : nullptr;
+    } else if (attn_prepare_kmax(a, workspace, workspace_bytes, stream) != HV_OK) {
+        return HV_ERR_LAUNCH;
+    }
     {
         const int64_t nwg = (int64_t)a.n_qtiles * n_heads;
         const int ntile = (n_kv + KVT - 1) / KVT;
@@ -110,6 +121,25 @@
                                                                                            a.n_splits);
     }
     return hv_check_launch();
+}
+
+}
+
+extern "C" int hv_attn_fwd_bf16(const void* q, const void* k, const void* v, void* o, int64_t stride_q, int64_t stride_k,
+                                int64_t stride_v, int64_t stride_o, int n_q, int n_kv, int n_heads, int head_dim,
+                                float scale, void* workspace, int64_t workspace_bytes, hipStream_t stream) {
+    return attn_fwd_impl(q, k, v, o, stride_q, stride_k, stride_v, stride_o, n_q, n_kv, n_heads, head_dim, scale, nullptr, nullptr,
+                         workspace, workspace_bytes, stream);
+}
+
+extern "C" int hv_attn_fwd_qnorm_bf16(const void* q, const void* k, const void* v, void* o, int64_t stride_q, int64_t stride_k,
+                                      int64_t stride_v, int64_t stride_o, int n_q, int n_kv, int n_heads, int head_dim, float scale,
+                                      const void* q_weight_lo, const void* q_weight_hi, const float* cos_tab, const float* sin_tab,
+                                      int n_split, float eps, void* bound, void* workspace, int64_t workspace_bytes,
+                                      hipStream_t stream) {
+    const QNormArgs qn{q_weight_lo, q_weight_hi, cos_tab, sin_tab, n_split, eps};
+    return attn_fwd_impl(q, k, v, o, stride_q, stride_k, stride_v, stride_o, n_q, n_kv, n_heads, head_dim, scale, &qn, bound,
+                         workspace, workspace_bytes, stream);
 }
 
 extern "C" int hv_attn_partial_bf16(const void* q, const void* k, const void* v, int64_t stride_q, int64_t stride_k, int64_t stride_v,
diff --git a/hunyuanvideo_efficiency_amd/csrc/hv_attention.hpp b/hunyuanvideo_efficiency_amd/csrc/hv_attention.hpp
--- a/hunyuanvideo_efficiency_amd/csrc/hv_attention.hpp
+++ b/hunyuanvideo_efficiency_amd/csrc/hv_attention.hpp
@@ -19,6 +19,10 @@
     float* part_ml;
     int partial;
     const unsigned* kmax2;
+    const bf16_t* qw_lo = nullptr; const bf16_t* qw_hi = nullptr;
+    const float* q_cos = nullptr; const float* q_sin = nullptr;
+    int q_split = 0;
+    float q_eps = 0.f;
 };
 constexpr int KMAX_BYTES = 256;
 constexpr int KMAX_HEADS = 62;
diff --git a/hunyuanvideo_efficiency_amd/csrc/hv_attention_w4.hip b/hunyuanvideo_efficiency_amd/csrc/hv_attention_w4.hip
--- a/hunyuanvideo_efficiency_amd/csrc/hv_attention_w4.hip
+++ b/hunyuanvideo_efficiency_amd/csrc/hv_attention_w4.hip
@@ -101,6 +101,40 @@
         u32x4 raw[8];
 #pragma unroll
         for (int ks = 0; ks < 8; ++ks) raw[ks] = *reinterpret_cast<const u32x4*>(qp + ks * 16);
+        if (a.qw_lo) {
+            float cs[8];
+#pragma unroll
+            for (int ks = 0; ks < 8; ++ks) {
+                float x[8];
+                unpack8(raw[ks], x);
+                cs[ks] = qk_chunk_sumsq(x);
+            }
+            const float ss = half_swap_sum(((cs[0] + cs[4]) + (cs[2] + cs[6])) + ((cs[1] + cs[5]) + (cs[3] + cs[7])));
+            const float r = qk_rms_scale(ss, a.q_eps);
+            const bool lo = qrow < a.q_split;
+            const bool rope = lo && a.q_cos != nullptr;
+            const bf16_t* gw = (lo ? a.qw_lo : a.qw_hi) + lh * 8;
+            const float* cp = a.q_cos + (int64_t)qrow * D + lh * 8;
+            const float* sp = a.q_sin + (int64_t)qrow * D + lh * 8;
+#pragma unroll
+            for (int ks = 0; ks < 8; ++ks) {
+                float x[8], w[8], y[8];
+                unpack8(raw[ks], x);
+                unpack8(*reinterpret_cast<const u32x4*>(gw + ks * 16), w);
+                qk_chunk_norm(x, r, w, y);
+                if (rope) {
+                    const float4 c0 = *reinterpret_cast<const float4*>(cp + ks * 16), c1 = *reinterpret_cast<const float4*>(cp + ks * 16 + 4);
+                    const float4 s0 = *reinterpret_cast<const float4*>(sp + ks * 16), s1 = *reinterpret_cast<const float4*>(sp + ks * 16 + 4);
+                    const float c[8] = {c0.x, c0.y, c0.z, c0.w, c1.x, c1.y, c1.z, c1.w};
+                    const float s[8] = {s0.x, s0.y, s0.z, s0.w, s1.x, s1.y, s1.z, s1.w};
+                    float o[8];
+                    qk_chunk_rope(y, c, s, o);
+                    raw[ks] = pack8(o);
+                } else {
+                    raw[ks] = pack8(y);
+                }
+            }
+        }
         static_for<0, 32>([&](auto I) {
             constexpr int i = decltype(I)::value;
             const uint32_t w = raw[i >> 2][i & 3];
diff --git a/hunyuanvideo_efficiency_amd/csrc/hv_common.hpp b/hunyuanvideo_efficiency_amd/csrc/hv_common.hpp
--- a/hunyuanvideo_efficiency_amd/csrc/hv_common.hpp
+++ b/hunyuanvideo_efficiency_amd/csrc/hv_common.hpp
@@ -99,6 +99,42 @@
     return (uint32_t)(int)__fmul_rn(x, 255.0f);
 }
 
+__device__ __forceinline__ float qk_chunk_sumsq(const float (&x)[8]) {
+#pragma clang fp contract(off)
+    float ss = __builtin_fmaf(x[1], x[1], x[0] * x[0]);
+#pragma unroll
+    for (int j = 2; j < 8; ++j) {
+        const float sq = x[j] * x[j];
+        ss = ss + sq;
+    }
+    return ss;
+}
+__device__ __forceinline__ float qk_rms_scale(float ss, float eps) { return rsqrtf(__builtin_fmaf(ss, 1.0f / 128.0f, eps)); }
+__device__ __forceinline__ void qk_chunk_norm(const float (&x)[8], float r, const float (&w)[8], float (&y)[8]) {
+#pragma clang fp contract(off)
+#pragma unroll
+    for (int j = 0; j < 8; ++j) y[j] = rbf(rbf(x[j] * r) * w[j]);
+}
+__device__ __forceinline__ void qk_chunk_rope(const float (&y)[8], const float (&c)[8], const float (&s)[8], float (&o)[8]) {
+#pragma clang fp contract(off)
+#pragma unroll
+    for (int j = 0; j < 8; j += 2) {
+        const float x0 = y[j + 1] * s[j], x1 = y[j] * s[j + 1];
+        o[j] = __builtin_fmaf(y[j], c[j], -x0);
+        o[j + 1] = __builtin_fmaf(y[j + 1], c[j + 1], x1);
+    }
+}
+__device__ __forceinline__ float kmax_piece_sumsq(const u32x4& w) {
+#pragma clang fp contract(off)
+    float t[4];
+#pragma unroll
+    for (int j = 0; j < 4; ++j) {
+        const float hh = bf2f_hi(w[j]) * bf2f_hi(w[j]);
+        t[j] = __builtin_fmaf(bf2f_lo(w[j]), bf2f_lo(w[j]), hh);
+    }
+    return ((t[0] + t[1]) + t[2]) + t[3];
+}
+
 struct HvPerDeviceOnce { bool done[64] = {}; };
 static inline int hv_set_max_lds(HvPerDeviceOnce& once, const void* fn, int bytes) {
     int dev = 0;
diff --git a/hunyuanvideo_efficiency_amd/csrc/hv_rowwise.hip b/hunyuanvideo_efficiency_amd/csrc/hv_rowwise.hip
--- a/hunyuanvideo_efficiency_amd/csrc/hv_rowwise.hip
+++ b/hunyuanvideo_efficiency_amd/csrc/hv_rowwise.hip
@@ -289,6 +289,103 @@
     return hv_check_launch();
 }
 
+constexpr int KNORM_ROWS = 64, KNORM_U = 2;
+template <int N>
+__device__ __forceinline__ float row_ror_add(float v) {
+    return v + __int_as_float(__builtin_amdgcn_update_dpp(0, __float_as_int(v), 0x120 + N, 0xF, 0xF, false));
+}
+__device__ __forceinline__ float row16_sum(float v) { return row_ror_add<1>(row_ror_add<2>(row_ror_add<4>(row_ror_add<8>(v)))); }
+template <int NP>
+__global__ __launch_bounds__(256) void knorm_rope_kmax_kernel(bf16_t* __restrict__ kx, const bf16_t* __restrict__ kw,
+                                                               const float* __restrict__ cosT, const float* __restrict__ sinT,
+                                                               int64_t n_rows, int64_t n_rope, int64_t n_bound, int H, int64_t ld,
+                                                               float eps, unsigned* __restrict__ bound) {
+    const int sub = threadIdx.x & 15, grp = threadIdx.x >> 4;
+    float wk[8];
+    unpack8(*reinterpret_cast<const u32x4*>(kw + sub * 8), wk);
+    const int64_t r0 = (int64_t)blockIdx.x * KNORM_ROWS, r1 = r0 + KNORM_ROWS < n_rows ? r0 + KNORM_ROWS : n_rows;
+    float best[NP];
+#pragma unroll
+    for (int i = 0; i < NP; ++i) best[i] = 0.f;
+    for (int64_t rb = r0; rb < r1; rb += KNORM_U) {
+        u32x4 raw[KNORM_U][NP];
+        float4 tc[KNORM_U][2], ts[KNORM_U][2];
+#pragma unroll
+        for (int u = 0; u < KNORM_U; ++u) {
+            const int64_t row = rb + u;
+            if (row < r1) {
+#pragma unroll
+                for (int i = 0; i < NP; ++i)
+                    if (grp + 16 * i < H) raw[u][i] = *reinterpret_cast<const u32x4*>(kx + row * ld + (grp + 16 * i) * 128 + sub * 8);
+                if (row < n_rope) {
+                    const float4* cp = reinterpret_cast<const float4*>(cosT + row * 128 + sub * 8);
+                    const float4* sp = reinterpret_cast<const float4*>(sinT + row * 128 + sub * 8);
+                    tc[u][0] = cp[0], tc[u][1] = cp[1], ts[u][0] = sp[0], ts[u][1] = sp[1];
+                }
+            }
+        }
+#pragma unroll
+        for (int u = 0; u < KNORM_U; ++u) {
+            const int64_t row = rb + u;
+            if (row >= r1) break;
+            const bool rope = row < n_rope;
+#pragma unroll
+            for (int i = 0; i < NP; ++i) {
+                if (grp + 16 * i >= H) continue;
+                float x[8], y[8], o[8];
+                unpack8(raw[u][i], x);
+                const float ss = row16_sum(qk_chunk_sumsq(x));
+                qk_chunk_norm(x, qk_rms_scale(ss, eps), wk, y);
+                u32x4 w;
+                if (rope) {
+                    const float c[8] = {tc[u][0].x, tc[u][0].y, tc[u][0].z, tc[u][0].w, tc[u][1].x, tc[u][1].y, tc[u][1].z, tc[u][1].w};
+                    const float s[8] = {ts[u][0].x, ts[u][0].y, ts[u][0].z, ts[u][0].w, ts[u][1].x, ts[u][1].y, ts[u][1].z, ts[u][1].w};
+                    qk_chunk_rope(y, c, s, o);
+                    w = pack8(o);
+                } else {
+                    w = pack8(y);
+                }
+                *reinterpret_cast<u32x4*>(kx + row * ld + (grp + 16 * i) * 128 + sub * 8) = w;
+                const float k2 = row16_sum(kmax_piece_sumsq(w));
+                if (row < n_bound) best[i] = fmaxf(best[i], k2);
+            }
+        }
+    }
+    if (bound && sub == 0) {
+#pragma unroll
+        for (int i = 0; i < NP; ++i) {
+            const int h = grp + 16 * i;
+            const unsigned bits = __float_as_uint(best[i]);
+            if (h < H && bits > __atomic_load_n(bound + h, __ATOMIC_RELAXED)) atomicMax(bound + h, bits);
+        }
+    }
+}
+
+extern "C" int hv_knorm_rope_kmax_bf16(void* qkv, const void* k_weight, const float* cos_tab, const float* sin_tab, int64_t n_rows,
+                                       int64_t n_rope, int64_t n_bound, int n_heads, int head_dim, int64_t ld, int64_t k_offset,
+                                       float eps, void* bound, hipStream_t stream) {
+    if (!qkv || !k_weight || head_dim != 128 || n_heads <= 0 || n_heads > 64 || n_rows < 0 || n_rope < 0 || n_rope > n_rows ||
+        n_bound < 0 || n_bound > n_rows || (ld & 7) || (k_offset & 7) || (n_rope > 0 && (!cos_tab || !sin_tab)) ||
+        (n_bound > 0 && (!bound || n_heads > 62)))
+        return HV_ERR_ARG;
+    if (n_rows == 0) return HV_OK;
+    const dim3 grid((unsigned)((n_rows + KNORM_ROWS - 1) / KNORM_ROWS)), block(256);
+    bf16_t* kx = (bf16_t*)qkv + k_offset;
+    unsigned* bp = n_bound > 0 ? (unsigned*)bound : nullptr;
+    auto launch = [&](auto np) {
+        knorm_rope_kmax_kernel<decltype(np)::value><<<grid, block, 0, stream>>>(kx, (const bf16_t*)k_weight, cos_tab, sin_tab, n_rows,
+                                                                               n_rope, n_bound, n_heads, ld, eps, bp);
+    };
+    switch ((n_heads + 15) / 16) {
+        case 1: launch(std::integral_constant<int, 1>{}); break;
+        case 2: launch(std::integral_constant<int, 2>{}); break;
+        case 3: launch(std::integral_constant<int, 3>{}); break;
+        default: launch(std::integral_constant<int, 4>{}); break;
+    }
+    return hv_check_launch();
+}
+extern "C" int hv_knorm_rows_per_block(void) { return KNORM_ROWS; }
+
 template <int MM>
 __global__ __launch_bounds__(256) void gemv_kernel(const bf16_t* __restrict__ x, const bf16_t* __restrict__ W,
                                                     const bf16_t* __restrict__ b, const bf16_t* __restrict__ addend,
diff --git a/hunyuanvideo_efficiency_amd/csrc/hv_torch_ops.cpp b/hunyuanvideo_efficiency_amd/csrc/hv_torch_ops.cpp
--- a/hunyuanvideo_efficiency_amd/csrc/hv_torch_ops.cpp
+++ b/hunyuanvideo_efficiency_amd/csrc/hv_torch_ops.cpp
@@ -69,6 +69,23 @@
     check_rc(hv_qknorm_rope_scatter_bf16(a0, a1, a2, a3, a4, (int64_t)n_rows, (int64_t)n_rope, (int)n_heads, (int)head_dim, (int64_t)ld, (int64_t)k_offset, (float)eps, a12, (int64_t)dst_ld, (int)heads_per_block, (int64_t)dst_block_stride, stream), "qknorm_rope_scatter_bf16");
 }
 
+void op_knorm_rope_kmax_bf16(const OptT& qkv, const OptT& k_weight, const OptT& cos_tab, const OptT& sin_tab, int64_t n_rows, int64_t n_rope, int64_t n_bound, int64_t n_heads, int64_t head_dim, int64_t ld, int64_t k_offset, double eps, const OptT& bound) {
+    Dev dev("knorm_rope_kmax_bf16");
+    auto a0 = (void*)dev.p(qkv, "qkv");
+    auto a1 = (const void*)dev.p(k_weight, "k_weight");
+    auto a2 = (const float*)dev.p(cos_tab, "cos_tab");
+    auto a3 = (const float*)dev.p(sin_tab, "sin_tab");
+    auto a12 = (void*)dev.p(bound, "bound");
+    TORCH_CHECK(dev.idx >= 0, "hv::knorm_rope_kmax_bf16: needs at least one GPU tensor");
+    c10::hip::HIPGuard guard(dev.idx);
+    hipStream_t stream = c10::hip::getCurrentHIPStream(dev.idx).stream();
+    check_rc(hv_knorm_rope_kmax_bf16(a0, a1, a2, a3, (int64_t)n_rows, (int64_t)n_rope, (int64_t)n_bound, (int)n_heads, (int)head_dim, (int64_t)ld, (int64_t)k_offset, (float)eps, a12, stream), "knorm_rope_kmax_bf16");
+}
+
+int64_t op_knorm_rows_per_block() {
+    return (int64_t)hv_knorm_rows_per_block();
+}
+
 void op_gemm_bf16(const OptT& A, int64_t lda, const OptT& W, int64_t ldw, const OptT& bias, int64_t M, int64_t N, int64_t K, const OptT& out0, int64_t ld0, int64_t act0, int64_t n_split, const OptT& out1, int64_t ld1, int64_t act1, const OptT& gate, const OptT& res, int64_t ld_res) {
     Dev dev("gemm_bf16");
     auto a0 = (const void*)dev.p(A, "A");
@@ -118,6 +135,24 @@
     c10::hip::HIPGuard guard(dev.idx);
     hipStream_t stream = c10::hip::getCurrentHIPStream(dev.idx).stream();
     check_rc(hv_attn_fwd_bf16(a0, a1, a2, a3, (int64_t)stride_q, (int64_t)stride_k, (int64_t)stride_v, (int64_t)stride_o, (int)n_q, (int)n_kv, (int)n_heads, (int)head_dim, (float)scale, a13, (int64_t)workspace_bytes, stream), "attn_fwd_bf16");
+}
+
+void op_attn_fwd_qnorm_bf16(const OptT& q, const OptT& k, const OptT& v, const OptT& o, int64_t stride_q, int64_t stride_k, int64_t stride_v, int64_t stride_o, int64_t n_q, int64_t n_kv, int64_t n_heads, int64_t head_dim, double scale, const OptT& q_weight_lo, const OptT& q_weight_hi, const OptT& cos_tab, const OptT& sin_tab, int64_t n_split, double eps, const OptT& bound, const OptT& workspace, int64_t workspace_bytes) {
+    Dev dev("attn_fwd_qnorm_bf16");
+    auto a0 = (const void*)dev.p(q, "q");
+    auto a1 = (const void*)dev.p(k, "k");
+    auto a2 = (const void*)dev.p(v, "v");
+    auto a3 = (void*)dev.p(o, "o");
+    auto a13 = (const void*)dev.p(q_weight_lo, "q_weight_lo");
+    auto a14 = (const void*)dev.p(q_weight_hi, "q_weight_hi");
+    auto a15 = (const float*)dev.p(cos_tab, "cos_tab");
+    auto a16 = (const float*)dev.p(sin_tab, "sin_tab");
+    auto a19 = (void*)dev.p(bound, "bound");
+    auto a20 = (void*)dev.p(workspace, "workspace");
+    TORCH_CHECK(dev.idx >= 0, "hv::attn_fwd_qnorm_bf16: needs at least one GPU tensor");
+    c10::hip::HIPGuard guard(dev.idx);
+    hipStream_t stream = c10::hip::getCurrentHIPStream(dev.idx).stream();
+    check_rc(hv_attn_fwd_qnorm_bf16(a0, a1, a2, a3, (int64_t)stride_q, (int64_t)stride_k, (int64_t)stride_v, (int64_t)stride_o, (int)n_q, (int)n_kv, (int)n_heads, (int)head_dim, (float)scale, a13, a14, a15, a16, (int)n_split, (float)eps, a19, a20, (int64_t)workspace_bytes, stream), "attn_fwd_qnorm_bf16");
 }
 
 int64_t op_attn_workspace_bytes(int64_t n_q, int64_t n_kv, int64_t n_heads) {
@@ -549,10 +584,13 @@
     m.def("ln_modulate_bf16(Tensor? x, Tensor? shift_or_bias, Tensor? scale_or_weight, Tensor(a!)? out, int M, int D, int ldx, int ldo, float eps, int mode) -> ()");
     m.def("qknorm_rope_bf16(Tensor(a!)? qkv, Tensor? q_weight, Tensor? k_weight, Tensor? cos_tab, Tensor? sin_tab, int n_rows, int n_rope, int n_heads, int head_dim, int ld, int k_offset, float eps) -> ()");
     m.def("qknorm_rope_scatter_bf16(Tensor? qkv, Tensor? q_weight, Tensor? k_weight, Tensor? cos_tab, Tensor? sin_tab, int n_rows, int n_rope, int n_heads, int head_dim, int ld, int k_offset, float eps, Tensor(a!)? dst, int dst_ld, int heads_per_block, int dst_block_stride) -> ()");
+    m.def("knorm_rope_kmax_bf16(Tensor(a!)? qkv, Tensor? k_weight, Tensor? cos_tab, Tensor? sin_tab, int n_rows, int n_rope, int n_bound, int n_heads, int head_dim, int ld, int k_offset, float eps, Tensor(b!)? bound) -> ()");
+    m.def("knorm_rows_per_block() -> int");
     m.def("gemm_bf16(Tensor? A, int lda, Tensor? W, int ldw, Tensor? bias, int M, int N, int K, Tensor(a!)? out0, int ld0, int act0, int n_split, Tensor(b!)? out1, int ld1, int act1, Tensor? gate, Tensor? res, int ld_res) -> ()");
     m.def("linear_smallm_bf16(Tensor? x, Tensor? W, Tensor? bias, Tensor? addend, Tensor(a!)? out, int M, int N, int K, int ldx, int ldo, int act) -> ()");
     m.def("timestep_embedding_bf16(Tensor? t, Tensor(a!)? out, int n_t, int dim, float max_period) -> ()");
     m.def("attn_fwd_bf16(Tensor? q, Tensor? k, Tensor? v, Tensor(a!)? o, int stride_q, int stride_k, int stride_v, int stride_o, int n_q, int n_kv, int n_heads, int head_dim, float scale, Tensor(b!)? workspace, int workspace_bytes) -> ()");
+    m.def("attn_fwd_qnorm_bf16(Tensor? q, Tensor? k, Tensor? v, Tensor(a!)? o, int stride_q, int stride_k, int stride_v, int stride_o, int n_q, int n_kv, int n_heads, int head_dim, float scale, Tensor? q_weight_lo, Tensor? q_weight_hi, Tensor? cos_tab, Tensor? sin_tab, int n_split, float eps, Tensor(b!)? bound, Tensor(c!)? workspace, int workspace_bytes) -> ()");
     m.def("attn_workspace_bytes(int n_q, int n_kv, int n_heads) -> int");
     m.def("attn_w4_loop_signature() -> int");
     m.def("attn_partial_bf16(Tensor? q, Tensor? k, Tensor? v, int stride_q, int stride_k, int stride_v, int n_q, int n_kv, int n_heads, int head_dim, float scale, Tensor(a!)? part_o, Tensor(b!)? part_ml, int n_slots, int slot, int splits) -> ()");
@@ -600,10 +638,12 @@
     m.impl("ln_modulate_bf16", &op_ln_modulate_bf16);
     m.impl("qknorm_rope_bf16", &op_qknorm_rope_bf16);
     m.impl("qknorm_rope_scatter_bf16", &op_qknorm_rope_scatter_bf16);
+    m.impl("knorm_rope_kmax_bf16", &op_knorm_rope_kmax_bf16);
     m.impl("gemm_bf16", &op_gemm_bf16);
     m.impl("linear_smallm_bf16", &op_linear_smallm_bf16);
     m.impl("timestep_embedding_bf16", &op_timestep_embedding_bf16);
     m.impl("attn_fwd_bf16", &op_attn_fwd_bf16);
+    m.impl("attn_fwd_qnorm_bf16", &op_attn_fwd_qnorm_bf16);
     m.impl("attn_partial_bf16", &op_attn_partial_bf16);
     m.impl("attn_merge_bf16", &op_attn_merge_bf16);
     m.impl("patchify_f32_bf16", &op_patchify_f32_bf16);
@@ -641,6 +681,7 @@
 
 TORCH_LIBRARY_IMPL(hv, CompositeExplicitAutograd, m) {
     m.impl("abi_version", &op_abi_version);
+    m.impl("knorm_rows_per_block", &op_knorm_rows_per_block);
     m.impl("attn_workspace_bytes", &op_attn_workspace_bytes);
     m.impl("attn_w4_loop_signature", &op_attn_w4_loop_signature);
     m.impl("attn_suggest_splits", &op_attn_suggest_splits);
diff --git a/hunyuanvideo_efficiency_amd/modules/attenion.py b/hunyuanvideo_efficiency_amd/modules/attenion.py
--- a/hunyuanvideo_efficiency_amd/modules/attenion.py
+++ b/hunyuanvideo_efficiency_amd/modules/attenion.py
@@ -66,21 +66,31 @@
     return out
 
 
-def segment_attention_(hybrid_seq_parallel_attn, qkv: torch.Tensor, cat: torch.Tensor, s_img: int, cu1: int, heads: int, d: int):
+def segment_attention_(hybrid_seq_parallel_attn, qkv: torch.Tensor, cat: torch.Tensor, s_img: int, cu1: int, heads: int, d: int,
+                       qnorm=None):
     s = qkv.shape[0]
     q, k, v, o = qkv[:, :d], qkv[:, d:2 * d], qkv[:, 2 * d:], cat[:, :d]
     if hybrid_seq_parallel_attn is None:
         if cu1 > 0:
-            ops.attn_fwd(q[:cu1], k[:cu1], v[:cu1], o[:cu1], heads)
+            if qnorm is None:
+                ops.attn_fwd(q[:cu1], k[:cu1], v[:cu1], o[:cu1], heads)
+            else:
+                w_img, w_txt, cos, sin, n_split, eps, bound = qnorm
+                ops.attn_fwd(q[:cu1], k[:cu1], v[:cu1], o[:cu1], heads, qnorm=(w_img, w_txt, cos, sin, min(n_split, cu1), eps), bound=bound)
     else:
+        assert qnorm is None, "sequence parallelism takes q already normalised"
         hybrid_seq_parallel_attn.run_fused(qkv, cat, s_img, cu1, heads, d)
-    if s > cu1:
-        ops.attn_fwd(q[cu1:], k[cu1:], v[cu1:], o[cu1:], heads)
+    pad_segment_attention_(qkv, cat, cu1, heads, d, qnorm=qnorm)
 
 
-def pad_segment_attention_(qkv: torch.Tensor, cat: torch.Tensor, cu1: int, heads: int, d: int):
+def pad_segment_attention_(qkv: torch.Tensor, cat: torch.Tensor, cu1: int, heads: int, d: int, qnorm=None):
     if qkv.shape[0] > cu1:
-        ops.attn_fwd(qkv[cu1:, :d], qkv[cu1:, d:2 * d], qkv[cu1:, 2 * d:], cat[cu1:, :d], heads)
+        if qnorm is None:
+            ops.attn_fwd(qkv[cu1:, :d], qkv[cu1:, d:2 * d], qkv[cu1:, 2 * d:], cat[cu1:, :d], heads)
+        else:
+            w_txt, eps = qnorm[1], qnorm[5]
+            ops.attn_fwd(qkv[cu1:, :d], qkv[cu1:, d:2 * d], qkv[cu1:, 2 * d:], cat[cu1:, :d], heads,
+                         qnorm=(w_txt, w_txt, None, None, 0, eps))
 
 
 def parallel_attention(hybrid_seq_parallel_attn, q, k, v, img_q_len, img_kv_len, cu_seqlens_q, cu_seqlens_kv):
diff --git a/hunyuanvideo_efficiency_amd/modules/models.py b/hunyuanvideo_efficiency_amd/modules/models.py
--- a/hunyuanvideo_efficiency_amd/modules/models.py
+++ b/hunyuanvideo_efficiency_amd/modules/models.py
@@ -25,6 +25,12 @@
         self.patches = None
         self.final = None
         self.xq = self.xs = self.catq = self.cats = None
+        self.kbound = None
+
+    def clear_bounds(self, n_slots: int):
+        if self.kbound is None or self.kbound.shape[0] < n_slots:
+            self.kbound = torch.empty(n_slots, ops.BOUND_WORDS, dtype=torch.int32, device=self.x.device)
+        self.kbound.zero_()
 
     def fp8_buffers(self):
         if self.xq is None:
@@ -40,6 +46,10 @@
 def _use_fp8_mfma(block, *layers) -> bool:
     return bool(getattr(block, "fp8_mfma", False)) and all(
         l.weight.dtype == torch.float8_e4m3fn and l.in_features >= 384 and l.in_features % 128 == 0 for l in layers)
+
+
+def _fused_qknorm(sp, ws: _Workspace) -> bool:
+    return sp is None and ops.FUSED_QKNORM and ws.x.is_cuda
 
 
 def _ln(ws: _Workspace, lo: int, hi: int, shift, scale, fp8: bool):
@@ -113,12 +123,14 @@
         self.deterministic = False
 
     def run(self, ws: _Workspace, s_img: int, s_txt: int, vec: torch.Tensor, cu1: int,
-            cos: Optional[torch.Tensor], sin: Optional[torch.Tensor]):
+            cos: Optional[torch.Tensor], sin: Optional[torch.Tensor], slot: int = 0):
         d = ws.x.shape[1]
         H = self.heads_num
         streams = (("txt", s_img, s_img + s_txt, 0), ("img", 0, s_img, s_img if cos is not None else 0))
         sp = self.hybrid_seq_parallel_attn
         overlap = sp is not None and hasattr(sp, "send") and H % 2 == 0
+        fused = _fused_qknorm(sp, ws)
+        bound = ws.kbound[slot] if fused else None
         mods = {}
         fp8 = {s: _use_fp8_mfma(self, getattr(self, f"{s}_attn_qkv"), getattr(self, f"{s}_attn_proj"), getattr(self, f"{s}_mlp").fc1,
                                 getattr(self, f"{s}_mlp").fc2) for s in ("img", "txt")}
@@ -134,13 +146,18 @@
                 _sp_chunked_qkv(sp, ws, qkv_l, fp8[s], qw, kw, cos, sin, s_img, cu1, n_rope, H, d)
             else:
                 _gemm(ws, qkv_l, "xmod", lo, hi, fp8[s], out=ws.qkv[lo:hi])
-                ops.qknorm_rope_(ws.qkv[lo:hi], qw, kw, cos, sin, n_rope, H, d)
+                if fused:
+                    ops.knorm_rope_kmax_(ws.qkv[lo:hi], kw, cos, sin, n_rope, H, d, bound=bound,
+                                         n_bound=s_img if s == "img" else cu1 - s_img)
+                else:
+                    ops.qknorm_rope_(ws.qkv[lo:hi], qw, kw, cos, sin, n_rope, H, d)
         segs = None
         if overlap:
             segs = sp.attend_async(ws.cat, ws.cat.stride(0))
             pad_segment_attention_(ws.qkv, ws.cat, cu1, H, d)
         else:
-            segment_attention_(sp, ws.qkv, ws.cat, s_img, cu1, H, d)
+            qnorm = (self.img_attn_q_norm.weight, self.txt_attn_q_norm.weight, cos, sin, s_img, 1e-6, bound) if fused else None
+            segment_attention_(sp, ws.qkv, ws.cat, s_img, cu1, H, d, qnorm=qnorm)
         streams = (streams[1], streams[0])
         for s, lo, hi, _ in streams:
             _, _, g1, sh2, sc2, g2 = mods[s]
@@ -162,6 +179,7 @@
         assert img.shape[0] == 1, "batch 1 (cfg-distilled model, SURVEY.md top)"
         s_img, s_txt, d = img.shape[1], txt.shape[1], img.shape[2]
         ws = _Workspace(s_img, s_txt, d, self.img_mlp.fc1.weight.shape[0], img.device)
+        ws.clear_bounds(1)
         ws.x[:s_img].copy_(img[0])
         ws.x[s_img:].copy_(txt[0])
         cu1 = int(cu_seqlens_q[1])
@@ -199,7 +217,7 @@
         self.deterministic = False
 
     def run(self, ws: _Workspace, s_img: int, s_txt: int, vec: torch.Tensor, cu1: int,
-            cos: Optional[torch.Tensor], sin: Optional[torch.Tensor]):
+            cos: Optional[torch.Tensor], sin: Optional[torch.Tensor], slot: int = 0):
         d, H = self.hidden_size, self.heads_num
         m = ops.linear_smallm(vec, self.modulation.linear.w(), self.modulation.linear.bias, silu_in=True)
         shift, scale, gate = m[0, :d], m[0, d:2 * d], m[0, 2 * d:]
@@ -222,8 +240,14 @@
             return
         else:
             _gemm(ws, self.linear1, "xmod", 0, s_all, fp8, out=ws.qkv, n_split=3 * d, out1=ws.cat[:, d:], act1=ops.ACT_GELU_TANH)
-            ops.qknorm_rope_(ws.qkv, self.q_norm.weight, self.k_norm.weight, cos, sin, n_rope, H, d)
-            segment_attention_(sp, ws.qkv, ws.cat, s_img, cu1, H, d)
+            if _fused_qknorm(sp, ws):
+                bound = ws.kbound[slot]
+                ops.knorm_rope_kmax_(ws.qkv, self.k_norm.weight, cos, sin, n_rope, H, d, bound=bound, n_bound=cu1)
+                qnorm = (self.q_norm.weight, self.q_norm.weight, cos, sin, s_img, 1e-6, bound)
+            else:
+                ops.qknorm_rope_(ws.qkv, self.q_norm.weight, self.k_norm.weight, cos, sin, n_rope, H, d)
+                qnorm = None
+            segment_attention_(sp, ws.qkv, ws.cat, s_img, cu1, H, d, qnorm=qnorm)
         _gemm(ws, self.linear2, "cat", 0, s_all, fp8, out=ws.x, gate=gate, res=ws.x)
 
     def forward(self, x, vec, txt_len, cu_seqlens_q=None, cu_seqlens_kv=None, max_seqlen_q=None, max_seqlen_kv=None,
@@ -231,6 +255,7 @@
         assert x.shape[0] == 1
         s, d = x.shape[1], x.shape[2]
         ws = _Workspace(s - txt_len, txt_len, d, self.mlp_hidden_dim, x.device)
+        ws.clear_bounds(1)
         ws.x.copy_(x[0])
         cos, sin = freqs_cis if freqs_cis is not None else (None, None)
         self.run(ws, s - txt_len, txt_len, vec.to(BF16).contiguous(), int(cu_seqlens_q[1]), cos, sin)
@@ -382,10 +407,12 @@
         cos = freqs_cos.to(device=dev, dtype=torch.float32).contiguous() if freqs_cos is not None else None
         sin = freqs_sin.to(device=dev, dtype=torch.float32).contiguous() if freqs_sin is not None else None
 
-        for block in self.double_blocks:
-            block.run(ws, s_img, s_txt, vec, cu1, cos, sin)
-        for block in self.single_blocks:
-            block.run(ws, s_img, s_txt, vec, cu1, cos, sin)
+        n_double = len(self.double_blocks)
+        ws.clear_bounds(n_double + len(self.single_blocks))
+        for i, block in enumerate(self.double_blocks):
+            block.run(ws, s_img, s_txt, vec, cu1, cos, sin, slot=i)
+        for i, block in enumerate(self.single_blocks):
+            block.run(ws, s_img, s_txt, vec, cu1, cos, sin, slot=n_double + i)
 
         img = self.final_layer.run(ws, s_img, vec)
         out = ops.unpatchify(img, self.unpatchify_channels, ot, oh, ow)
diff --git a/hunyuanvideo_efficiency_amd/ops.py b/hunyuanvideo_efficiency_amd/ops.py
--- a/hunyuanvideo_efficiency_amd/ops.py
+++ b/hunyuanvideo_efficiency_amd/ops.py
@@ -9,6 +9,9 @@
 BF16 = torch.bfloat16
 ACT_NONE, ACT_GELU_TANH, ACT_SILU = 0, 1, 2
 PROFILE_ATTN = None
+FUSED_QKNORM = True
+KNORM_ROWS = 64
+BOUND_WORDS = 64
 
 
 def _chk(t: torch.Tensor, dtype, name: str, last_contig: bool = True):
@@ -71,6 +74,23 @@
         return out
     _lib.call("qknorm_rope_bf16", qkv, q_weight, k_weight, cos, sin, n,
                                                n_rope, n_heads, 128, ld, k_offset, eps)
+    return qkv
+
+
+def knorm_rope_kmax_(qkv, k_weight, cos, sin, n_rope: int, n_heads: int, k_offset: int, bound=None, n_bound: int = 0,
+                     eps: float = 1e-6):
+    _chk(qkv, BF16, "qkv")
+    n, w, ld = _rows(qkv, "qkv")
+    _chk(k_weight, BF16, "k_weight")
+    assert k_offset + n_heads * 128 <= w and 0 <= n_rope <= n and 0 <= n_bound <= n
+    if n_rope > 0:
+        _chk(cos, torch.float32, "cos"), _chk(sin, torch.float32, "sin")
+        assert cos.is_contiguous() and sin.is_contiguous() and cos.shape[-1] == 128 and cos.shape[0] >= n_rope and sin.shape == cos.shape
+    if n_bound > 0:
+        _chk(bound, torch.int32, "bound")
+        assert bound.is_contiguous() and bound.numel() == BOUND_WORDS
+    _lib.call("knorm_rope_kmax_bf16", qkv, k_weight, cos if n_rope > 0 else None, sin if n_rope > 0 else None, n, n_rope, n_bound,
+              n_heads, 128, ld, k_offset, eps, bound if n_bound > 0 else None)
     return qkv
 
 
@@ -147,7 +167,15 @@
     return ws
 
 
-def attn_fwd(q, k, v, out, n_heads: int, scale: Optional[float] = None, kv_split_workspace: bool = True):
+def _attn_split_workspace(n_q, n_kv, n_heads, device):
+    if n_kv < 64 * 64 or ((n_q + 255) // 256) * n_heads >= 16 * 256:
+        return None
+    return _attn_workspace(n_q, n_kv, n_heads, device)
+
+
+def attn_fwd(q, k, v, out, n_heads: int, scale: Optional[float] = None, kv_split_workspace: bool = True, qnorm=None, bound=None):
+    if qnorm is None:
+        assert bound is None, "a caller-filled bound area goes with qnorm"
     for t, nm in ((q, "q"), (k, "k"), (v, "v"), (out, "out")):
         _chk(t, BF16, nm)
         assert t.dim() == 2
@@ -159,10 +187,26 @@
     if prof is not None:
         e0, e1 = torch.cuda.Event(enable_timing=True), torch.cuda.Event(enable_timing=True)
         e0.record()
-    ws = _attn_workspace(n_q, n_kv, n_heads, q.device) if kv_split_workspace else None
-    _lib.call("attn_fwd_bf16", q, k, v, out, q.stride(0), k.stride(0), v.stride(0),
-                                            out.stride(0), n_q, n_kv, n_heads, 128, scale, ws,
-                                            0 if ws is None else ws.numel())
+    if qnorm is not None:
+        w_lo, w_hi, cos, sin, n_split, eps = qnorm
+        _chk(w_lo, BF16, "q_weight_lo"), _chk(w_hi, BF16, "q_weight_hi")
+        assert w_lo.numel() == 128 and w_hi.numel() == 128 and 0 <= n_split <= n_q
+        if cos is not None and n_split > 0:
+            _chk(cos, torch.float32, "cos"), _chk(sin, torch.float32, "sin")
+            assert cos.is_contiguous() and sin.is_contiguous() and cos.shape[-1] == 128 and cos.shape[0] >= n_split and sin.shape == cos.shape
+        else:
+            cos = sin = None
+        if bound is not None:
+            _chk(bound, torch.int32, "bound")
+            assert bound.is_contiguous() and bound.numel() == BOUND_WORDS
+        ws = _attn_split_workspace(n_q, n_kv, n_heads, q.device) if kv_split_workspace else None
+        _lib.call("attn_fwd_qnorm_bf16", q, k, v, out, q.stride(0), k.stride(0), v.stride(0), out.stride(0), n_q, n_kv, n_heads, 128,
+                  scale, w_lo, w_hi, cos, sin, n_split, eps, bound, ws, 0 if ws is None else ws.numel())
+    else:
+        ws = _attn_workspace(n_q, n_kv, n_heads, q.device) if kv_split_workspace else None
+        _lib.call("attn_fwd_bf16", q, k, v, out, q.stride(0), k.stride(0), v.stride(0),
+                                                out.stride(0), n_q, n_kv, n_heads, 128, scale, ws,
+                                                0 if ws is None else ws.numel())
     if prof is not None:
         e1.record()
         prof.append((e0, e1, n_q, n_kv, n_heads))
diff --git a/include/hv_kernels.h b/include/hv_kernels.h
--- a/include/hv_kernels.h
+++ b/include/hv_kernels.h
@@ -25,6 +25,11 @@
                                 int64_t k_offset, float eps, void* dst, int64_t dst_ld, int heads_per_block,
                                 int64_t dst_block_stride, hipStream_t stream);
 
+int hv_knorm_rope_kmax_bf16(void* qkv, const void* k_weight, const float* cos_tab, const float* sin_tab, int64_t n_rows,
+                            int64_t n_rope, int64_t n_bound, int n_heads, int head_dim, int64_t ld, int64_t k_offset, float eps,
+                            void* bound, hipStream_t stream);
+int hv_knorm_rows_per_block(void);
+
 int hv_gemm_bf16(const void* A, int64_t lda, const void* W, int64_t ldw, const void* bias, int M, int N, int K,
                  void* out0, int64_t ld0, int act0, int n_split, void* out1, int64_t ld1, int act1,
                  const void* gate, const void* res, int64_t ld_res, hipStream_t stream);
@@ -38,6 +43,11 @@
 int hv_attn_fwd_bf16(const void* q, const void* k, const void* v, void* o, int64_t stride_q, int64_t stride_k,
                      int64_t stride_v, int64_t stride_o, int n_q, int n_kv, int n_heads, int head_dim,
                      float scale, void* workspace, int64_t workspace_bytes, hipStream_t stream);
+
+int hv_attn_fwd_qnorm_bf16(const void* q, const void* k, const void* v, void* o, int64_t stride_q, int64_t stride_k,
+                           int64_t stride_v, int64_t stride_o, int n_q, int n_kv, int n_heads, int head_dim, float scale,
+                           const void* q_weight_lo, const void* q_weight_hi, const float* cos_tab, const float* sin_tab,
+                           int n_split, float eps, void* bound, void* workspace, int64_t workspace_bytes, hipStream_t stream);
 
 int64_t hv_attn_workspace_bytes(int n_q, int n_kv, int n_heads);
 int hv_attn_w4_loop_signature(void);
```
